# bhansconnect/burn-ppo

Hardware: AMD Instinct MI355X
Metric: env-steps/sec (rollout+GAE+PPO update) at 1/2/4/8 MI355X; steps-to-475-return CartPole (higher is better)
Workload: dtype f32

## Files before the change

### burn-ppo_amd/csrc/bppo_api.hip

```cpp
#include <algorithm>
#include <pthread.h>
#include <chrono>
#include <cmath>
#include <cstdio>
#include <cstdlib>
#include <cstring>
#include <new>
#include <thread>
#include <sys/prctl.h>
#include <x86intrin.h>
#include "bppo_internal.h"
#include "shuffle_host.h"
#include "bppo_wide.h"

using namespace bppo;

namespace bppo {
static double tsc_per_ms() {
    static double v = 0.0;
    if (v == 0.0) {
        const auto t0 = std::chrono::steady_clock::now();
        const uint64_t c0 = __rdtsc();
        std::this_thread::sleep_for(std::chrono::milliseconds(20));
        const uint64_t c1 = __rdtsc();
// ... 210 lines not shown
    }
    c->net = make_layout(*cfg, c->D, c->G, c->A);
    const size_t np = c->net.n_params;
    const size_t TN = (size_t)c->T * c->N;
    c->adam_t.assign(2 * c->net.n_layers, 0);
    TRY(dalloc(c, &c->d_params, np));
    TRY(dalloc(c, &c->d_m1, np));
    TRY(dalloc(c, &c->d_m2, np));
    TRY(dalloc(c, &c->d_grad, np + 64));
    c->slab_rows = 256 * 8;
    c->relu_mfma = cfg->relu ? 1 : 0;
    if (!c->wide) TRY(dalloc(c, &c->d_slab, c->slab_rows * (np + 64)));
    TRY(dalloc(c, &c->d_cp, (size_t)4 * c->N));
    TRY(dalloc(c, &c->d_steps, (size_t)c->N));
    TRY(dalloc(c, &c->d_env_pos, (size_t)c->N));
    TRY(dalloc(c, &c->d_ep_ret, (size_t)c->N * c->P));
    TRY(dalloc(c, &c->d_ep_len, (size_t)c->N));
    if (!c->wide) TRY(dalloc(c, &c->d_obs, TN * c->D));
    TRY(dalloc(c, &c->d_rew, TN));
    TRY(dalloc(c, &c->d_rew_raw, TN));
    TRY(dalloc(c, &c->d_done, TN));
    TRY(dalloc(c, &c->d_val, TN));
    TRY(dalloc(c, &c->d_logp, TN));
    TRY(dalloc(c, &c->d_adv, TN));
    TRY(dalloc(c, &c->d_ret, TN));
    TRY(dalloc(c, &c->d_act, TN));
    if (!c->wide || cfg->normalize_returns) TRY(dalloc(c, &c->d_X, TN));
    if (!c->wide && cfg->hidden_size == 64 && cfg->num_hidden == 2 && cfg->relu)
    {
        TRY(dalloc(c, &c->d_gumbel, TN * 2));
        TRY(dalloc(c, &c->d_rpool, (size_t)RPOOL_K * c->N));
        TRY(dalloc(c, &c->d_rpos, (size_t)RPOOL_K * c->N));
    }
    TRY(dalloc(c, &c->d_on, (size_t)2 * c->D + 1));
    if (!c->wide) TRY(dalloc(c, &c->d_obs_part, (size_t)c->N * 2 * c->D));
    if (!c->wide) {
        TRY(dalloc(c, &c->d_act_in, (size_t)c->N));
        TRY(dalloc(c, &c->d_scr_r, (size_t)c->N));
        TRY(dalloc(c, &c->d_bxc, (size_t)c->N * c->D));
        BPPO_HIP(c, hipMalloc((void **)&c->d_scr_d, (size_t)c->N));
    }
    TRY(dalloc(c, &c->d_rn_returns, (size_t)c->N * c->P));
    TRY(dalloc(c, &c->d_rn_stats, 4));
    TRY(dalloc(c, &c->d_scan_agg, (TN + 4095) / 4096 + 1));
    TRY(dalloc(c, &c->d_last_v, (size_t)c->N));
    c->eps_cap = (int)std::min<size_t>((size_t)c->T * c->N + 4096, (size_t)INT32_MAX / 2);
    TRY(dalloc(c, &c->d_eps, (size_t)c->eps_cap));
    TRY(dalloc(c, &c->d_ep_count, 1));
    TRY(dalloc(c, &c->d_ep_sum, ROLL_HOST_WORDS));
    TRY(dalloc(c, &c->d_err, 1));
    TRY(dalloc(c, &c->d_perm_base, TN));
    c->d_perm = c->d_perm_base;
    TRY(dalloc(c, &c->d_perm_ep, TN * (size_t)cfg->num_epochs));
    TRY(dalloc(c, &c->d_inv_ep, TN * (size_t)cfg->num_epochs));
    TRY(dalloc(c, &c->d_advpart, (size_t)ADV_STREAM_BLOCKS * ADV_STREAM_MAXM * 4));
    BPPO_HIP(c, make_side_stream(dev, &c->fy_stream));
    for (int e = 0; e < cfg->num_epochs && e < SHUF_MAX_EPOCHS; e++)
        BPPO_HIP(c, hipEventCreateWithFlags(&c->fy_ev[e], hipEventDisableTiming));
    TRY(dalloc(c, &c->d_fy, 4 * TN));
    TRY(dalloc(c, &c->d_scan, TN / 8192 + 2));
    BPPO_HIP(c, fy_ranges_init(c->fyr, (uint32_t)TN));
    TRY(dalloc(c, &c->d_red, 4 * 1024 + 64));
    TRY(dalloc(c, &c->d_mb_stats, (size_t)4 * std::max(cfg->num_minibatches, 2)));
    c->d_mb_cur = c->d_mb_stats;
    TRY(dalloc(c, &c->d_rows, (size_t)cfg->num_epochs * cfg->num_minibatches * (WM_COUNT + 4)));
    BPPO_HIP(c, hipHostMalloc((void **)&c->h_rows,
                              sizeof(float) * (size_t)cfg->num_epochs * cfg->num_minibatches * (WM_COUNT + 4),
                              hipHostMallocDefault));
    if (!c->wide && cfg->hidden_size == 64 && cfg->num_hidden == 2 && cfg->relu && c->D == 5)
    {
        BPPO_HIP(c, hipMalloc((void **)&c->d_rowA, sizeof(float4) * 2 * TN));
        BPPO_HIP(c, hipMalloc((void **)&c->d_rowB, sizeof(float2) * TN));
    }
    BPPO_HIP(c, hipHostMalloc((void **)&c->h_red, sizeof(double) * (4 * 1024 + 64 + 2 * ROLL_HOST_WORDS),
                              hipHostMallocDefault));
    BPPO_HIP(c, hipEventCreateWithFlags(&c->ev_upd, hipEventDisableTiming));
    BPPO_HIP(c, hipEventRecord(c->ev_upd, c->stream));
    BPPO_HIP(c, hipEventCreateWithFlags(&c->ev_block, hipEventDisableTiming | hipEventBlockingSync));
    for (int i = 0; i < TM_SLOTS; i++) {
        BPPO_HIP(c, hipEventCreate(&c->ev[i][0]));
        BPPO_HIP(c, hipEventCreate(&c->ev[i][1]));
    }
    for (int i = 0; i < bppo_ctx::MB_EV; i++) {
        BPPO_HIP(c, hipEventCreate(&c->mb_ev[i][0]));
        BPPO_HIP(c, hipEventCreate(&c->mb_ev[i][1]));
    }
    c->rng_key = seed_key(cfg->seed);
    c->rng_pos = 0;
    TRY(c->shuf.init(dev, c->rng_key, cfg->rng_stream, (uint32_t)TN, cfg->num_epochs, TN * (uint64_t)c->A, c->err,
                     cfg->shuffle_windows != 0));
    c->on_mean.assign(c->D, 0.0); c->on_m2.assign(c->D, 0.0); c->on_count = 0;
    c->u_ret = c->d_ret; c->u_val = c->d_val;
    c->shaping_v.assign(1, cfg->reward_shaping_coef); c->shaping_s.assign(1, 0);
    if (cfg->normalize_values) TRY(popart_alloc(c));
    if (c->wide) {
        TRY(wide_init(c));
        TRY(wide_reset(c));
        TRY(wide_pack(c));
    } else {
        TRY(launch_cartpole_reset(c));
    }
    BPPO_HIP(c, sync_stream(c));
    return BPPO_OK;
}

extern "C" bppo_status bppo_create(const bppo_config *cfg, int hip_device, void *hip_stream,
                                   bppo_ctx **out) {
    if (!cfg || !out) return BPPO_ERR_ARG;
    bppo_ctx *c = new bppo_ctx();
    bppo_status s = ctx_init(c, cfg, hip_device, hip_stream);
    *out = c;
    return s;
}

extern "C" void bppo_destroy(bppo_ctx *c) {
    if (!c) return;
    if (c->ev_thread.joinable()) c->ev_thread.join();
    if (c->ev_stream) { (void)hipStreamSynchronize(c->ev_stream); (void)hipStreamDestroy(c->ev_stream); }
    if (c->ev_gae) (void)hipEventDestroy(c->ev_gae);
    if (c->ev_copied) (void)hipEventDestroy(c->ev_copied);
    for (float *h : {c->h_ev_v, c->h_ev_r, c->h_ev_valid}) if (h) (void)hipHostFree(h);
    if (c->fy_stream) (void)hipStreamSynchronize(c->fy_stream);
    c->shuf.shutdown();
    if (c->stream) (void)hipStreamSynchronize(c->stream);
    wide_free(c);
    popart_free(c);
    void *ptrs[] = {c->d_params, c->d_m1, c->d_m2, c->d_grad, c->d_slab, c->d_cp, c->d_steps,
                    c->d_env_pos, c->d_ep_ret, c->d_ep_len, c->d_obs, c->d_rew, c->d_rew_raw,
                    c->d_done, c->d_val, c->d_logp, c->d_adv, c->d_ret, c->d_act, c->d_X, c->d_on,
                    c->d_obs_part, c->d_rn_returns, c->d_rn_stats, c->d_scan_agg, c->d_last_v,
                    c->d_eps, c->d_ep_count, c->d_ep_sum, c->d_err, c->d_perm_base, c->d_perm_ep, c->d_inv_ep, c->d_advpart, c->d_fy, c->d_scan,
                    c->d_red, c->d_mb_stats, c->d_gumbel, c->d_rpool, c->d_rpos, c->d_rows, c->d_rowA, c->d_rowB};
    for (void *p : ptrs) if (p) (void)hipFree(p);
    fy_ranges_free(c->fyr);
    if (c->h_red) (void)hipHostFree(c->h_red);
    if (c->h_rows) (void)hipHostFree(c->h_rows);
    if (c->ev_block) (void)hipEventDestroy(c->ev_block);
    if (c->ev_upd) (void)hipEventDestroy(c->ev_upd);
    for (int i = 0; i < TM_SLOTS; i++) {
        if (c->ev[i][0]) (void)hipEventDestroy(c->ev[i][0]);
        if (c->ev[i][1]) (void)hipEventDestroy(c->ev[i][1]);
    }
    for (auto &pr : c->mb_ev)
        for (hipEvent_t e : pr) if (e) (void)hipEventDestroy(e);
    if (c->fy_stream) { (void)hipStreamSynchronize(c->fy_stream); (void)hipStreamDestroy(c->fy_stream); }
    for (hipEvent_t e : c->fy_ev) if (e) (void)hipEventDestroy(e);
    if (c->own_stream && c->stream) (void)hipStreamDestroy(c->stream);
    delete c;
}

extern "C" size_t bppo_num_params(const bppo_ctx *c) { return c ? c->net.n_params : 0; }

static void drop_prefetch(bppo_ctx *c) {
    if (!c->prefetched) return;
    c->prefetched = false;
    c->collected = 0;
    c->gae_done = 0;
}

extern "C" bppo_status bppo_params_set(bppo_ctx *c, const float *h, size_t n) {
    if (!c || !h || n != c->net.n_params) { if (c) c->err = "params_set: size mismatch"; return BPPO_ERR_ARG; }
    drop_prefetch(c);
    BPPO_HIP(c, hipMemcpyAsync(c->d_params, h, n * 4, hipMemcpyHostToDevice, c->stream));
    if (c->wide) TRY(wide_pack(c));
    BPPO_HIP(c, sync_stream(c));
    return BPPO_OK;
}

extern "C" bppo_status bppo_params_get(bppo_ctx *c, float *h, size_t n) {
    if (!c || !h || n != c->net.n_params) { if (c) c->err = "params_get: size mismatch"; return BPPO_ERR_ARG; }
    BPPO_HIP(c, hipMemcpyAsync(h, c->d_params, n * 4, hipMemcpyDeviceToHost, c->stream));
    BPPO_HIP(c, sync_stream(c));
    return BPPO_OK;
}

extern "C" bppo_status bppo_forward(bppo_ctx *c, const float *obs, const float *priv, int32_t B,
                                    float *logits, float *values) {
    if (!c || !obs || B <= 0) return BPPO_ERR_ARG;
    if (c->wide) return wide_forward_host(c, obs, priv, B, logits, values);
    struct Scratch { float *p[3] = {nullptr, nullptr, nullptr}; ~Scratch() { for (float *q : p) (void)hipFree(q); } } t;
    BPPO_HIP(c, hipMalloc((void **)&t.p[0], sizeof(float) * (size_t)B * c->D));
    BPPO_HIP(c, hipMalloc((void **)&t.p[1], sizeof(float) * (size_t)B * c->A));
    BPPO_HIP(c, hipMalloc((void **)&t.p[2], sizeof(float) * (size_t)B));
    float *d_o = t.p[0], *d_l = t.p[1], *d_v = t.p[2];
    BPPO_HIP(c, hipMemcpyAsync(d_o, obs, sizeof(float) * (size_t)B * c->D, hipMemcpyHostToDevice, c->stream));
    bppo_status s = launch_forward_rows(c, d_o, B, d_l, d_v);
    if (s == BPPO_OK) {
        if (logits) BPPO_HIP(c, hipMemcpyAsync(logits, d_l, sizeof(float) * (size_t)B * c->A, hipMemcpyDeviceToHost, c->stream));
        if (values) BPPO_HIP(c, hipMemcpyAsync(values, d_v, sizeof(float) * (size_t)B, hipMemcpyDeviceToHost, c->stream));
    }
    const bppo_status ss = sync_stream(c) == hipSuccess ? BPPO_OK : BPPO_ERR_HIP;
    return s != BPPO_OK ? s : ss;
}

extern "C" bppo_status bppo_rng_get(bppo_ctx *c, uint64_t *p) {
    if (!c || !p) return BPPO_ERR_ARG;
    *p = c->rng_pos;
    return BPPO_OK;
}
extern "C" bppo_status bppo_rng_set(bppo_ctx *c, uint64_t p) {
    if (!c) return BPPO_ERR_ARG;
    drop_prefetch(c);
    c->shuf_slot = -1;
    c->fy_slot = -1; c->fy_done = 0;
    c->rng_pos = p;
    return BPPO_OK;
}

extern "C" bppo_status bppo_rng_fill_bytes(bppo_ctx *c, uint8_t *dst, size_t n) {
    if (!c || (!dst && n)) return BPPO_ERR_ARG;
    const size_t nw = (n + 3) / 4;
    uint32_t blk[16];
    uint64_t cached = ~0ull;
    for (size_t i = 0; i < nw; i++) {
        const uint64_t pos = c->rng_pos + i;
        if ((pos >> 4) != cached) { chacha12_block(c->rng_key, pos >> 4, c->cfg.rng_stream, blk); cached = pos >> 4; }
        const uint32_t w = blk[pos & 15];
        for (int b = 0; b < 4 && 4 * i + b < n; b++) dst[4 * i + b] = (uint8_t)(w >> (8 * b));
    }
    c->rng_pos += nw;
    c->shuf_slot = -1;
    c->fy_slot = -1; c->fy_done = 0;
    return BPPO_OK;
}

extern "C" bppo_status bppo_rng_from_seed(bppo_ctx *c, const uint8_t *seed) {
    if (!c || !seed) return BPPO_ERR_ARG;
    drop_prefetch(c);
    Key8 k;
    for (int i = 0; i < 8; i++)
        k.k[i] = (uint32_t)seed[4 * i] | ((uint32_t)seed[4 * i + 1] << 8) | ((uint32_t)seed[4 * i + 2] << 16) |
                 ((uint32_t)seed[4 * i + 3] << 24);
    BPPO_HIP(c, sync_stream(c));
    BPPO_HIP(c, hipStreamSynchronize(c->fy_stream));
    c->fy_slot = -1; c->fy_done = 0;
    c->shuf.shutdown();
    c->shuf.~ShuffleEngine();
    new (&c->shuf) ShuffleEngine();
    c->rng_key = k;
    c->rng_pos = 0;
    c->shuf_slot = -1;
    const size_t TN = (size_t)c->T * c->N;
    TRY(c->shuf.init(c->dev, c->rng_key, c->cfg.rng_stream, (uint32_t)TN, c->cfg.num_epochs, TN * (uint64_t)c->A, c->err,
                     c->cfg.shuffle_windows != 0));
    return BPPO_OK;
}

extern "C" bppo_status bppo_rng_key_get(bppo_ctx *c, uint32_t *key) {
    if (!c || !key) return BPPO_ERR_ARG;
    for (int i = 0; i < 8; i++) key[i] = c->rng_key.k[i];
    return BPPO_OK;
}

extern "C" bppo_status bppo_optimizer_get(bppo_ctx *c, float *m1, float *m2, int32_t *steps, size_t n) {
    if (!c || n != c->net.n_params) { if (c) c->err = "optimizer_get: size mismatch"; return BPPO_ERR_ARG; }
    if (m1) BPPO_HIP(c, hipMemcpyAsync(m1, c->d_m1, n * 4, hipMemcpyDeviceToHost, c->stream));
    if (m2) BPPO_HIP(c, hipMemcpyAsync(m2, c->d_m2, n * 4, hipMemcpyDeviceToHost, c->stream));
    BPPO_HIP(c, sync_stream(c));
    if (steps)
        for (int l = 0; l < c->net.n_layers; l++)
            for (int k = 0; k < 2; k++) steps[2 * c->net.rec[l] + k] = c->adam_t[2 * l + k];
    return BPPO_OK;
}

extern "C" bppo_status bppo_optimizer_set(bppo_ctx *c, const float *m1, const float *m2, const int32_t *steps,
                                          size_t n) {
    if (!c || !m1 || !m2 || !steps || n != c->net.n_params) {
        if (c) c->err = "optimizer_set: size mismatch";
        return BPPO_ERR_ARG;
    }
    BPPO_HIP(c, hipMemcpyAsync(c->d_m1, m1, n * 4, hipMemcpyHostToDevice, c->stream));
    BPPO_HIP(c, hipMemcpyAsync(c->d_m2, m2, n * 4, hipMemcpyHostToDevice, c->stream));
    BPPO_HIP(c, sync_stream(c));
    for (int l = 0; l < c->net.n_layers; l++)
        for (int k = 0; k < 2; k++) c->adam_t[2 * l + k] = steps[2 * c->net.rec[l] + k];
    return BPPO_OK;
}

extern "C" size_t bppo_num_param_tensors(const bppo_ctx *c) { return c ? c->adam_t.size() : 0; }

extern "C" bppo_status bppo_vecenv_reset(bppo_ctx *c) {
    if (!c) return BPPO_ERR_ARG;
    drop_prefetch(c);
    TRY(c->wide ? wide_reset(c) : launch_cartpole_reset(c));
    BPPO_HIP(c, sync_stream(c));
    return BPPO_OK;
}

extern "C" bppo_status bppo_vecenv_observe(bppo_ctx *c, float *obs, int32_t *players, uint8_t *masks,
                                           float *priv) {
    (void)priv; (void)masks;
    if (!c) return BPPO_ERR_ARG;
    if (c->wide) return wide_observe_host(c, obs, players, masks, priv);
    if (obs) {
        TRY(launch_cartpole_observe(c, c->d_bxc));
        BPPO_HIP(c, hipMemcpyAsync(obs, c->d_bxc, sizeof(float) * (size_t)c->N * c->D, hipMemcpyDeviceToHost, c->stream));
        BPPO_HIP(c, sync_stream(c));
    }
    if (players) std::fill(players, players + c->N, 0);
    return BPPO_OK;
}

extern "C" bppo_status bppo_vecenv_step(bppo_ctx *c, const int32_t *actions, float *obs, float *rewards,
                                        uint8_t *dones, bppo_episode *eps, int32_t cap, int32_t *n_eps) {
    if (!c || !actions) return BPPO_ERR_ARG;
    const int N = c->N;
    if (c->wide) {
        BPPO_HIP(c, hipMemsetAsync(c->d_ep_count, 0, 4, c->stream));
        int32_t cnt = 0;
        TRY(wide_step_host(c, actions, obs, rewards, dones, &cnt));
        if (n_eps) *n_eps = cnt;
        if (eps && cap > 0 && cnt > 0) {
            std::vector<EpisodeRec> recs(std::min(cnt, c->eps_cap));
            BPPO_HIP(c, hipMemcpy(recs.data(), c->d_eps, sizeof(EpisodeRec) * recs.size(), hipMemcpyDeviceToHost));
            std::sort(recs.begin(), recs.end(), [](const EpisodeRec &a, const EpisodeRec &b) {
                return a.env_index < b.env_index; });
            for (int i = 0; i < (int)recs.size() && i < cap; i++) {
                std::memcpy(eps[i].total_reward, recs[i].total_reward, sizeof(float) * BPPO_MAX_PLAYERS);
                eps[i].length = recs[i].length; eps[i].env_index = recs[i].env_index;
                eps[i].step = recs[i].step; eps[i].pad = 0;
            }
        }
        return BPPO_OK;
    }
    int32_t *d_a = c->d_act_in; float *d_r = c->d_scr_r, *d_o = c->d_bxc; uint8_t *d_d = c->d_scr_d;
    BPPO_HIP(c, hipMemcpyAsync(d_a, actions, sizeof(int32_t) * N, hipMemcpyHostToDevice, c->stream));
    BPPO_HIP(c, hipMemsetAsync(c->d_ep_count, 0, 4, c->stream));
    TRY(launch_cartpole_vecenv_step(c, d_a, d_r, d_d, d_o));
    if (rewards) BPPO_HIP(c, hipMemcpyAsync(rewards, d_r, sizeof(float) * N, hipMemcpyDeviceToHost, c->stream));
    if (dones) BPPO_HIP(c, hipMemcpyAsync(dones, d_d, N, hipMemcpyDeviceToHost, c->stream));
    if (obs) BPPO_HIP(c, hipMemcpyAsync(obs, d_o, sizeof(float) * (size_t)N * c->D, hipMemcpyDeviceToHost, c->stream));
    int32_t cnt = 0;
    BPPO_HIP(c, hipMemcpyAsync(&cnt, c->d_ep_count, 4, hipMemcpyDeviceToHost, c->stream));
    BPPO_HIP(c, sync_stream(c));
    if (n_eps) *n_eps = cnt;
    if (eps && cap > 0 && cnt > 0) {
        std::vector<EpisodeRec> recs(std::min(cnt, c->eps_cap));
        BPPO_HIP(c, hipMemcpy(recs.data(), c->d_eps, sizeof(EpisodeRec) * recs.size(), hipMemcpyDeviceToHost));
        std::sort(recs.begin(), recs.end(), [](const EpisodeRec &a, const EpisodeRec &b) {
            return a.env_index < b.env_index; });
        for (int i = 0; i < (int)recs.size() && i < cap; i++) {
            std::memcpy(eps[i].total_reward, recs[i].total_reward, sizeof(float) * BPPO_MAX_PLAYERS);
            eps[i].length = recs[i].length; eps[i].env_index = recs[i].env_index;
            eps[i].step = recs[i].step; eps[i].pad = 0;
        }
    }
    return BPPO_OK;
}

extern "C" bppo_status bppo_vecenv_set_step(bppo_ctx *c, uint64_t s) {
    if (!c) return BPPO_ERR_ARG;
    c->env_step = s;
    return BPPO_OK;
}

extern "C" bppo_status bppo_set_reward_shaping_schedule(bppo_ctx *c, const double *values, const uint64_t *steps,
                                                        int32_t n) {
    if (!c || n < 0 || (n > 0 && (!values || !steps))) return BPPO_ERR_ARG;
    std::vector<double> v(values, values + n);
    std::vector<uint64_t> s(steps, steps + n);
    if (bppo::schedule_get(v, s, 0) < 0.0) { c->err = "reward_shaping_coef must be >= 0"; return BPPO_ERR_ARG; }
    c->shaping_v = std::move(v); c->shaping_s = std::move(s);
    return BPPO_OK;
}

extern "C" bppo_status bppo_obs_norm_get(bppo_ctx *c, double *mean, double *m2, double *count) {
    if (!c) return BPPO_ERR_ARG;
    std::vector<double> h(2 * c->D + 1);
    BPPO_HIP(c, hipMemcpyAsync(h.data(), c->d_on, sizeof(double) * h.size(), hipMemcpyDeviceToHost, c->stream));
    BPPO_HIP(c, sync_stream(c));
    if (mean) std::memcpy(mean, h.data(), sizeof(double) * c->D);
    if (m2) std::memcpy(m2, h.data() + c->D, sizeof(double) * c->D);
    if (count) *count = h[2 * c->D];
    return BPPO_OK;
}

extern "C" bppo_status bppo_obs_norm_set(bppo_ctx *c, const double *mean, const double *m2, double count) {
    if (!c || !mean || !m2) return BPPO_ERR_ARG;
    drop_prefetch(c);
    std::vector<double> h(2 * c->D + 1);
    std::memcpy(h.data(), mean, sizeof(double) * c->D);
    std::memcpy(h.data() + c->D, m2, sizeof(double) * c->D);
    h[2 * c->D] = count;
    BPPO_HIP(c, hipMemcpyAsync(c->d_on, h.data(), sizeof(double) * h.size(), hipMemcpyHostToDevice, c->stream));
    BPPO_HIP(c, sync_stream(c));
    return BPPO_OK;
}

extern "C" bppo_status bppo_ret_norm_get(bppo_ctx *c, double *mvc, double *returns) {
    if (!c) return BPPO_ERR_ARG;
    if (mvc) BPPO_HIP(c, hipMemcpyAsync(mvc, c->d_rn_stats, sizeof(double) * 3, hipMemcpyDeviceToHost, c->stream));
    if (returns) BPPO_HIP(c, hipMemcpyAsync(returns, c->d_rn_returns, sizeof(double) * (size_t)c->N * c->P, hipMemcpyDeviceToHost, c->stream));
    BPPO_HIP(c, sync_stream(c));
    return BPPO_OK;
}

extern "C" bppo_status bppo_ret_norm_set(bppo_ctx *c, const double *mvc, const double *returns) {
    if (!c) return BPPO_ERR_ARG;
    drop_prefetch(c);
    if (mvc) BPPO_HIP(c, hipMemcpyAsync(c->d_rn_stats, mvc, sizeof(double) * 3, hipMemcpyHostToDevice, c->stream));
    if (returns) BPPO_HIP(c, hipMemcpyAsync(c->d_rn_returns, returns, sizeof(double) * (size_t)c->N * c->P, hipMemcpyHostToDevice, c->stream));
    BPPO_HIP(c, sync_stream(c));
    return BPPO_OK;
}

extern "C" bppo_status bppo_popart_get(bppo_ctx *c, double *st) {
    if (!c || !st) return BPPO_ERR_ARG;
    st[0] = c->pa_mean; st[1] = c->pa_m2; st[2] = c->pa_count; st[3] = c->pa_eps;
    return BPPO_OK;
}

extern "C" bppo_status bppo_popart_set(bppo_ctx *c, const double *st) {
    if (!c || !st) return BPPO_ERR_ARG;
    drop_prefetch(c);
    c->pa_mean = st[0]; c->pa_m2 = st[1]; c->pa_count = st[2]; c->pa_eps = st[3];
    return BPPO_OK;
}

static bppo_status tm_begin(bppo_ctx *c, int slot) {
    BPPO_HIP(c, hipEventRecord(c->ev[slot][0], c->stream));
    return BPPO_OK;
}
static bppo_status tm_end(bppo_ctx *c, int slot) {
    BPPO_HIP(c, hipEventRecord(c->ev[slot][1], c->stream));
    return BPPO_OK;
}
static void tm_read(bppo_ctx *c, int slot) {
    float ms = 0;
    if (event_ms(c->ev[slot][0], c->ev[slot][1], &ms)) c->last_ms[slot] = ms;
}

static bppo_status fy_enqueue_ready(bppo_ctx *c, int slot) {
    const size_t B = (size_t)c->T * c->N;
    if (slot != c->fy_slot) {
        c->fy_slot = slot; c->fy_done = 0;
        BPPO_HIP(c, hipStreamWaitEvent(c->fy_stream, c->ev_upd, 0));
    }
    if (c->shuf.failed(c->err)) return BPPO_ERR_HIP;
    while (c->fy_done < c->cfg.num_epochs && c->shuf.epoch_ready(slot, c->fy_done)) {
        const int e = c->fy_done;
        if (c->shuf.failed(c->err)) return BPPO_ERR_HIP;
        BPPO_HIP(c, hipStreamWaitEvent(c->fy_stream, c->shuf.ev[slot][e], 0));
        if (e > 0) BPPO_HIP(c, hipStreamWaitEvent(c->fy_stream, c->fy_ev[e - 1], 0));
        BPPO_HIP(c, hipEventRecord(c->ev[TM_SHUFFLE][0], c->fy_stream));
        BPPO_HIP(c, fisher_yates_device(c->shuf.d_J[slot] + (size_t)e * B, (uint32_t)B, c->d_fy, c->d_scan,
                                        c->d_perm_ep + (size_t)e * B, c->fy_stream, &c->fyr,
                                        c->d_inv_ep + (size_t)e * B));
        BPPO_HIP(c, hipEventRecord(c->ev[TM_SHUFFLE][1], c->fy_stream));
        BPPO_HIP(c, hipEventRecord(c->fy_ev[e], c->fy_stream));
        c->fy_done++;
    }
    return BPPO_OK;
}

static double *roll_host(bppo_ctx *c, int slot) { return c->h_red + 4 * 1024 + 64 + (size_t)slot * ROLL_HOST_WORDS; }

static bppo_status collect_enqueue(bppo_ctx *c, bool summary) {
    const size_t TN = (size_t)c->T * c->N;
    c->coll_slot ^= 1;
    const int tro = c->coll_slot ? TM_ROLLOUT_B : TM_ROLLOUT, trn = c->coll_slot ? TM_RETNORM_B : TM_RETNORM;
    if (c->wide) {
        BPPO_HIP(c, hipMemsetAsync(c->d_ep_count, 0, 4, c->stream));
        BPPO_HIP(c, hipMemsetAsync(c->d_err, 0, 4, c->stream));
    }
    const uint64_t base = c->rng_pos;
    TRY(tm_begin(c, tro));
    if (c->wide) TRY(wide_collect(c, base));
    else {
        TRY(launch_cartpole_rollout(c, base, nullptr, nullptr, c->cfg.normalize_obs));
        TRY(popart_denorm(c, c->d_val, TN));
    }
    TRY(tm_end(c, tro));
    if (!opp_active(c)) {
        c->shuf_slot = c->shuf.ensure(base + TN * (uint64_t)c->A);
        TRY(fy_enqueue_ready(c, c->shuf_slot));
    }
    if (opp_active(c)) {
        TRY(opp_rollout_end(c));
    } else {
        c->rng_pos = base + TN * (uint64_t)c->A;
        c->shuf_slot = c->shuf.ensure(c->rng_pos);
    }
    if (c->cfg.normalize_obs) TRY(launch_obs_norm_merge(c));
    TRY(tm_begin(c, trn));
    if (c->cfg.normalize_returns) TRY(launch_return_norm(c));
    else if (!c->wide) BPPO_HIP(c, hipMemcpyAsync(c->d_rew, c->d_rew_raw, TN * 4, hipMemcpyDeviceToDevice, c->stream));
    TRY(tm_end(c, trn));
    int32_t *hv = reinterpret_cast<int32_t *>(roll_host(c, c->coll_slot));
    if (summary) {
        TRY(launch_episode_summary(c, c->d_ep_sum));
        BPPO_HIP(c, hipMemcpyAsync(hv, c->d_ep_sum, sizeof(double) * ROLL_HOST_WORDS, hipMemcpyDeviceToHost, c->stream));
    } else {
        BPPO_HIP(c, hipMemcpyAsync(&hv[0], c->d_ep_count, 4, hipMemcpyDeviceToHost, c->stream));
        BPPO_HIP(c, hipMemcpyAsync(&hv[1], c->d_err, 4, hipMemcpyDeviceToHost, c->stream));
    }
    c->collected = 1; c->gae_done = 0;
    c->rollout_rng_pos[c->coll_slot] = c->rng_pos;
    return BPPO_OK;
}

static bppo_status collect_finish(bppo_ctx *c, bppo_rollout_info *info, int slot) {
    float ms = 0;
    const int tro = slot ? TM_ROLLOUT_B : TM_ROLLOUT, trn = slot ? TM_RETNORM_B : TM_RETNORM;
    if (event_ms(c->ev[tro][0], c->ev[tro][1], &ms)) c->last_ms[TM_ROLLOUT] = ms;
    if (event_ms(c->ev[trn][0], c->ev[trn][1], &ms)) c->last_ms[TM_RETNORM] = ms;
    const int32_t *hv = reinterpret_cast<const int32_t *>(roll_host(c, slot));
    const double *part = roll_host(c, slot) + 2;
    if (hv[1] & 2) { c->err = "Empty action mask: an env has no valid action"; return BPPO_ERR_EMPTY_MASK; }
    if (hv[1] & 1) { c->err = "NaN/Inf in log probs — model producing corrupt logits"; return BPPO_ERR_NONFINITE; }
    if (hv[1] & 4) { c->err = "opponent pool: pos_to_opp names a model index outside [0, n_models)"; return BPPO_ERR_ARG; }
    if (hv[1] & 8) { c->err = "Invalid action: outside the env's action mask"; return BPPO_ERR_ARG; }
    if (hv[1]) { c->err = "collect_rollouts: unknown device error flag"; return BPPO_ERR_HIP; }
    if (info) {
        info->episodes = hv[0];
        info->rng_word_pos = c->rollout_rng_pos[slot];
        info->mean_return = 0; info->mean_length = 0;
        const int n = std::min(hv[0], c->eps_cap);
        if (n > 0) {
            double sr = 0, sl = 0;
            for (int b = 0; b < EP_SUMMARY_BLOCKS; b++) { sr += part[2 * b]; sl += part[2 * b + 1]; }
            info->mean_return = (float)(sr / n); info->mean_length = (float)(sl / n);
        }
    }
    return BPPO_OK;
}

extern "C" bppo_status bppo_collect_rollouts(bppo_ctx *c, bppo_rollout_info *info) {
    if (!c) return BPPO_ERR_ARG;
    if (c->prefetched) c->prefetched = false;
    else TRY(collect_enqueue(c, info != nullptr));
    BPPO_HIP(c, sync_stream(c));
    return collect_finish(c, info, c->coll_slot);
}

extern "C" bppo_status bppo_rollout_episodes(bppo_ctx *c, bppo_episode *eps, int32_t cap, int32_t *n) {
    if (!c) return BPPO_ERR_ARG;
    int32_t cnt = 0;
    BPPO_HIP(c, hipMemcpyAsync(&cnt, c->d_ep_count, 4, hipMemcpyDeviceToHost, c->stream));
    BPPO_HIP(c, sync_stream(c));
    int m = std::min(cnt, c->eps_cap);
    std::vector<EpisodeRec> recs(m);
    if (m) {
        BPPO_HIP(c, hipMemcpyAsync(recs.data(), c->d_eps, sizeof(EpisodeRec) * m, hipMemcpyDeviceToHost, c->stream));
        BPPO_HIP(c, sync_stream(c));
    }
    std::sort(recs.begin(), recs.end(), [](const EpisodeRec &a, const EpisodeRec &b) {
        return a.step != b.step ? a.step < b.step : a.env_index < b.env_index; });
    for (int i = 0; i < m && i < cap; i++) {
        std::memcpy(eps[i].total_reward, recs[i].total_reward, sizeof(float) * BPPO_MAX_PLAYERS);
        eps[i].length = recs[i].length; eps[i].env_index = recs[i].env_index;
        eps[i].step = recs[i].step; eps[i].pad = 0;
    }
    if (n) *n = cnt;
    return BPPO_OK;
}

static bppo_status gae_enqueue(bppo_ctx *c) {
    c->prefetched = false;
    if (c->wide) {
        TRY(tm_begin(c, TM_GAE));
        TRY(wide_bootstrap_gae(c));
        TRY(tm_end(c, TM_GAE));
        c->gae_done = 1;
        return BPPO_OK;
    }
    TRY(tm_begin(c, TM_BOOT));
    TRY(launch_bootstrap(c, nullptr, nullptr, c->cfg.normalize_obs));
    TRY(popart_denorm(c, c->d_last_v, (size_t)c->N));
    TRY(tm_end(c, TM_BOOT));
    TRY(tm_begin(c, TM_GAE));
    bool packed = false;
    hipError_t he = hipSuccess;
    bppo_status s = launch_gae_1p(c->d_rew, c->d_done, c->d_val, c->d_last_v, c->T, c->N,
                                  (float)c->cfg.gamma, (float)c->cfg.gae_lambda, c->d_adv, c->d_ret,
                                  c->stream, c->rows_from_rollout ? c->d_rowB : nullptr, &packed, &he);
    c->rows_packed = packed;
    if (s != BPPO_OK) return he != hipSuccess ? hip_fail(c, he, "k_gae_1p launch") : s;
    TRY(tm_end(c, TM_GAE));
    c->gae_done = 1;
    return BPPO_OK;
}

extern "C" bppo_status bppo_compute_gae(bppo_ctx *c) {
    if (!c || !c->collected) { if (c) c->err = "compute_gae before collect_rollouts"; return BPPO_ERR_ARG; }
    TRY(gae_enqueue(c));
    BPPO_HIP(c, sync_stream(c));
    if (!c->wide) tm_read(c, TM_BOOT);
    tm_read(c, TM_GAE);
    return BPPO_OK;
}

static float ev_reference_f32(const float *v, const float *r, const float *valid, size_t n_all) {
#pragma clang fp contract(off)
    size_t n_ = 0;
    float s_r = 0.0f, s_res = 0.0f;
    for (size_t i = 0; i < n_all; i++) {
        if (valid && !(valid[i] > 0.5f)) continue;
        s_r += r[i];
        s_res += r[i] - v[i];
        n_++;
    }
    const float n = (float)n_;
    if (n < 2.0f) return 0.0f;
    const float mr = s_r / n, mres = s_res / n;
    float q_r = 0.0f, q_res = 0.0f;
    for (size_t i = 0; i < n_all; i++) {
        if (valid && !(valid[i] > 0.5f)) continue;
        const float d = r[i] - mr;
        q_r += d * d;
        const float e = (r[i] - v[i]) - mres;
        q_res += e * e;
    }
    const float vr = q_r / n;
    if (vr < 1e-8f) return 0.0f;
    return 1.0f - (q_res / n) / vr;
}

extern "C" bppo_status bppo_set_explained_variance_mode(bppo_ctx *c, int32_t mode) {
    if (!c || mode < 0 || mode > 1) return BPPO_ERR_ARG;
    if (mode == 1 && !c->h_ev_v) {
        const size_t TN = (size_t)c->T * c->N;
        hipStream_t st = nullptr;
        hipEvent_t e_gae = nullptr, e_cp = nullptr;
        float *hv = nullptr, *hr = nullptr, *hm = nullptr;
        hipError_t e = hipStreamCreateWithFlags(&st, hipStreamNonBlocking);
        if (e == hipSuccess) e = hipEventCreateWithFlags(&e_gae, hipEventDisableTiming);
        if (e == hipSuccess) e = hipEventCreateWithFlags(&e_cp, hipEventDisableTiming | hipEventBlockingSync);
        if (e == hipSuccess) e = hipHostMalloc((void **)&hv, TN * 4, hipHostMallocDefault);
        if (e == hipSuccess) e = hipHostMalloc((void **)&hr, TN * 4, hipHostMallocDefault);
        if (e == hipSuccess) e = hipHostMalloc((void **)&hm, TN * 4, hipHostMallocDefault);
        if (e != hipSuccess) {
            for (float *h : {hv, hr, hm}) if (h) (void)hipHostFree(h);
            if (e_cp) (void)hipEventDestroy(e_cp);
            if (e_gae) (void)hipEventDestroy(e_gae);
            if (st) (void)hipStreamDestroy(st);
            return hip_fail(c, e, "explained-variance reference mode: allocation");
        }
        c->ev_stream = st; c->ev_gae = e_gae; c->ev_copied = e_cp;
        c->h_ev_r = hr; c->h_ev_valid = hm;
        c->h_ev_v = hv;
    }
    c->ev_mode = mode;
    return BPPO_OK;
}

extern "C" bppo_status bppo_debug_record_params(bppo_ctx *c, float *host, int32_t max_minibatches) {
    if (!c || max_minibatches < 0) return BPPO_ERR_ARG;
    c->dbg_params = max_minibatches > 0 ? host : nullptr;
    c->dbg_params_max = host ? max_minibatches : 0;
    return BPPO_OK;
}

extern "C" bppo_status bppo_set_minibatch_kernel(bppo_ctx *c, int32_t mode) {
    if (!c || mode < 0 || mode > 2) return BPPO_ERR_ARG;
    c->mb_kernel = mode;
    return BPPO_OK;
}

static bppo_status ev_reference_begin(bppo_ctx *c, const float *d_valid) {
    const size_t TN = (size_t)c->T * c->N;
    if (c->ev_thread.joinable()) c->ev_thread.join();
    BPPO_HIP(c, hipEventRecord(c->ev_gae, c->stream));
    BPPO_HIP(c, hipStreamWaitEvent(c->ev_stream, c->ev_gae, 0));
    BPPO_HIP(c, hipMemcpyAsync(c->h_ev_v, c->d_val, TN * 4, hipMemcpyDeviceToHost, c->ev_stream));
    BPPO_HIP(c, hipMemcpyAsync(c->h_ev_r, c->d_ret, TN * 4, hipMemcpyDeviceToHost, c->ev_stream));
    if (d_valid) BPPO_HIP(c, hipMemcpyAsync(c->h_ev_valid, d_valid, TN * 4, hipMemcpyDeviceToHost, c->ev_stream));
    BPPO_HIP(c, hipEventRecord(c->ev_copied, c->ev_stream));
    const bool vf = d_valid != nullptr;
    c->ev_thread = std::thread([c, TN, vf]() {
        (void)pthread_setname_np(pthread_self(), "bppo-ev");
        (void)hipEventSynchronize(c->ev_copied);
        c->ev_ref = ev_reference_f32(c->h_ev_v, c->h_ev_r, vf ? c->h_ev_valid : nullptr, TN);
    });
    return BPPO_OK;
}

extern "C" bppo_status bppo_ppo_update(bppo_ctx *c, double lr, double ent_coef, bppo_update_metrics *m) {
    if (!c || !c->gae_done) { if (c) c->err = "ppo_update before compute_gae"; return BPPO_ERR_ARG; }
    const bool opp = opp_active(c);
    if (opp) {
        if (c->fy_done > 0) BPPO_HIP(c, hipStreamWaitEvent(c->stream, c->fy_ev[c->fy_done - 1], 0));
        c->fy_slot = -1; c->fy_done = 0;
        c->d_perm = c->d_perm_base;
        TRY(opp_compact_valid(c));
    }
    if (!opp && c->shuf_slot < 0) c->shuf_slot = c->shuf.ensure(c->rng_pos);
    const int slot = c->shuf_slot;
    const size_t B = opp ? (size_t)c->n_valid : (size_t)c->T * c->N;
    std::vector<uint32_t> Jh(opp ? std::max<size_t>(B, 1) * c->cfg.num_epochs : 0);
    uint64_t opp_pos = c->rng_pos;
    const int M = c->cfg.num_minibatches;
    const size_t base_mb = B / M, rem = B % M;
    const int np = (int)c->net.n_params;
    const int NM = WM_COUNT;
    std::vector<float> rows;
    int epochs_run = 0;
    bool stop = false;
    double wait_ms = 0.0;
    TRY(tm_begin(c, TM_UPDATE));
    struct EvCopyGuard {
        bppo_ctx *c; bool armed = false;
        ~EvCopyGuard() { if (armed) (void)hipStreamWaitEvent(c->stream, c->ev_copied, 0); }
    } ev_guard{c};
    if (c->ev_mode == 1) { TRY(ev_reference_begin(c, opp ? c->d_valid : nullptr)); ev_guard.armed = true; }
    TRY(popart_update_begin(c, opp ? c->d_valid : nullptr));
    if (c->d_rowA && !c->rows_packed) TRY(launch_pack_rows(c));
    c->rows_packed = false;
    float fw_ms = 0, sh_ms = 0;
    const bool deferred = c->cfg.target_kl < 0 && !(c->allreduce && c->world > 1 && !c->allreduce_async);
    int nrow = 0;
    const int last_run_mb = (base_mb > 0 || (c->allreduce && c->world > 1)) ? M - 1 : (int)rem - 1;
    bool fw_recorded = false;
    bool first_mb = true;
    size_t rows_done = 0;
    for (int ep = 0; ep < c->cfg.num_epochs && !stop; ep++) {
        epochs_run++;
        hipEvent_t s0 = c->ev[TM_SHUFFLE][0], s1 = c->ev[TM_SHUFFLE][1];
        if (opp) {
            uint32_t *J = Jh.data() + (size_t)ep * B;
            auto w0 = std::chrono::steady_clock::now();
            opp_pos = shuffle_walk_host(c->rng_key, c->cfg.rng_stream, opp_pos, (uint32_t)B, J);
            wait_ms += std::chrono::duration<double, std::milli>(std::chrono::steady_clock::now() - w0).count();
            BPPO_HIP(c, hipMemcpyAsync(c->d_Jopp, J, sizeof(uint32_t) * B, hipMemcpyHostToDevice, c->stream));
            BPPO_HIP(c, hipEventRecord(s0, c->stream));
            if (B) TRY(launch_fisher_yates(c, c->d_Jopp, (uint32_t)B));
            if (B) TRY(opp_map_perm(c, (uint32_t)B));
            BPPO_HIP(c, hipEventRecord(s1, c->stream));
        } else {
            if (slot != c->fy_slot || ep >= c->fy_done) {
                auto w0 = std::chrono::steady_clock::now();
                c->shuf.wait_epoch(slot, ep);
                wait_ms += std::chrono::duration<double, std::milli>(std::chrono::steady_clock::now() - w0).count();
            }
            TRY(fy_enqueue_ready(c, slot));
            BPPO_HIP(c, hipStreamWaitEvent(c->stream, c->fy_ev[ep], 0));
            c->d_perm = c->d_perm_ep + (size_t)ep * B;
        }
        const bool lockstep = c->allreduce && c->world > 1;
        if (B == 0 && !lockstep) continue;
        if (B) TRY(launch_epoch_adv_stats(c, (uint32_t)B, M, opp ? nullptr : c->d_inv_ep + (size_t)ep * B));
        size_t start = 0;
        for (int mb = 0; mb < M; mb++) {
            const size_t sz = base_mb + ((size_t)mb < rem ? 1 : 0);
            if (sz == 0 && !lockstep) continue;
            const bool fw_timed = !deferred || (ep == c->cfg.num_epochs - 1 && mb == last_run_mb);
            if (fw_timed) BPPO_HIP(c, hipEventRecord(c->ev[TM_FWDBWD][0], c->stream));
            c->d_mb_cur = c->d_mb_stats + 4 * mb;
            float c1[64], c2[64];
            for (int t = 0; t < 2 * c->net.n_layers; t++) {
                int ti = ++c->adam_t[t];
                c1[t] = 1.0f - powi_f32(0.9f, ti);
                c2[t] = 1.0f - powi_f32(0.999f, ti);
            }
            float *metric_dst = c->d_rows + (size_t)nrow * (NM + 4);
            const bool multi = c->allreduce && c->world > 1;
            if (sz == 0) {
                BPPO_HIP(c, hipMemsetAsync(c->d_grad, 0, sizeof(float) * ((size_t)np + 64), c->stream));
                BPPO_HIP(c, hipMemsetAsync(c->d_mb_cur, 0, sizeof(float) * 4, c->stream));
                static const float ninf = -INFINITY;
                BPPO_HIP(c, hipMemcpyAsync(c->d_grad + np + GRAD_VEMAX_LOCAL, &ninf, sizeof(float),
                                           hipMemcpyHostToDevice, c->stream));
            } else if (c->wide) {
                if (c->dbg_params && nrow < c->dbg_params_max)
                    BPPO_HIP(c, hipMemcpyAsync(c->dbg_params + (size_t)nrow * np, c->d_params, sizeof(float) * np,
                                               hipMemcpyDeviceToHost, c->stream));
                TRY(wide_minibatch(c, (uint32_t)start, (uint32_t)sz, ent_coef, first_mb));
            } else {
                if (c->dbg_params && nrow < c->dbg_params_max)
                    BPPO_HIP(c, hipMemcpyAsync(c->dbg_params + (size_t)nrow * np, c->d_params, sizeof(float) * np,
                                               hipMemcpyDeviceToHost, c->stream));
                TRY(launch_minibatch(c, (uint32_t)start, (uint32_t)sz, (float)ent_coef, first_mb));
            }
            if (fw_timed) { BPPO_HIP(c, hipEventRecord(c->ev[TM_FWDBWD][1], c->stream)); fw_recorded = true; }
            first_mb = false;
            if (multi) {
                if (!c->allreduce_async) BPPO_HIP(c, sync_stream(c));
                if (c->allreduce(c->d_grad, (size_t)np + NM, c->allreduce_user) != 0) {
                    c->err = "all-reduce callback failed";
                    return BPPO_ERR_COMM;
                }
            }
            TRY(launch_adam(c, (float)lr, c1, c2, metric_dst, NM));
            if (c->wide) TRY(wide_pack(c));
            nrow++;
            if (!deferred) {
                std::vector<float> row(NM + 4);
                BPPO_HIP(c, hipMemcpyAsync(row.data(), c->d_rows + (size_t)(nrow - 1) * (NM + 4), sizeof(float) * (NM + 4),
                                           hipMemcpyDeviceToHost, c->stream));
                BPPO_HIP(c, sync_stream(c));
                float ms = 0;
                if (event_ms(c->ev[TM_FWDBWD][0], c->ev[TM_FWDBWD][1], &ms)) fw_ms = ms;
                if (mb == 0 && event_ms(s0, s1, &ms)) sh_ms = ms;
                rows.insert(rows.end(), row.begin(), row.end());
            }
            if (!deferred && c->cfg.target_kl >= 0) {
                const float *row = &rows[rows.size() - (NM + 4)];
                const float n = row[10] > 0 ? row[10] : 1.0f;
                if (row[3] / n > (float)c->cfg.target_kl) { stop = true; rows_done = start + sz; break; }
            }
            start += sz;
        }
    }
    if (deferred && nrow > 0) {
        rows.resize((size_t)nrow * (NM + 4));
        BPPO_HIP(c, hipMemcpyAsync(c->h_rows, c->d_rows, sizeof(float) * rows.size(), hipMemcpyDeviceToHost, c->stream));
    }
    TRY(tm_end(c, TM_UPDATE));
    c->last_wait_ms = wait_ms;
    c->last_walk_ms = 0.0;
    c->last_met = 0;
    if (opp) {
        c->rng_pos = opp_pos;
        c->last_walk_ms = wait_ms;
        BPPO_HIP(c, hipStreamSynchronize(c->stream));
    } else {
        c->rng_pos = c->shuf.win ? c->shuf.job_end(slot) : c->shuf.end_pos[slot][epochs_run - 1];
        for (int e = 0; e < epochs_run; e++) {
            c->last_walk_ms += c->shuf.walk_ms[slot][e];
            c->last_met += c->shuf.coalesced[slot][e] >= 0 && e > 0;
        }
        c->last_spec_mwords = (double)c->shuf.spec_words.exchange(0) * 1e-6;
        c->last_true_mwords = (double)c->shuf.true_words.exchange(0) * 1e-6;
        c->last_walk_cpu_ms = (double)c->shuf.tsc_walk.exchange(0) / tsc_per_ms();
        c->last_words_cpu_ms = (double)c->shuf.tsc_words.exchange(0) / tsc_per_ms();
        c->shuf_slot = -1;
        if (c->fy_slot == slot && c->fy_done > 0)
            BPPO_HIP(c, hipStreamWaitEvent(c->stream, c->fy_ev[c->fy_done - 1], 0));
        c->fy_slot = -1;
        c->fy_done = 0;
        BPPO_HIP(c, c->shuf.release(slot, c->stream));
        c->shuf.ensure(c->rng_pos + (uint64_t)c->T * c->N * (uint64_t)c->A);
    }
    TRY(popart_target_stats(c, stop ? epochs_run - 1 : epochs_run, rows_done, opp ? c->d_valid : nullptr));
    TRY(launch_explained_variance(c, opp ? c->d_valid : nullptr));
    if (ev_guard.armed) { ev_guard.armed = false; BPPO_HIP(c, hipStreamWaitEvent(c->stream, c->ev_copied, 0)); }
    BPPO_HIP(c, hipEventRecord(c->ev_upd, c->stream));
    if (c->prefetch_next) {
        c->prefetch_next = false;
        c->env_step = c->prefetch_env_step;
        TRY(collect_enqueue(c, true));
        c->prefetched = true;
        BPPO_HIP(c, wait_event(c, c->ev_upd));
    } else {
        BPPO_HIP(c, sync_stream(c));
    }
    if (deferred && nrow > 0) {
        std::memcpy(rows.data(), c->h_rows, sizeof(float) * rows.size());
        float ms = 0;
        if (fw_recorded && event_ms(c->ev[TM_FWDBWD][0], c->ev[TM_FWDBWD][1], &ms)) fw_ms = ms;
        if (event_ms(c->ev[TM_SHUFFLE][0], c->ev[TM_SHUFFLE][1], &ms)) sh_ms = ms;
    }
    double ev4[4];
    explained_variance_sums(c, ev4);
    if (c->ev_thread.joinable()) c->ev_thread.join();
    tm_read(c, TM_UPDATE);
    if (c->mb_ev_n > 0) {
        double sum = 0.0, ks[2] = {0.0, 0.0};
        float lo = INFINITY, hi = 0.0f;
        int n = 0, kn[2] = {0, 0};
        for (int i = 0; i < c->mb_ev_n; i++) {
            float ms = 0.0f;
            if (!event_ms(c->mb_ev[i][0], c->mb_ev[i][1], &ms)) continue;
            sum += ms; lo = std::min(lo, ms); hi = std::max(hi, ms); n++;
            ks[c->mb_ev_split[i]] += ms; kn[c->mb_ev_split[i]]++;
        }
        if (n) { c->mb_k_mean = (float)(sum / n); c->mb_k_min = lo; c->mb_k_max = hi; }
        c->mb_k_exact = kn[0] ? (float)(ks[0] / kn[0]) : 0.0f;
        c->mb_k_split = kn[1] ? (float)(ks[1] / kn[1]) : 0.0f;
        c->mb_ev_n = 0;
    }
    c->mb_launch = 0;
    c->last_ms[TM_FWDBWD] = fw_ms;
    c->last_ms[TM_SHUFFLE] = sh_ms;
    c->last_rows = rows;
    if (m) {
        std::memset(m, 0, sizeof *m);
        const int nup = (int)(rows.size() / (NM + 4));
        float tp = 0, tv = 0, th = 0, tk = 0, tc = 0, tl = 0, tvm = 0, trm = 0, tam = 0, tas = 0;
        float tamin = INFINITY, tamax = -INFINITY, tvem = 0, tves = 0, tvemax = -INFINITY;
        float tav = 0, tevp = 0;
        for (int u = 0; u < nup; u++) {
            const float *r = &rows[(size_t)u * (NM + 4)];
            const float n = r[10] > 0 ? r[10] : 1.0f;
            const float pl = r[0] / n, vl = 0.5f * (r[1] / n), h = r[2] / n;
            tp += pl; tv += vl; th += h; tk += r[3] / n; tc += r[4] / n;
            tl += pl + vl * (float)c->cfg.value_coef + (-h) * (float)ent_coef;
            tvm += r[5] / n; trm += r[6] / n;
            const float vem = r[7] / n;
            tvem += vem;
            const double var = n > 1 ? ((double)r[8] - (double)n * vem * vem) / (double)(n - 1) : 0.0;
            tves += sqrtf((float)std::max(var, 0.0));
            tvemax = std::max(tvemax, r[9]);
            tav += r[WM_VALID] / n;
            tevp += r[WM_NCHOICE] > 0 ? r[WM_HV] / r[WM_NCHOICE] : 0.0f;
            tam += r[NM]; tas += r[NM + 1];
            tamin = std::min(tamin, r[NM + 2]); tamax = std::max(tamax, r[NM + 3]);
        }
        const float n = (float)nup;
        m->policy_loss = tp / n; m->value_loss = tv / n; m->entropy = th / n;
        m->entropy_scaled = m->entropy / logf((float)c->A);
        m->approx_kl = tk / n; m->clip_fraction = tc / n; m->total_loss = tl / n;
        m->value_mean = tvm / n; m->returns_mean = trm / n;
        m->adv_mean_raw = tam / n; m->adv_std_raw = tas / n; m->adv_min_raw = tamin; m->adv_max_raw = tamax;
        m->value_error_mean = tvem / n; m->value_error_std = tves / n; m->value_error_max = tvemax;
        const double Bn = (double)B;
        const double mr = ev4[0] / Bn, vr = ev4[1] / Bn - mr * mr;
        const double mres = ev4[2] / Bn, vres = ev4[3] / Bn - mres * mres;
        m->explained_variance = (B < 2 || vr < 1e-8) ? 0.0f : (float)(1.0 - vres / vr);
        if (c->ev_mode == 1) m->explained_variance = c->ev_ref;
        if (c->cfg.env_kind != BPPO_ENV_CARTPOLE) { m->avg_valid_actions = tav / n; m->entropy_valid_pct = tevp / n; }
        m->num_updates = nup; m->epochs_run = epochs_run;
        m->value_norm_target_mean = m->value_norm_target_std = NAN;
        m->value_norm_rescale_mag = c->pa_rescale_mag;
        if (c->cfg.normalize_values && c->pa_tcount > 0) {
            const double mean = c->pa_tsum / c->pa_tcount, var = c->pa_tsq / c->pa_tcount - mean * mean;
            m->value_norm_target_mean = (float)mean;
            m->value_norm_target_std = (float)std::sqrt(std::max(var, 0.0));
        }
    }
    c->collected = 0; c->gae_done = 0;
    return BPPO_OK;
}

extern "C" bppo_status bppo_train_step(bppo_ctx *c, double lr, double ent_coef, bppo_rollout_info *info,
                                       bppo_update_metrics *m) {
    if (!c) return BPPO_ERR_ARG;
    const auto t0 = std::chrono::steady_clock::now();
    c->sync_wait_ms = 0.0;
    if (c->prefetched) c->prefetched = false;
    else TRY(collect_enqueue(c, info != nullptr));
    TRY(gae_enqueue(c));
    const bppo_status us = bppo_ppo_update(c, lr, ent_coef, m);
    if (us == BPPO_OK) { if (!c->wide) tm_read(c, TM_BOOT); tm_read(c, TM_GAE); }
    const bppo_status cs = collect_finish(c, info, c->coll_slot);
    c->last_host_ms = std::chrono::duration<double, std::milli>(std::chrono::steady_clock::now() - t0).count() -
                      c->sync_wait_ms;
    c->last_sync_ms = c->sync_wait_ms;
    return cs != BPPO_OK ? cs : us;
}

extern "C" bppo_status bppo_train_steps(bppo_ctx *c, int32_t n, const double *lr, const double *ent_coef,
                                        uint64_t global_step0, bppo_rollout_info *infos, bppo_update_metrics *ms,
                                        const char *const *phase_keys, int32_t nkeys, float *phase_sums) {
    if (!c || n < 0 || !lr || !ent_coef || (nkeys > 0 && (!phase_keys || !phase_sums))) return BPPO_ERR_ARG;
    for (int k = 0; k < nkeys; k++) phase_sums[k] = 0.0f;
    const uint64_t TN = (uint64_t)c->T * c->N * (uint64_t)c->world;
    for (int32_t k = 0; k < n; k++) {
        const auto t0 = std::chrono::steady_clock::now();
        c->sync_wait_ms = 0.0;
        if (!c->prefetched) { c->env_step = global_step0 + (uint64_t)k * TN; TRY(collect_enqueue(c, true)); }
        c->prefetched = false;
        const int slot = c->coll_slot;
        TRY(gae_enqueue(c));
        c->prefetch_next = k + 1 < n;
        c->prefetch_env_step = global_step0 + (uint64_t)(k + 1) * TN;
        const bppo_status us = bppo_ppo_update(c, lr[k], ent_coef[k], ms ? &ms[k] : nullptr);
        c->prefetch_next = false;
        if (us != BPPO_OK) { (void)sync_stream(c); c->collected = c->prefetched ? 1 : 0; return us; }
        if (!c->wide) tm_read(c, TM_BOOT);
        tm_read(c, TM_GAE);
        const bppo_status cs = collect_finish(c, infos ? &infos[k] : nullptr, slot);
        if (cs != BPPO_OK) { (void)sync_stream(c); c->collected = c->prefetched ? 1 : 0; return cs; }
        c->last_host_ms = std::chrono::duration<double, std::milli>(std::chrono::steady_clock::now() - t0).count() -
                          c->sync_wait_ms;
        c->last_sync_ms = c->sync_wait_ms;
        for (int q = 0; q < nkeys; q++) {
            float v = 0.0f;
            if (bppo_last_kernel_ms(c, phase_keys[q], &v) == BPPO_OK) phase_sums[q] += v;
        }
    }
    return BPPO_OK;
}

static bppo_status check_world(bppo_ctx *c, int32_t world) {
    if (world > 1 && c->cfg.normalize_values) {
        if (c->d_pa_gather) { BPPO_HIP(c, hipFree(c->d_pa_gather)); c->d_pa_gather = nullptr; }
        BPPO_HIP(c, hipMalloc((void **)&c->d_pa_gather, sizeof(float) * 9 * (size_t)world));
    }
    return BPPO_OK;
}

extern "C" bppo_status bppo_set_rank(bppo_ctx *c, int32_t rank) {
    if (!c || rank < 0) return BPPO_ERR_ARG;
    c->rank = rank;
    return BPPO_OK;
}

extern "C" bppo_status bppo_set_allreduce(bppo_ctx *c, bppo_allreduce_fn fn, void *user, int32_t world) {
    if (!c || world < 1) return BPPO_ERR_ARG;
    TRY(check_world(c, world));
    c->allreduce = fn; c->allreduce_user = user; c->world = world; c->allreduce_async = 0;
    return BPPO_OK;
}

extern "C" bppo_status bppo_set_allreduce_async(bppo_ctx *c, bppo_allreduce_fn fn, void *user, int32_t world) {
    if (!c || world < 1) return BPPO_ERR_ARG;
    TRY(check_world(c, world));
    c->allreduce = fn; c->allreduce_user = user; c->world = world; c->allreduce_async = 1;
    return BPPO_OK;
}

extern "C" bppo_status bppo_get_stream(bppo_ctx *c, void **stream) {
    if (!c || !stream) return BPPO_ERR_ARG;
    *stream = (void *)c->stream;
    return BPPO_OK;
}

struct BufDesc { void *ptr; size_t bytes; };
static BufDesc find_buf(bppo_ctx *c, const char *name) {
    const size_t TN = (size_t)c->T * c->N;
    if (!strcmp(name, "obs")) return {c->d_obs, TN * c->D * 4};
    if (!strcmp(name, "actions")) return {c->d_act, TN * 4};
    if (!strcmp(name, "rewards")) return {c->d_rew, TN * 4};
    if (!strcmp(name, "raw_rewards")) return {c->d_rew_raw, TN * 4};
    if (!strcmp(name, "valid")) return {c->d_valid, c->d_valid ? TN * 4 : 0};
    if (!strcmp(name, "dones")) return {c->d_done, TN * 4};
    if (!strcmp(name, "values")) return {c->d_val, TN * 4};
    if (!strcmp(name, "log_probs")) return {c->d_logp, TN * 4};
    if (!strcmp(name, "advantages")) return {c->d_adv, TN * 4};
    if (!strcmp(name, "returns")) return {c->d_ret, TN * 4};
    if (!strcmp(name, "all_rewards")) return {c->d_rew, TN * 4};
    if (!strcmp(name, "perm")) return {c->d_perm, TN * 4};
    if (!strncmp(name, "perm_ep:", 8)) {
        const int e = atoi(name + 8);
        if (e < 0 || e >= c->cfg.num_epochs || !c->d_perm_ep) return {nullptr, 0};
        return {c->d_perm_ep + (size_t)e * TN, TN * 4};
    }
    if (!strcmp(name, "last_values")) return {c->d_last_v, (size_t)c->N * 4};
    if (!strcmp(name, "grad")) return {c->d_grad, c->net.n_params * 4};
    return {nullptr, 0};
}

extern "C" bppo_status bppo_buffer_get(bppo_ctx *c, const char *name, void *host, size_t bytes) {
    if (!c || !name || !host) return BPPO_ERR_ARG;
    if (c->wide) {
        bool handled = false;
        bppo_status s = wide_buffer_get(c, name, host, bytes, &handled);
        if (handled) return s;
    }
    BufDesc b = find_buf(c, name);
    if (!b.ptr || bytes < b.bytes) { c->err = std::string("buffer_get: unknown buffer or too small: ") + name; return BPPO_ERR_ARG; }
    BPPO_HIP(c, hipMemcpyAsync(host, b.ptr, b.bytes, hipMemcpyDeviceToHost, c->stream));
    BPPO_HIP(c, sync_stream(c));
    return BPPO_OK;
}

extern "C" int32_t bppo_minibatch_rows(bppo_ctx *c, float *out, int32_t max_rows, int32_t *row_width) {
    if (!c) return -1;
    const int32_t w = WM_COUNT + 4;
    const int32_t n = (int32_t)(c->last_rows.size() / (size_t)w);
    if (row_width) *row_width = w;
    if (out && max_rows > 0)
        std::memcpy(out, c->last_rows.data(), sizeof(float) * (size_t)std::min(n, max_rows) * (size_t)w);
    return n;
}

extern "C" bppo_status bppo_buffer_set(bppo_ctx *c, const char *name, const void *host, size_t bytes) {
    if (!c || !name || !host) return BPPO_ERR_ARG;
    BufDesc b = find_buf(c, name);
    if (!b.ptr || bytes != b.bytes) { c->err = std::string("buffer_set: unknown buffer or size mismatch: ") + name; return BPPO_ERR_ARG; }
    BPPO_HIP(c, hipMemcpyAsync(b.ptr, host, b.bytes, hipMemcpyHostToDevice, c->stream));
    BPPO_HIP(c, sync_stream(c));
    if (!strcmp(name, "advantages") || !strcmp(name, "returns")) c->gae_done = c->collected = 1;
    c->rows_packed = c->rows_from_rollout = false;
    return BPPO_OK;
}

extern "C" bppo_status bppo_gae_device(const float *r, const float *d, const float *v, const float *lv,
                                       int32_t T, int32_t N, float gamma, float lambda, float *adv,
                                       float *ret, void *stream) {
    if (!r || !d || !v || !lv || !adv || !ret || T < 0 || N < 0) return BPPO_ERR_ARG;
    return launch_gae_1p(r, d, v, lv, T, N, gamma, lambda, adv, ret, (hipStream_t)stream);
}

extern "C" bppo_status bppo_gae_rows_device(const float *r, const float *d, const float *v, const float *lv,
                                            int32_t T, int32_t N, float gamma, float lambda, float *adv,
                                            float *ret, float *rows, void *stream) {
    if (!r || !d || !v || !lv || !adv || !ret || !rows || T < 0 || N < 0) return BPPO_ERR_ARG;
    if (N % 4 != 0 || T > 128 ||
        ((uintptr_t)r | (uintptr_t)d | (uintptr_t)v | (uintptr_t)lv | (uintptr_t)adv | (uintptr_t)ret | (uintptr_t)rows) % 16)
        return BPPO_ERR_UNSUPPORTED;
    bool packed = false;
    const bppo_status s = launch_gae_1p(r, d, v, lv, T, N, gamma, lambda, adv, ret, (hipStream_t)stream,
                                        reinterpret_cast<float2 *>(rows), &packed);
    return s != BPPO_OK ? s : packed ? BPPO_OK : BPPO_ERR_UNSUPPORTED;
}

extern "C" bppo_status bppo_gae_mp_device(const float *ar, const int32_t *pl, const float *d,
                                          const float *v, const float *lvpp, int32_t T, int32_t N,
                                          int32_t P, float gamma, float lambda, float *adv, float *ret,
                                          void *stream) {
    if (!ar || !pl || !d || !v || !lvpp || !adv || !ret || T < 0 || N < 0 || P < 1 || P > BPPO_MAX_PLAYERS)
        return BPPO_ERR_ARG;
    return launch_gae_mp(ar, pl, d, v, lvpp, T, N, P, gamma, lambda, adv, ret, (hipStream_t)stream);
}

extern "C" bppo_status bppo_last_kernel_ms(bppo_ctx *c, const char *k, float *ms) {
    if (!c || !k || !ms) return BPPO_ERR_ARG;
    static const char *names[8] = {"rollout", "gae", "update", "minibatch", "return_norm", "shuffle",
                                   "adam", "bootstrap"};
    for (int i = 0; i < 8; i++)
        if (!strcmp(k, names[i])) { *ms = c->last_ms[i]; return BPPO_OK; }
    if (!strcmp(k, "shuffle_walk")) { *ms = (float)c->last_walk_ms; return BPPO_OK; }
    if (!strcmp(k, "minibatch_kernel")) { *ms = c->mb_k_mean; return BPPO_OK; }
    if (!strcmp(k, "minibatch_kernel_min")) { *ms = c->mb_k_min; return BPPO_OK; }
    if (!strcmp(k, "minibatch_kernel_max")) { *ms = c->mb_k_max; return BPPO_OK; }
    if (!strcmp(k, "minibatch_kernel_split")) { *ms = c->mb_k_split; return BPPO_OK; }
    if (!strcmp(k, "minibatch_kernel_exact")) { *ms = c->mb_k_exact; return BPPO_OK; }
    if (!strcmp(k, "shuffle_wait")) { *ms = (float)c->last_wait_ms; return BPPO_OK; }
    if (!strcmp(k, "host_enqueue")) { *ms = (float)c->last_host_ms; return BPPO_OK; }
    if (!strcmp(k, "host_sync_wait")) { *ms = (float)c->last_sync_ms; return BPPO_OK; }
    if (!strcmp(k, "shuffle_walk_tsc_ms")) { *ms = (float)c->last_walk_cpu_ms; return BPPO_OK; }
    if (!strcmp(k, "shuffle_words_tsc_ms")) { *ms = (float)c->last_words_cpu_ms; return BPPO_OK; }
    if (!strcmp(k, "shuffle_spec_mwords")) { *ms = (float)c->last_spec_mwords; return BPPO_OK; }
    if (!strcmp(k, "shuffle_true_mwords")) { *ms = (float)c->last_true_mwords; return BPPO_OK; }
    if (!strcmp(k, "shuffle_met")) { *ms = (float)c->last_met; return BPPO_OK; }
    return BPPO_ERR_ARG;
}

extern "C" bppo_status bppo_debug_libm(int32_t which, int32_t device, const float *x, float *y, size_t n) {
    if (!x || !y) return BPPO_ERR_ARG;
    if (!device) {
        for (size_t i = 0; i < n; i++) {
            float v = x[i];
            switch (which) {
            case 0: y[i] = bppo_math::logf_glibc(v); break;
            case 1: y[i] = bppo_math::sinf_glibc(v); break;
            case 2: y[i] = bppo_math::cosf_glibc(v); break;
            case 3: y[i] = -bppo_math::logf_glibc(-bppo_math::logf_glibc(v)); break;
            case 5: y[i] = bppo_math::tanhf_glibc(v); break;
            default: y[i] = bppo_math::expf_glibc(v); break;
            }
        }
        return BPPO_OK;
    }
    float *dx = nullptr, *dy = nullptr;
    if (hipMalloc((void **)&dx, n * 4) != hipSuccess || hipMalloc((void **)&dy, n * 4) != hipSuccess) return BPPO_ERR_HIP;
    bppo_status s = BPPO_ERR_HIP;
    if (hipMemcpy(dx, x, n * 4, hipMemcpyHostToDevice) == hipSuccess &&
        launch_libm(which, dx, dy, n) == BPPO_OK && hipDeviceSynchronize() == hipSuccess &&
        hipMemcpy(y, dy, n * 4, hipMemcpyDeviceToHost) == hipSuccess)
        s = BPPO_OK;
    (void)hipFree(dx); (void)hipFree(dy);
    return s;
}

extern "C" bppo_status bppo_debug_shuffle_chain(uint64_t seed, uint64_t stream, uint64_t word_pos, uint32_t n,
                                                uint32_t *J, uint64_t *end_pos) {
    if (!J && n) return BPPO_ERR_ARG;
    const Key8 key = seed_key(seed);
    const uint64_t e = shuffle_walk_host(key, stream, word_pos, n, J);
    if (end_pos) *end_pos = e;
    return BPPO_OK;
}

extern "C" bppo_status bppo_debug_chain_walk2(uint64_t seed, uint64_t stream, uint64_t pos_a, uint64_t pos_b,
                                              uint32_t n, uint32_t piece, uint64_t *end_a, uint64_t *end_b) {
    if (!end_a || !end_b || piece < 1) return BPPO_ERR_ARG;
    const Key8 key = seed_key(seed);
    struct Ch { uint64_t pos; uint32_t r; std::vector<uint32_t> w; size_t off, left; } ch[2];
    ch[0].pos = pos_a; ch[1].pos = pos_b;
    auto refill = [&](Ch &c) {
        const uint64_t q = (c.pos / piece + 1) * piece;
        c.w.resize(q - c.pos);
        bppo_host::chacha12_words(key.k, stream, c.pos, c.w.data(), c.w.size());
        c.off = 0;
        c.left = c.w.size();
    };
    for (Ch &c : ch) { c.r = n; refill(c); }
    auto live = [](const Ch &c) { return c.r >= 2; };
    auto advance = [&](Ch &c, size_t u) {
        c.off += u; c.left -= u; c.pos += u;
        if (live(c) && c.left == 0) refill(c);
    };
    while (live(ch[0]) && live(ch[1])) {
        size_t u0 = 0, u1 = 0;
        bppo_host::chain_walk2_nj(ch[0].w.data() + ch[0].off, ch[0].left, &ch[0].r, &u0,
                                  ch[1].w.data() + ch[1].off, ch[1].left, &ch[1].r, &u1);
        advance(ch[0], u0);
        advance(ch[1], u1);
    }
    for (Ch &c : ch)
        while (live(c)) advance(c, bppo_host::chain_walk_nj(c.w.data() + c.off, c.left, &c.r));
    *end_a = ch[0].pos;
    *end_b = ch[1].pos;
    return BPPO_OK;
}

extern "C" bppo_status bppo_debug_shuffle_engine(uint64_t seed, uint64_t stream, uint64_t start, uint32_t n,
                                                 int32_t epochs, uint64_t gap, int32_t jobs, int32_t windows,
                                                 uint32_t *J, uint64_t *ends, int32_t *met) {
    if (!J || !ends || n < 2 || epochs < 1 || epochs > SHUF_MAX_EPOCHS || jobs < 1) return BPPO_ERR_ARG;
    ShuffleEngine *e = new ShuffleEngine();
    std::string err;
    bppo_status s = e->init(0, seed_key(seed), stream, n, epochs, gap, err, windows != 0);
    uint64_t pos = start;
    for (int j = 0; j < jobs && s == BPPO_OK; j++) {
        const int slot = e->ensure(pos);
        for (int k = 0; k < epochs; k++) e->wait_epoch(slot, k);
        const size_t o = (size_t)j * epochs;
        if (hipStreamSynchronize(e->copy) != hipSuccess ||
            hipMemcpy(J + o * n, e->d_J[slot], sizeof(uint32_t) * (size_t)n * epochs, hipMemcpyDeviceToHost) != hipSuccess)
            s = BPPO_ERR_HIP;
        for (int k = 0; k < epochs; k++) {
            ends[o + k] = e->end_pos[slot][k];
            if (met) met[o + k] = e->coalesced[slot][k];
        }
        pos = e->job_end(slot) + gap;
    }
    e->shutdown();
    delete e;
    return s;
}

extern "C" bppo_status bppo_debug_fisher_yates(int32_t device, const uint32_t *J, uint32_t n, uint32_t *perm) {
    if (!J || !perm) return BPPO_ERR_ARG;
// ... 51 lines not shown
```

### burn-ppo_amd/csrc/bppo_internal.h

```cpp
#pragma once
#include <hip/hip_runtime.h>
#include <stdint.h>
#include <stddef.h>
#include <stdlib.h>
#include <string>
#include <vector>
#include <thread>
#include <mutex>
#include <condition_variable>
#include <atomic>
#include <memory>
#include "../../include/bppo.h"
#include "bppo_device.h"

namespace bppo {

struct NetLayout {
    static constexpr int MAX_LAYERS = 16;
    int n_layers = 0;
    int in[MAX_LAYERS], out[MAX_LAYERS];
    size_t w[MAX_LAYERS], b[MAX_LAYERS];
    int n_actor_hidden = 0;
    int policy = 0, value = 0;
    int critic_first = -1;
// ... 173 lines not shown

struct bppo_ctx {
    bppo_config cfg;
    int dev = 0;
    hipStream_t stream = nullptr;
    bool own_stream = false;
    std::string err;
    int N = 0, T = 0, D = 0, A = 0, P = 1, G = 0;
    int Pa = 1;
    bppo::NetLayout net;
    float *d_params = nullptr, *d_m1 = nullptr, *d_m2 = nullptr;
    std::vector<int32_t> adam_t;
    float *d_grad = nullptr;
    double *d_grad64 = nullptr;
    float *d_slab = nullptr;
    size_t slab_rows = 0;
    int slab_used = 0;
    int relu_mfma = 1;
    int mb_kernel = 0;
    float *dbg_params = nullptr;
    int dbg_params_max = 0;
    float *d_cp = nullptr;
    int32_t *d_steps = nullptr;
    uint64_t *d_env_pos = nullptr;
    float *d_ep_ret = nullptr;
    int32_t *d_ep_len = nullptr;
    uint64_t env_step = 0;
    std::vector<double> shaping_v;
    std::vector<uint64_t> shaping_s;
    float *d_obs = nullptr, *d_rew = nullptr, *d_rew_raw = nullptr, *d_done = nullptr;
    float *d_val = nullptr, *d_logp = nullptr, *d_adv = nullptr, *d_ret = nullptr;
    int32_t *d_act = nullptr;
    double *d_X = nullptr;
    float *d_gumbel = nullptr;
    float4 *d_rpool = nullptr;
    uint64_t *d_rpos = nullptr;
    double *d_on = nullptr;
    std::vector<double> on_mean, on_m2;
    double on_count = 0;
    double *d_obs_part = nullptr;
    double *d_rn_returns = nullptr;
    double *d_rn_stats = nullptr;
    bppo::Welford *d_scan_agg = nullptr;
    float *d_last_v = nullptr;
    bppo::EpisodeRec *d_eps = nullptr;
    int32_t *d_ep_count = nullptr;
    int32_t eps_cap = 0;
    double *d_ep_sum = nullptr;
    int32_t *d_err = nullptr;
    bppo::Key8 rng_key{};
    uint64_t rng_pos = 0;
    bppo::ShuffleEngine shuf;
    uint32_t *d_perm = nullptr;
    uint32_t *d_perm_base = nullptr;
    uint32_t *d_perm_ep = nullptr;
    uint32_t *d_inv_ep = nullptr;
    double *d_advpart = nullptr;
    hipStream_t fy_stream = nullptr;
    hipEvent_t fy_ev[bppo::SHUF_MAX_EPOCHS] = {};
    int fy_slot = -1, fy_done = 0;
    uint32_t *d_fy = nullptr;
    uint32_t *d_scan = nullptr;
    bppo::FyRanges fyr;
    int shuf_slot = -1;
    double *d_red = nullptr;
    double *h_red = nullptr;
    float *h_rows = nullptr;
    float *d_mb_stats = nullptr;
    float *d_mb_cur = nullptr;
    float *d_rows = nullptr;
    std::vector<float> last_rows;
    float4 *d_rowA = nullptr;
    float2 *d_rowB = nullptr;
    bppo_allreduce_fn allreduce = nullptr;
    void *allreduce_user = nullptr;
    int world = 1;
    int rank = -1;
    float *d_pa_gather = nullptr;
    int allreduce_async = 0;
    int wide = 0;
    int L = 0;
    int rows_max = 0;
    void *d_wstate = nullptr;
    float *d_xc = nullptr;
    float *d_obs_raw = nullptr;
    int opp_K = 0, n_opp = 0;
    float *d_opp_params = nullptr;
    double *d_opp_on = nullptr;
    std::vector<int> opp_has_norm;
    int32_t *d_lpos = nullptr, *d_p2o = nullptr, *d_curopp = nullptr;
    int32_t *d_group = nullptr, *d_gpos = nullptr;
    float *d_valid = nullptr;
    uint64_t *d_rngpos = nullptr;
    float *d_oraw = nullptr, *d_oxc = nullptr, *d_ologits = nullptr;
    uint32_t *d_vidx = nullptr, *d_Jopp = nullptr;
    uint32_t *d_nvalid = nullptr;
    uint32_t n_valid = 0;
    int32_t *d_gbase = nullptr, *h_gbase = nullptr;
    double *d_obsw_part = nullptr;
    size_t obsw_part_n = 0;
    uint8_t *d_mask = nullptr;
    int32_t *d_players = nullptr;
    float *d_allr = nullptr;
    float *d_lvpp = nullptr;
    float *d_hbuf = nullptr;
    size_t hoff[16] = {};
    float *d_logits = nullptr, *d_values = nullptr;
    float *d_xcg = nullptr;
    float *d_dout = nullptr;
    float *d_dz[2] = {nullptr, nullptr};
    float *d_heads = nullptr, *d_heads_b = nullptr;
    float *d_part = nullptr, *d_colsum = nullptr;
    double *d_mpart = nullptr;
    float *d_cnn_y[2][4] = {};
    float *d_cnn_f[2] = {nullptr, nullptr};
    float *d_cnn_dy[2] = {nullptr, nullptr};
    float *d_cnn_wt = nullptr, *d_cnn_wd = nullptr, *d_cnn_owt = nullptr, *d_cnn_dwt = nullptr;
    size_t cnn_wt_off[2][4] = {};
    size_t cnn_wd_off[2][4] = {};
    int cnn_stacks = 1;
    double pa_mean = 0.0, pa_m2 = 0.0, pa_count = 0.0, pa_eps = 1e-4;
    float pa_rescale_mag = 0.0f;
    double pa_tsum = 0.0, pa_tsq = 0.0, pa_tcount = 0.0;
    float *d_ret_n = nullptr, *d_val_n = nullptr;
    double *d_pa_part = nullptr;
    const float *u_ret = nullptr, *u_val = nullptr;
    float *d_bxc = nullptr;
    uint8_t *d_bmask = nullptr;
    int32_t *d_bplayers = nullptr;
    int32_t *d_act_in = nullptr;
    float *d_scr_r = nullptr;
    uint8_t *d_scr_d = nullptr;
    hipEvent_t ev[bppo::TM_SLOTS][2] = {};
    hipEvent_t ev_block = nullptr;
    float last_ms[8] = {0};
    double last_walk_ms = 0.0, last_wait_ms = 0.0;
    double sync_wait_ms = 0.0, last_host_ms = 0.0, last_sync_ms = 0.0;
    double wait_est_us = 0.0;
    static constexpr int MB_EV = 64;
    hipEvent_t mb_ev[MB_EV][2] = {};
    int mb_ev_n = 0;
    int mb_launch = 0;
    float mb_k_mean = 0.0f, mb_k_min = 0.0f, mb_k_max = 0.0f;
    bool mb_ev_split[MB_EV] = {};
    float mb_k_split = 0.0f, mb_k_exact = 0.0f;
    double last_spec_mwords = 0.0, last_true_mwords = 0.0;
    double last_walk_cpu_ms = 0.0, last_words_cpu_ms = 0.0;
    int last_met = 0;
    int collected = 0, gae_done = 0;
    hipEvent_t ev_upd = nullptr;
    int coll_slot = 1;
    uint64_t rollout_rng_pos[2] = {0, 0};
    bool prefetch_next = false, prefetched = false;
    bool rows_from_rollout = false, rows_packed = false;
    uint64_t prefetch_env_step = 0;
    int ev_mode = 0;
    hipStream_t ev_stream = nullptr;
    hipEvent_t ev_gae = nullptr, ev_copied = nullptr;
    float *h_ev_v = nullptr, *h_ev_r = nullptr, *h_ev_valid = nullptr;
    std::thread ev_thread;
    float ev_ref = 0.0f;
};

namespace bppo {
inline bool env_set(const char *name) { return getenv(name) != nullptr; }
inline int env_int(const char *name, int dflt) {
    const char *v = getenv(name);
    return v ? atoi(v) : dflt;
}
enum { TM_ROLLOUT = 0, TM_GAE = 1, TM_UPDATE = 2, TM_FWDBWD = 3, TM_RETNORM = 4, TM_SHUFFLE = 5,
       TM_ADAM = 6, TM_BOOT = 7 };
enum { TM_ROLLOUT_B = 8, TM_RETNORM_B = 9 };

bppo_status launch_cartpole_reset(bppo_ctx *c);
bppo_status launch_cartpole_rollout(bppo_ctx *c, uint64_t base_pos, const double *mean,
                                    const double *sd, int norm_on);
bppo_status launch_cartpole_vecenv_step(bppo_ctx *c, const int32_t *d_actions, float *d_rew,
                                        uint8_t *d_done, float *d_obs_out);
bppo_status launch_cartpole_observe(bppo_ctx *c, float *d_obs_out);
bppo_status launch_obs_norm_merge(bppo_ctx *c);
bppo_status launch_episode_summary(bppo_ctx *c, double *host_slot);
bppo_status launch_obs_norm_rows(bppo_ctx *c, int rows, float *x, int ld, float *raw);
bppo_status launch_obs_norm_rows_on(bppo_ctx *c, int rows, float *x, int ld, float *raw, const double *on);
bppo_status launch_bootstrap(bppo_ctx *c, const double *mean, const double *sd, int norm_on);
bppo_status launch_forward_rows(bppo_ctx *c, const float *d_obs, int B, float *d_logits,
                                float *d_values);
bppo_status launch_gae_1p(const float *r, const float *d, const float *v, const float *lv, int T,
                          int N, float gamma, float lambda, float *adv, float *ret, hipStream_t s,
                          float2 *pairs = nullptr, bool *pairs_done = nullptr, hipError_t *herr = nullptr);
bppo_status launch_gae_mp(const float *ar, const int32_t *pl, const float *d, const float *v,
                          const float *lvpp, int T, int N, int P, float gamma, float lambda,
                          float *adv, float *ret, hipStream_t s, hipError_t *herr = nullptr);
bppo_status launch_return_norm(bppo_ctx *c);
bppo_status launch_fisher_yates(bppo_ctx *c, const uint32_t *d_J, uint32_t n);
hipError_t fisher_yates_device(const uint32_t *d_J, uint32_t n, uint32_t *scratch, uint32_t *scan, uint32_t *perm,
                               hipStream_t st, const FyRanges *rg, uint32_t *inv = nullptr);
hipError_t fy_ranges_init(FyRanges &r, uint32_t n);
void fy_ranges_free(FyRanges &r);
bppo_status launch_epoch_adv_stats(bppo_ctx *c, uint32_t B, int M, const uint32_t *inv = nullptr);
bppo_status launch_minibatch(bppo_ctx *c, uint32_t start, uint32_t n, float ent_coef, bool exact);
bppo_status launch_adam(bppo_ctx *c, float lr, const float *c1, const float *c2, float *metric_dst = nullptr,
                        int nm = 0);
bppo_status launch_metric_row(bppo_ctx *c, float *dst, int nm);
bppo_status launch_pack_rows(bppo_ctx *c);
bppo_status launch_explained_variance(bppo_ctx *c, const float *valid);
void explained_variance_sums(bppo_ctx *c, double *out4);
bppo_status wide_init(bppo_ctx *c);
void wide_free(bppo_ctx *c);
bppo_status wide_reset(bppo_ctx *c);
bppo_status wide_pack(bppo_ctx *c);
bppo_status wide_forward(bppo_ctx *c, int rows, const float *xc, int ldxc, float *logits, float *values,
                         int split = 0);
bppo_status wide_forward_actor(bppo_ctx *c, int rows, const float *xc, int ldxc, const float *params, float *logits);
bppo_status cnn_alloc(bppo_ctx *c);
void cnn_free(bppo_ctx *c);
bppo_status cnn_pack(bppo_ctx *c, const float *params, float *wt, float *wd);
bppo_status cnn_features(bppo_ctx *c, int s, int rows, const float *x, int ldx, const float *params, const float *wt);
bppo_status cnn_backward(bppo_ctx *c, int s, int rows, const float *x, int ldx, float *dF, float *grad, int exact);
inline int wide_exact_grad(const bppo_ctx *c) {
    if (c->mb_kernel == 1) return 2;
    return c->mb_kernel == 0 ? 1 : 0;
}
bool opp_active(const bppo_ctx *c);
bppo_status opp_alloc(bppo_ctx *c);
void opp_free(bppo_ctx *c);
bppo_status opp_rollout_begin(bppo_ctx *c, uint64_t base);
bppo_status opp_step_group(bppo_ctx *c, int t);
bppo_status opp_step_forwards(bppo_ctx *c);
bppo_status opp_step_seats(bppo_ctx *c, int t);
bppo_status opp_rollout_end(bppo_ctx *c);
bppo_status opp_compact_valid(bppo_ctx *c);
bppo_status opp_map_perm(bppo_ctx *c, uint32_t n);
bppo_status wide_collect(bppo_ctx *c, uint64_t base);
bppo_status wide_bootstrap_gae(bppo_ctx *c);
bppo_status wide_minibatch(bppo_ctx *c, uint32_t start, uint32_t n, double ent_coef, bool first);
bppo_status wide_observe_host(bppo_ctx *c, float *obs, int32_t *players, uint8_t *masks, float *priv);
bppo_status wide_step_host(bppo_ctx *c, const int32_t *actions, float *obs, float *rewards, uint8_t *dones,
                           int32_t *n_eps);
bppo_status wide_forward_host(bppo_ctx *c, const float *obs, const float *priv, int B, float *logits,
                              float *values);
bppo_status wide_buffer_get(bppo_ctx *c, const char *name, void *host, size_t bytes, bool *handled);
double popart_std(const bppo_ctx *c);

inline double schedule_get(const std::vector<double> &v, const std::vector<uint64_t> &s, uint64_t step) {
    const size_t n = v.size();
    if (n == 0) return 0.0;
    if (n == 1 || step <= s[0]) return v[0];
    for (size_t i = 0; i + 1 < n; i++)
        if (step >= s[i] && step < s[i + 1]) {
            const double t = (double)(step - s[i]) / (double)(s[i + 1] - s[i]);
            return v[i] + (v[i + 1] - v[i]) * t;
        }
    return v[n - 1];
}
inline float shaping_coef(const bppo_ctx *c) { return (float)schedule_get(c->shaping_v, c->shaping_s, c->env_step); }
bppo_status popart_alloc(bppo_ctx *c);
void popart_free(bppo_ctx *c);
bppo_status popart_denorm(bppo_ctx *c, float *v, size_t n);
bppo_status popart_update_begin(bppo_ctx *c, const float *valid);
bppo_status popart_target_stats(bppo_ctx *c, int full_epochs, size_t rows_done, const float *valid);
bppo_status launch_libm(int which, const float *d_x, float *d_y, size_t n);

inline bppo_status hip_fail(bppo_ctx *c, hipError_t e, const char *what) {
    if (c) c->err = std::string(what) + ": " + hipGetErrorString(e);
    return BPPO_ERR_HIP;
}
inline bppo_status launch_check(bppo_ctx *c, const char *kernel) {
    const hipError_t e = hipGetLastError();
    return e == hipSuccess ? BPPO_OK : hip_fail(c, e, kernel);
}
inline hipError_t event_query(hipEvent_t ev) {
    const hipError_t e = hipEventQuery(ev);
    if (e != hipSuccess) (void)hipGetLastError();
    return e;
}
inline bool event_ms(hipEvent_t a, hipEvent_t b, float *ms) {
    const hipError_t e = hipEventElapsedTime(ms, a, b);
    if (e != hipSuccess) (void)hipGetLastError();
    return e == hipSuccess;
}
}

#define TRY(x)                                 \
    do {                                       \
        bppo_status _s = (x);                  \
        if (_s != BPPO_OK) return _s;          \
    } while (0)

#define BPPO_HIP(c, expr)                                                   \
    do {                                                                    \
        hipError_t _e = (expr);                                             \
        if (_e != hipSuccess) return bppo::hip_fail((c), _e, #expr);        \
    } while (0)
```

### burn-ppo_amd/csrc/k_gae.hip

```cpp
#include "bppo_internal.h"
#include <algorithm>

namespace bppo {

constexpr int GAE_UNROLL = 8;

__global__ void __launch_bounds__(256) k_gae_1p(const float *__restrict__ r,
                                                const float *__restrict__ d,
                                                const float *__restrict__ v,
                                                const float *__restrict__ lv, int T, int N,
                                                float gamma, float lambda, float *__restrict__ adv,
                                                float *__restrict__ ret) {
    const int e = blockIdx.x * blockDim.x + threadIdx.x;
    if (e >= N) return;
    const float gl = gamma * lambda;
    float last = 0.0f;
    float nv = lv[e];
    int t = T - 1;
    for (; t >= GAE_UNROLL - 1; t -= GAE_UNROLL) {
        float rr[GAE_UNROLL], dd[GAE_UNROLL], vv[GAE_UNROLL];
#pragma unroll
        for (int u = 0; u < GAE_UNROLL; u++) {
            const size_t i = (size_t)(t - u) * N + e;
            rr[u] = r[i]; dd[u] = d[i]; vv[u] = v[i];
        }
#pragma unroll
        for (int u = 0; u < GAE_UNROLL; u++) {
            const size_t i = (size_t)(t - u) * N + e;
            const float om = 1.0f - dd[u];
            const float delta = __fsub_rn(__builtin_fmaf(gamma * nv, om, rr[u]), vv[u]);
            last = __builtin_fmaf(gl * om, last, delta);
            adv[i] = last;
            ret[i] = __fadd_rn(last, vv[u]);
            nv = vv[u];
        }
    }
    for (; t >= 0; t--) {
        const size_t i = (size_t)t * N + e;
        const float vv = v[i], om = 1.0f - d[i];
        const float delta = __fsub_rn(__builtin_fmaf(gamma * nv, om, r[i]), vv);
        last = __builtin_fmaf(gl * om, last, delta);
        adv[i] = last;
        ret[i] = __fadd_rn(last, vv);
        nv = vv;
    }
}

constexpr int GSEG_WAVES = 16, GSEG_L = 8;
__global__ void __launch_bounds__(GSEG_WAVES * 64) k_gae_1p_seg(const float4 *__restrict__ r,
                                                                 const float4 *__restrict__ d,
                                                                 const float4 *__restrict__ v,
                                                                 const float4 *__restrict__ lv, int T, int N4,
                                                                 int L, float gamma, float lambda,
                                                                 float4 *__restrict__ adv, float4 *__restrict__ ret,
                                                                 float2 *__restrict__ pairs) {
    __shared__ float4 carry[GSEG_WAVES][64];
    const int lane = threadIdx.x & 63, w = threadIdx.x >> 6;
    const int g = blockIdx.x * 64 + lane;
    const bool ok = g < N4;
    const int t0 = w * L, n = max(0, min(T, t0 + L) - t0);
    const float gl = gamma * lambda;
    float4 x0[GSEG_L], x1[GSEG_L], vv[GSEG_L], vnext = make_float4(0.f, 0.f, 0.f, 0.f);
    if (ok) {
#pragma unroll
        for (int u = 0; u < GSEG_L; u++)
            if (u < n) {
                const size_t i = (size_t)(t0 + u) * N4 + g;
                x0[u] = r[i]; x1[u] = d[i]; vv[u] = v[i];
            }
        if (n > 0) vnext = t0 + n < T ? v[(size_t)(t0 + n) * N4 + g] : lv[g];
    }
#pragma unroll
    for (int u = 0; u < GSEG_L; u++) {
        if (u >= n) continue;
        const float4 nv = u + 1 < n ? vv[u + 1 < GSEG_L ? u + 1 : u] : vnext;
        float4 &a = x0[u], &b = x1[u];
        const float4 vu = vv[u];
        float om;
        om = 1.0f - b.x; a.x = __fsub_rn(__builtin_fmaf(gamma * nv.x, om, a.x), vu.x); b.x = gl * om;
        om = 1.0f - b.y; a.y = __fsub_rn(__builtin_fmaf(gamma * nv.y, om, a.y), vu.y); b.y = gl * om;
        om = 1.0f - b.z; a.z = __fsub_rn(__builtin_fmaf(gamma * nv.z, om, a.z), vu.z); b.z = gl * om;
        om = 1.0f - b.w; a.w = __fsub_rn(__builtin_fmaf(gamma * nv.w, om, a.w), vu.w); b.w = gl * om;
    }
    for (int k = GSEG_WAVES - 1; k >= 0; k--) {
        if (w == k) {
            float4 A = k == GSEG_WAVES - 1 ? make_float4(0.f, 0.f, 0.f, 0.f) : carry[k + 1][lane];
#pragma unroll
            for (int u = GSEG_L - 1; u >= 0; u--) {
                if (u >= n) continue;
                A.x = __builtin_fmaf(x1[u].x, A.x, x0[u].x);
                A.y = __builtin_fmaf(x1[u].y, A.y, x0[u].y);
                A.z = __builtin_fmaf(x1[u].z, A.z, x0[u].z);
                A.w = __builtin_fmaf(x1[u].w, A.w, x0[u].w);
                x0[u] = A;
            }
            carry[k][lane] = A;
        }
        __syncthreads();
    }
    if (!ok) return;
#pragma unroll
    for (int u = 0; u < GSEG_L; u++) {
        if (u >= n) continue;
        const size_t i = (size_t)(t0 + u) * N4 + g;
        const float4 A = x0[u], vu = vv[u];
        adv[i] = A;
        const float4 R = make_float4(__fadd_rn(A.x, vu.x), __fadd_rn(A.y, vu.y), __fadd_rn(A.z, vu.z), __fadd_rn(A.w, vu.w));
        ret[i] = R;
        if (pairs) {
            float4 *o = reinterpret_cast<float4 *>(pairs + 4 * i);
            o[0] = make_float4(A.x, R.x, A.y, R.y);
            o[1] = make_float4(A.z, R.z, A.w, R.w);
        }
    }
}

template <int P>
__global__ void __launch_bounds__(256) k_gae_mp(const float *__restrict__ ar,
                                                const int32_t *__restrict__ pl,
                                                const float *__restrict__ d,
                                                const float *__restrict__ v,
                                                const float *__restrict__ lvpp, int T, int N,
                                                float gamma, float lambda, float *__restrict__ adv,
                                                float *__restrict__ ret) {
    const int e = blockIdx.x * blockDim.x + threadIdx.x;
    if (e >= N) return;
    const float gl = gamma * lambda;
    float carry[P], gc[P], nv[P];
#pragma unroll
    for (int p = 0; p < P; p++) { carry[p] = 0.0f; gc[p] = 0.0f; nv[p] = lvpp[(size_t)e * P + p]; }
    for (int t = T - 1; t >= 0; t--) {
        const size_t i = (size_t)t * N + e;
        const int a = pl[i];
        const float dn = d[i], vv = v[i];
        float rw[P];
#pragma unroll
        for (int p = 0; p < P; p++) rw[p] = ar[i * P + p];
        if (dn > 0.5f) {
#pragma unroll
            for (int p = 0; p < P; p++) carry[p] = 0.0f;
        }
        float ca = 0.0f, ra = 0.0f;
#pragma unroll
        for (int p = 0; p < P; p++) if (p == a) { ca = carry[p]; ra = rw[p]; }
        const float attributed = __fadd_rn(ra, ca);
#pragma unroll
        for (int p = 0; p < P; p++) carry[p] = p == a ? 0.0f : __fadd_rn(carry[p], rw[p]);
        if (dn > 0.5f) {
#pragma unroll
            for (int p = 0; p < P; p++) { gc[p] = 0.0f; if (p != a) nv[p] = 0.0f; }
        }
        float nva = 0.0f, gca = 0.0f;
#pragma unroll
        for (int p = 0; p < P; p++) if (p == a) { nva = nv[p]; gca = gc[p]; }
        const float om = 1.0f - dn;
        const float delta = __fsub_rn(__builtin_fmaf(gamma * nva, om, attributed), vv);
        const float A = __builtin_fmaf(gl * om, gca, delta);
        adv[i] = A;
        ret[i] = __fadd_rn(A, vv);
#pragma unroll
        for (int p = 0; p < P; p++) if (p == a) { gc[p] = A; nv[p] = vv; }
    }
}

template <int P>
__global__ void __launch_bounds__(GSEG_WAVES * 64) k_gae_mp_seg(const float *__restrict__ ar,
                                                               const int32_t *__restrict__ pl,
                                                               const float *__restrict__ d,
                                                               const float *__restrict__ v,
                                                               const float *__restrict__ lvpp, int T, int N, int L,
                                                               float gamma, float lambda, float *__restrict__ adv,
                                                               float *__restrict__ ret) {
    __shared__ float st[3 * P][64];
    const int lane = threadIdx.x & 63, w = threadIdx.x >> 6;
    const int e = blockIdx.x * 64 + lane;
    const bool ok = e < N;
    const int t0 = w * L, n = max(0, min(T, t0 + L) - t0);
    const float gl = gamma * lambda;
    int a_[GSEG_L];
    float dn_[GSEG_L], v_[GSEG_L], rw_[GSEG_L][P];
    if (ok) {
#pragma unroll
        for (int u = 0; u < GSEG_L; u++)
            if (u < n) {
                const size_t i = (size_t)(t0 + u) * N + e;
                a_[u] = pl[i]; dn_[u] = d[i]; v_[u] = v[i];
#pragma unroll
                for (int p = 0; p < P; p++) rw_[u][p] = ar[i * P + p];
            }
    }
    float out_a[GSEG_L];
    for (int k = GSEG_WAVES - 1; k >= 0; k--) {
        if (w == k && ok) {
            float carry[P], gc[P], nv[P];
#pragma unroll
            for (int p = 0; p < P; p++) {
                if (k == GSEG_WAVES - 1) { carry[p] = 0.0f; gc[p] = 0.0f; nv[p] = lvpp[(size_t)e * P + p]; }
                else { carry[p] = st[p][lane]; gc[p] = st[P + p][lane]; nv[p] = st[2 * P + p][lane]; }
            }
#pragma unroll
            for (int u = GSEG_L - 1; u >= 0; u--) {
                if (u >= n) continue;
                const int a = a_[u];
                const float dn = dn_[u], vv = v_[u];
                if (dn > 0.5f) {
#pragma unroll
                    for (int p = 0; p < P; p++) carry[p] = 0.0f;
                }
                float ca = 0.0f, ra = 0.0f;
#pragma unroll
                for (int p = 0; p < P; p++) if (p == a) { ca = carry[p]; ra = rw_[u][p]; }
                const float attributed = __fadd_rn(ra, ca);
#pragma unroll
                for (int p = 0; p < P; p++) carry[p] = p == a ? 0.0f : __fadd_rn(carry[p], rw_[u][p]);
                if (dn > 0.5f) {
#pragma unroll
                    for (int p = 0; p < P; p++) { gc[p] = 0.0f; if (p != a) nv[p] = 0.0f; }
                }
                float nva = 0.0f, gca = 0.0f;
#pragma unroll
                for (int p = 0; p < P; p++) if (p == a) { nva = nv[p]; gca = gc[p]; }
                const float om = 1.0f - dn;
                const float delta = __fsub_rn(__builtin_fmaf(gamma * nva, om, attributed), vv);
                const float A = __builtin_fmaf(gl * om, gca, delta);
                out_a[u] = A;
#pragma unroll
                for (int p = 0; p < P; p++) if (p == a) { gc[p] = A; nv[p] = vv; }
            }
#pragma unroll
            for (int p = 0; p < P; p++) { st[p][lane] = carry[p]; st[P + p][lane] = gc[p]; st[2 * P + p][lane] = nv[p]; }
        }
        __syncthreads();
    }
    if (!ok) return;
#pragma unroll
    for (int u = 0; u < GSEG_L; u++) {
        if (u >= n) continue;
        const size_t i = (size_t)(t0 + u) * N + e;
        adv[i] = out_a[u];
        ret[i] = __fadd_rn(out_a[u], v_[u]);
    }
}

bppo_status launch_gae_1p(const float *r, const float *d, const float *v, const float *lv, int T,
                          int N, float gamma, float lambda, float *adv, float *ret, hipStream_t s,
                          float2 *pairs, bool *pairs_done, hipError_t *herr) {
    if (pairs_done) *pairs_done = false;
    if (T <= 0 || N <= 0) return BPPO_OK;
    const bool al = ((uintptr_t)r | (uintptr_t)d | (uintptr_t)v | (uintptr_t)lv | (uintptr_t)adv | (uintptr_t)ret |
                     (uintptr_t)pairs) % 16 == 0;
    if (N % 4 == 0 && T <= GSEG_WAVES * GSEG_L && al) {
        const int N4 = N / 4, L = (T + GSEG_WAVES - 1) / GSEG_WAVES;
        hipLaunchKernelGGL(k_gae_1p_seg, dim3((N4 + 63) / 64), dim3(GSEG_WAVES * 64), 0, s, (const float4 *)r,
                           (const float4 *)d, (const float4 *)v, (const float4 *)lv, T, N4, L, gamma, lambda,
                           (float4 *)adv, (float4 *)ret, pairs);
        if (pairs_done) *pairs_done = pairs != nullptr;
    } else {
        hipLaunchKernelGGL(k_gae_1p, dim3((N + 255) / 256), dim3(256), 0, s, r, d, v, lv, T, N, gamma,
                           lambda, adv, ret);
    }
    const hipError_t e = hipGetLastError();
    if (herr) *herr = e;
    return e == hipSuccess ? BPPO_OK : BPPO_ERR_HIP;
}

bppo_status launch_gae_mp(const float *ar, const int32_t *pl, const float *d, const float *v,
                          const float *lvpp, int T, int N, int P, float gamma, float lambda,
                          float *adv, float *ret, hipStream_t s, hipError_t *herr) {
    if (T <= 0 || N <= 0) return BPPO_OK;
    if (T <= GSEG_WAVES * GSEG_L && P >= 1 && P <= 6) {
        const int L = (T + GSEG_WAVES - 1) / GSEG_WAVES;
        const dim3 gs((N + 63) / 64), bs(GSEG_WAVES * 64);
#define MPSEG(P_) hipLaunchKernelGGL(k_gae_mp_seg<P_>, gs, bs, 0, s, ar, pl, d, v, lvpp, T, N, L, gamma, lambda, adv, ret)
        switch (P) {
        case 1: MPSEG(1); break;
        case 2: MPSEG(2); break;
        case 3: MPSEG(3); break;
        case 4: MPSEG(4); break;
        case 5: MPSEG(5); break;
        default: MPSEG(6); break;
        }
#undef MPSEG
        const hipError_t e = hipGetLastError();
        if (herr) *herr = e;
        return e == hipSuccess ? BPPO_OK : BPPO_ERR_HIP;
    }
    dim3 g((N + 255) / 256), b(256);
    switch (P) {
    case 1: hipLaunchKernelGGL(k_gae_mp<1>, g, b, 0, s, ar, pl, d, v, lvpp, T, N, gamma, lambda, adv, ret); break;
    case 2: hipLaunchKernelGGL(k_gae_mp<2>, g, b, 0, s, ar, pl, d, v, lvpp, T, N, gamma, lambda, adv, ret); break;
    case 3: hipLaunchKernelGGL(k_gae_mp<3>, g, b, 0, s, ar, pl, d, v, lvpp, T, N, gamma, lambda, adv, ret); break;
    case 4: hipLaunchKernelGGL(k_gae_mp<4>, g, b, 0, s, ar, pl, d, v, lvpp, T, N, gamma, lambda, adv, ret); break;
    case 5: hipLaunchKernelGGL(k_gae_mp<5>, g, b, 0, s, ar, pl, d, v, lvpp, T, N, gamma, lambda, adv, ret); break;
    case 6: hipLaunchKernelGGL(k_gae_mp<6>, g, b, 0, s, ar, pl, d, v, lvpp, T, N, gamma, lambda, adv, ret); break;
    default: return BPPO_ERR_ARG;
    }
    const hipError_t e = hipGetLastError();
    if (herr) *herr = e;
    return e == hipSuccess ? BPPO_OK : BPPO_ERR_HIP;
}

__device__ __forceinline__ Welford wmerge(Welford a, Welford b) {
    if (b.n == 0.0) return a;
    if (a.n == 0.0) return b;
    const double n = a.n + b.n, dl = b.mean - a.mean;
    Welford r;
    r.n = n;
    r.mean = a.mean + dl * (b.n / n);
    r.m2 = a.m2 + b.m2 + dl * dl * (a.n * b.n / n);
    return r;
}
__device__ __forceinline__ void wpush(Welford &s, double x) {
    s.n += 1.0;
    const double delta = x - s.mean;
    s.mean += delta / s.n;
    s.m2 += delta * (x - s.mean);
}

constexpr int RN_IPT = 16, RN_BLOCK = 256, RN_SEG = RN_IPT * RN_BLOCK;

constexpr int RN_TU = 16;
__global__ void k_rn_returns(int T, int N, double gamma, const float *__restrict__ rew_raw,
                             const float *__restrict__ done, double *__restrict__ returns_state,
                             double *__restrict__ X) {
    const int e = blockIdx.x * blockDim.x + threadIdx.x;
    if (e >= N) return;
    double x = returns_state[e];
    int t0 = 0;
    for (; t0 + RN_TU <= T; t0 += RN_TU) {
        float r[RN_TU], d[RN_TU];
#pragma unroll
        for (int k = 0; k < RN_TU; k++) {
            const size_t i = (size_t)(t0 + k) * N + e;
            r[k] = rew_raw[i];
            d[k] = done[i];
        }
#pragma unroll
        for (int k = 0; k < RN_TU; k++) {
            x = x * gamma + (double)r[k];
            X[(size_t)(t0 + k) * N + e] = x;
            if (d[k] != 0.0f) x = 0.0;
        }
    }
    for (; t0 < T; t0++) {
        const size_t i = (size_t)t0 * N + e;
        x = x * gamma + (double)rew_raw[i];
        X[i] = x;
        if (done[i] != 0.0f) x = 0.0;
    }
    returns_state[e] = x;
}

__global__ void k_rn_returns_mp(int T, int N, int P, double gamma, const float *rew_raw, const float *done,
                                const int32_t *players, const float *valid, double *returns_state, double *X) {
    const int e = blockIdx.x * blockDim.x + threadIdx.x;
    if (e >= N) return;
    double R0 = returns_state[(size_t)e * P], R1 = P > 1 ? returns_state[(size_t)e * P + 1] : 0.0;
    double R2 = P > 2 ? returns_state[(size_t)e * P + 2] : 0.0, R3 = P > 3 ? returns_state[(size_t)e * P + 3] : 0.0;
    auto step = [&](size_t i, int p, float r, float d, bool ok) {
        double x = p == 0 ? R0 : p == 1 ? R1 : p == 2 ? R2 : R3;
        x = x * gamma + (double)r;
        X[i] = ok ? x : __longlong_as_double(0x7ff8000000000000ll);
        if (d != 0.0f) x = 0.0;
        R0 = p == 0 ? x : R0; R1 = p == 1 ? x : R1; R2 = p == 2 ? x : R2; R3 = p == 3 ? x : R3;
    };
    const bool has_valid = valid != nullptr;
    const float *vsrc = has_valid ? valid : done;
    int t0 = 0;
    for (; t0 + RN_TU <= T; t0 += RN_TU) {
        int pl[RN_TU];
        float r[RN_TU], d[RN_TU], vv[RN_TU];
#pragma unroll
        for (int k = 0; k < RN_TU; k++) {
            const size_t i = (size_t)(t0 + k) * N + e;
            pl[k] = players[i]; r[k] = rew_raw[i]; d[k] = done[i]; vv[k] = vsrc[i];
        }
        bool ok[RN_TU];
#pragma unroll
        for (int k = 0; k < RN_TU; k++) ok[k] = !has_valid || vv[k] > 0.5f;
#pragma unroll
        for (int k = 0; k < RN_TU; k++) step((size_t)(t0 + k) * N + e, pl[k], r[k], d[k], ok[k]);
    }
    for (; t0 < T; t0++) {
        const size_t i = (size_t)t0 * N + e;
        step(i, players[i], rew_raw[i], done[i], !valid || valid[i] > 0.5f);
    }
    returns_state[(size_t)e * P] = R0;
    if (P > 1) returns_state[(size_t)e * P + 1] = R1;
    if (P > 2) returns_state[(size_t)e * P + 2] = R2;
    if (P > 3) returns_state[(size_t)e * P + 3] = R3;
}

__global__ void k_rn_scatter_acting(size_t n, int P, const int32_t *players, const float *rew, float *all_r) {
    for (size_t i = blockIdx.x * (size_t)blockDim.x + threadIdx.x; i < n; i += (size_t)gridDim.x * blockDim.x)
        all_r[i * P + players[i]] = rew[i];
}

__device__ Welford block_exclusive_scan(Welford mine, Welford *sh) {
    sh[threadIdx.x] = mine;
    __syncthreads();
    for (int off = 1; off < (int)blockDim.x; off <<= 1) {
        Welford v = sh[threadIdx.x];
        Welford u = threadIdx.x >= (unsigned)off ? sh[threadIdx.x - off] : Welford{0, 0, 0};
        __syncthreads();
        sh[threadIdx.x] = threadIdx.x >= (unsigned)off ? wmerge(u, v) : v;
        __syncthreads();
    }
    Welford incl = sh[threadIdx.x];
    Welford excl = threadIdx.x > 0 ? sh[threadIdx.x - 1] : Welford{0, 0, 0};
    (void)incl;
    __syncthreads();
    return excl;
}

constexpr int RN_PAD = RN_IPT + 1;
template <typename V>
__device__ __forceinline__ void rn_stage(size_t n, const V *X, V *xs) {
    const size_t base = (size_t)blockIdx.x * RN_SEG;
    V v[RN_IPT];
#pragma unroll
    for (int j = 0; j < RN_IPT; j++) {
        const size_t i = base + threadIdx.x + (size_t)j * RN_BLOCK;
        v[j] = i < n ? X[i] : (V)0;
    }
#pragma unroll
    for (int j = 0; j < RN_IPT; j++) {
        const int k = threadIdx.x + j * RN_BLOCK;
        xs[(k / RN_IPT) * RN_PAD + (k % RN_IPT)] = v[j];
    }
    __syncthreads();
}

__global__ void __launch_bounds__(RN_BLOCK) k_rn_block_agg(size_t n, const double *X, Welford *agg) {
    __shared__ Welford sh[RN_BLOCK];
    __shared__ double xs[RN_BLOCK * RN_PAD];
    rn_stage(n, X, xs);
    const size_t base = (size_t)blockIdx.x * RN_SEG + (size_t)threadIdx.x * RN_IPT;
    Welford s{0, 0, 0};
    for (int k = 0; k < RN_IPT; k++)
        if (base + k < n && !isnan(xs[threadIdx.x * RN_PAD + k])) wpush(s, xs[threadIdx.x * RN_PAD + k]);
    Welford ex = block_exclusive_scan(s, sh);
    if (threadIdx.x == blockDim.x - 1) agg[blockIdx.x] = wmerge(ex, s);
}

__global__ void __launch_bounds__(1024) k_rn_agg_scan(int nb, Welford *agg, double *stats) {
    __shared__ Welford sh[1024];
    const int per = (nb + 1023) / 1024;
    const int lo = threadIdx.x * per;
    Welford s{0, 0, 0};
    for (int k = 0; k < per; k++)
        if (lo + k < nb) s = wmerge(s, agg[lo + k]);
    Welford ex = block_exclusive_scan(s, sh);
    Welford run = wmerge(Welford{stats[2], stats[0], stats[1]}, ex);
    for (int k = 0; k < per; k++)
        if (lo + k < nb) {
            Welford a = agg[lo + k];
            agg[lo + k] = run;
            run = wmerge(run, a);
        }
    if (threadIdx.x == blockDim.x - 1 || (lo < nb && lo + per >= nb)) {
        if (lo < nb && lo + per >= nb) { stats[0] = run.mean; stats[1] = run.m2; stats[2] = run.n; }
    }
}

__global__ void __launch_bounds__(RN_BLOCK) k_rn_apply(size_t n, const double *X,
                                                       const float *rew_raw, const Welford *agg,
                                                       float clip, float *rew) {
    __shared__ Welford sh[RN_BLOCK];
    __shared__ double xs[RN_BLOCK * RN_PAD];
    __shared__ float rs[RN_BLOCK * RN_PAD];
    rn_stage(n, rew_raw, rs);
    rn_stage(n, X, xs);
    const size_t base = (size_t)blockIdx.x * RN_SEG + (size_t)threadIdx.x * RN_IPT;
    Welford s{0, 0, 0};
    for (int k = 0; k < RN_IPT; k++)
        if (base + k < n && !isnan(xs[threadIdx.x * RN_PAD + k])) wpush(s, xs[threadIdx.x * RN_PAD + k]);
    Welford ex = block_exclusive_scan(s, sh);
    Welford run = wmerge(agg[blockIdx.x], ex);
    for (int k = 0; k < RN_IPT; k++) {
        const size_t i = base + k;
        if (i >= n) break;
        if (!isnan(xs[threadIdx.x * RN_PAD + k])) wpush(run, xs[threadIdx.x * RN_PAD + k]);
        float r = rs[threadIdx.x * RN_PAD + k];
        if (run.n >= 2.0) {
            const double sd = sqrt(run.m2 / run.n + 1e-8);
            float z = (float)((double)r / sd);
            z = z < -clip ? -clip : z;
            z = z > clip ? clip : z;
            r = z;
        }
        rs[threadIdx.x * RN_PAD + k] = r;
    }
    __syncthreads();
    const size_t b0 = (size_t)blockIdx.x * RN_SEG;
    for (int k = threadIdx.x; k < RN_SEG; k += RN_BLOCK)
        if (b0 + k < n) rew[b0 + k] = rs[(k / RN_IPT) * RN_PAD + (k % RN_IPT)];
}

bppo_status launch_return_norm(bppo_ctx *c) {
    const size_t n = (size_t)c->T * c->N;
    const int nb = (int)((n + RN_SEG - 1) / RN_SEG);
    if (c->wide)
        hipLaunchKernelGGL(k_rn_returns_mp, dim3((c->N + 255) / 256), dim3(256), 0, c->stream, c->T, c->N, c->P,
                           c->cfg.gamma, c->d_rew_raw, c->d_done, c->d_players, c->n_opp ? c->d_valid : nullptr,
                           c->d_rn_returns, c->d_X);
    else
        hipLaunchKernelGGL(k_rn_returns, dim3((c->N + 255) / 256), dim3(256), 0, c->stream, c->T, c->N,
                           c->cfg.gamma, c->d_rew_raw, c->d_done, c->d_rn_returns, c->d_X);
    hipLaunchKernelGGL(k_rn_block_agg, dim3(nb), dim3(RN_BLOCK), 0, c->stream, n, c->d_X,
                       c->d_scan_agg);
    hipLaunchKernelGGL(k_rn_agg_scan, dim3(1), dim3(1024), 0, c->stream, nb, c->d_scan_agg,
                       c->d_rn_stats);
    hipLaunchKernelGGL(k_rn_apply, dim3(nb), dim3(RN_BLOCK), 0, c->stream, n, c->d_X, c->d_rew_raw,
                       c->d_scan_agg, (float)c->cfg.return_clip, c->d_rew);
    if (c->wide)
        hipLaunchKernelGGL(k_rn_scatter_acting, dim3((unsigned)std::min<size_t>((n + 255) / 256, 4096)), dim3(256), 0,
                           c->stream, n, c->P, c->d_players, c->d_rew, c->d_allr);
    TRY(launch_check(c, __func__));
    return BPPO_OK;
}

}
```

### burn-ppo_amd/csrc/k_rollout.hip

```cpp
#include "bppo_internal.h"
#include "bppo_mlp64.h"

namespace bppo {

struct ObsNorm5 {
    double mean[5], sd[5];
    bool on;
    __device__ __forceinline__ void load(const double *__restrict__ st, int norm_on) {
        const double cnt = st[10];
        on = norm_on && cnt >= 2.0;
#pragma unroll
        for (int d = 0; d < 5; d++) {
            const double var = st[5 + d] / cnt;
            double s = sqrt(var);
            sd[d] = s < 1e-8 ? 1e-8 : s;
            mean[d] = st[d];
        }
    }
    __device__ __forceinline__ void apply(const float (&raw)[5], float (&out)[5]) const {
#pragma unroll
        for (int d = 0; d < 5; d++) {
            if (!on) { out[d] = raw[d]; continue; }
            float z = (float)(((double)raw[d] - mean[d]) / sd[d]);
            z = z < -10.0f ? -10.0f : z;
            z = z > 10.0f ? 10.0f : z;
            out[d] = z;
        }
    }
};

struct ObsAcc5 {
    double x0[5], s1[5], s2[5];
    __device__ __forceinline__ void init(const float (&raw)[5]) {
#pragma unroll
        for (int d = 0; d < 5; d++) { x0[d] = (double)raw[d]; s1[d] = s2[d] = 0.0; }
    }
    __device__ __forceinline__ void push(const float (&raw)[5]) {
#pragma unroll
        for (int d = 0; d < 5; d++) {
            const double dd = (double)raw[d] - x0[d];
            s1[d] += dd;
            s2[d] += dd * dd;
        }
    }
    __device__ __forceinline__ void store(double T, double *part) const {
#pragma unroll
        for (int d = 0; d < 5; d++) {
            part[d] = x0[d] + s1[d] / T;
            const double m2 = s2[d] - s1[d] * s1[d] / T;
            part[5 + d] = m2 > 0.0 ? m2 : 0.0;
        }
    }
};

__device__ __forceinline__ void load_state(const float *cp, const int32_t *steps, int N, int e,
                                           CartPoleState &s) {
    s.x = cp[e]; s.x_dot = cp[N + e]; s.theta = cp[2 * N + e]; s.theta_dot = cp[3 * N + e];
    s.steps = steps[e];
}
__device__ __forceinline__ void store_state(float *cp, int32_t *steps, int N, int e,
                                            const CartPoleState &s) {
    cp[e] = s.x; cp[N + e] = s.x_dot; cp[2 * N + e] = s.theta; cp[3 * N + e] = s.theta_dot;
    steps[e] = s.steps;
}

__global__ void k_cartpole_reset(int N, uint64_t seed_base, float *cp, int32_t *steps,
                                 uint64_t *env_pos, float *ep_ret, int32_t *ep_len, float *obs) {
    int e = blockIdx.x * blockDim.x + threadIdx.x;
    if (e >= N) return;
    WordCursor c;
    c.init(seed_key(seed_base + (uint64_t)e), 0, 0);
    CartPoleState s;
    cartpole_reset(s, c);
    cartpole_reset(s, c);
    store_state(cp, steps, N, e, s);
    env_pos[e] = c.pos;
    ep_ret[e] = 0.0f;
    ep_len[e] = 0;
    if (obs) {
        float o[5];
        cartpole_obs(s, o);
        for (int d = 0; d < 5; d++) obs[e * 5 + d] = o[d];
    }
}

struct RolloutArgs {
    int N, T;
    uint64_t seed_base;
    float *cp; int32_t *steps; uint64_t *env_pos; float *ep_ret; int32_t *ep_len;
    Key8 key; uint64_t stream; uint64_t base_pos;
    const float *params; int n_params;
    const double *on; int norm_on;
    float *obs, *rew_raw, *done, *val, *logp; int32_t *act;
    double *obs_part;
    EpisodeRec *eps; int32_t *ep_count; int eps_cap;
    int32_t *err;
    float4 *rows;
    unsigned long long *stamps;
    const float4 *rpool; const uint64_t *rpos; int rpool_k;
};

#ifdef BPPO_RO_STAMPS
constexpr int RO_NSEG = 8;
#define RO_STAMP(k)                                                                              \
    do {                                                                                         \
        __builtin_amdgcn_sched_barrier(0);                                                       \
        unsigned long long t_;                                                                   \
        asm volatile("s_memtime %0\n\ts_waitcnt lgkmcnt(0)" : "=s"(t_)::"memory");               \
        __builtin_amdgcn_sched_barrier(0);                                                       \
        ro_acc[k] += t_ - ro_prev;                                                               \
        ro_prev = t_;                                                                            \
    } while (0)
#else
#define RO_STAMP(k) \
    do {            \
    } while (0)
#endif

template <int H, int NL, int ACT>
__global__ void __launch_bounds__(256) k_cartpole_rollout(RolloutArgs a) {
    extern __shared__ __attribute__((aligned(16))) float sP[];
    constexpr CpOffsets O = cp_offsets<H, NL>();
    for (int i = threadIdx.x; i < O.n; i += blockDim.x) sP[i] = a.params[i];
    __syncthreads();
    const int e = blockIdx.x * blockDim.x + threadIdx.x;
    if (e >= a.N) return;
    const int N = a.N;
    CartPoleState s;
    load_state(a.cp, a.steps, N, e, s);
    WordCursor ec;
    ec.init(seed_key(a.seed_base + (uint64_t)e), 0, a.env_pos[e]);
    float ep_ret = a.ep_ret[e];
    int32_t ep_len = a.ep_len[e];
    ObsNorm5 nz;
    nz.load(a.on, a.norm_on);
    ObsAcc5 oa;
    {
        float raw0[5];
        cartpole_obs(s, raw0);
        oa.init(raw0);
    }
    int32_t bad = 0;
#pragma unroll 1
    for (int t = 0; t < a.T; t++) {
        float raw[5], x[5];
        cartpole_obs(s, raw);
        oa.push(raw);
        nz.apply(raw, x);
        const size_t row = (size_t)t * N + e;
#pragma unroll
        for (int d = 0; d < 5; d++) a.obs[row * 5 + d] = x[d];
        float lg[2], v;
        int zero = 0;
        asm volatile("" : "+v"(zero));
        cp_forward<H, NL, ACT>(sP + zero, x, lg, v, sP + cp_stage_ofs<H, NL>() + threadIdx.x, blockDim.x);
        const uint64_t p0 = a.base_pos + row * 2;
        uint32_t blk[16];
        chacha12_block(a.key, p0 >> 4, a.stream, blk);
        const uint32_t l0 = (uint32_t)(p0 & 15);
        uint32_t w0 = blk[0], w1 = blk[1];
#pragma unroll
        for (int i = 1; i < 16; i++) w0 = l0 == (uint32_t)i ? blk[i] : w0;
#pragma unroll
        for (int i = 0; i < 15; i++) w1 = l0 == (uint32_t)i ? blk[i + 1] : w1;
        if (l0 == 15) {
            uint32_t b2[16];
            chacha12_block(a.key, (p0 >> 4) + 1, a.stream, b2);
            w1 = b2[0];
        }
        const float n0 = __fadd_rn(lg[0], gumbel_from_word(w0));
        const float n1 = __fadd_rn(lg[1], gumbel_from_word(w1));
        const int act = n1 > n0 ? 1 : 0;
        const float lp = log_prob_row<2>(lg, act);
        bad |= !isfinite(lp);
        float r;
        const bool done = cartpole_step(s, act, r);
        ep_ret = __fadd_rn(ep_ret, r);
        ep_len += 1;
        const int32_t k = wave_episode_slot(done, a.ep_count);
        if (done) {
            if (k < a.eps_cap) {
                EpisodeRec rec;
                rec.total_reward[0] = ep_ret;
                for (int p = 1; p < BPPO_MAX_PLAYERS; p++) rec.total_reward[p] = 0.0f;
                rec.length = ep_len; rec.env_index = e; rec.step = t; rec.pad = 0;
                a.eps[k] = rec;
            }
            cartpole_reset(s, ec);
            ep_ret = 0.0f;
            ep_len = 0;
        }
        a.act[row] = act;
        a.rew_raw[row] = r;
        a.done[row] = done ? 1.0f : 0.0f;
        a.val[row] = v;
        a.logp[row] = lp;
    }
    store_state(a.cp, a.steps, N, e, s);
    a.env_pos[e] = ec.pos;
    a.ep_ret[e] = ep_ret;
    a.ep_len[e] = ep_len;
    oa.store((double)a.T, a.obs_part + (size_t)e * 10);
    if (bad) atomicOr(a.err, 1);
}

constexpr int GUM_THREADS = 256;
__global__ void __launch_bounds__(GUM_THREADS) k_gumbel_words(Key8 key, uint64_t stream, uint64_t base,
                                                              uint64_t count, float *__restrict__ g,
                                                              int32_t *zero0, int32_t *zero1) {
    __shared__ float tile[16 * GUM_THREADS + GUM_THREADS / 2];
    if (blockIdx.x == 0 && threadIdx.x == 0) { *zero0 = 0; *zero1 = 0; }
    const uint64_t blk0 = (base >> 4) + blockIdx.x * (uint64_t)GUM_THREADS;
    const uint64_t b = blk0 + threadIdx.x, wb = blk0 * 16;
    if (b * 16 < base + count) {
        uint32_t blk[16];
        chacha12_block(key, b, stream, blk);
#pragma unroll
        for (int j = 0; j < 16; j++) {
            const int k = threadIdx.x * 16 + j;
            tile[k + (k >> 5)] = gumbel_from_word(blk[j]);
        }
    }
    __syncthreads();
#pragma unroll
    for (int j = 0; j < 16; j++) {
        const int k = j * GUM_THREADS + threadIdx.x;
        const uint64_t w = wb + k;
        if (w >= base && w < base + count) g[w - base] = tile[k + (k >> 5)];
    }
}

__global__ void __launch_bounds__(256) k_reset_pool(int N, int K, uint64_t seed_base, const uint64_t *__restrict__ env_pos,
                                                    float4 *__restrict__ pool, uint64_t *__restrict__ ppos) {
    const int e = blockIdx.x * blockDim.x + threadIdx.x;
    if (e >= N) return;
    WordCursor c;
    c.init(seed_key(seed_base + (uint64_t)e), 0, env_pos[e]);
    for (int j = 0; j < K; j++) {
        CartPoleState s;
        cartpole_reset(s, c);
        pool[(size_t)j * N + e] = make_float4(s.x, s.x_dot, s.theta, s.theta_dot);
        ppos[(size_t)j * N + e] = c.pos;
    }
}

__global__ void __launch_bounds__(512, 2) k_cartpole_rollout_mfma(RolloutArgs a, const float *__restrict__ gum) {
    using namespace mmb;
    extern __shared__ __attribute__((aligned(16))) float smem[];
    Params &S = *reinterpret_cast<Params *>(smem);
    const int tid = threadIdx.x, lane = tid & 63, wv = tid >> 6;
    Wave &B = reinterpret_cast<Wave *>(smem + sizeof(Params) / 4)[wv];
    load_params(S, a.params);
    __syncthreads();
    const int c = lane & 31, h = lane >> 5;
    const int N = a.N;
    const int e = (blockIdx.x * WAVES + wv) * TR + c;
    const bool mine = h == 0 && e < N;
    float b0k[2], b1k[2];
#pragma unroll
    for (int ct = 0; ct < 2; ct++) { b0k[ct] = S.b0[c + 32 * ct]; b1k[ct] = S.b1[c + 32 * ct]; }
    CartPoleState s{};
    WordCursor ec;
    float ep_ret = 0.0f;
    int32_t ep_len = 0;
    if (mine) {
        load_state(a.cp, a.steps, N, e, s);
        ec.init(seed_key(a.seed_base + (uint64_t)e), 0, a.env_pos[e]);
        ep_ret = a.ep_ret[e];
        ep_len = a.ep_len[e];
    }
    ObsNorm5 nz;
    nz.load(a.on, a.norm_on);
    ObsAcc5 oa;
    if (mine) {
        float raw0[5];
        cartpole_obs(s, raw0);
        oa.init(raw0);
    }
    int32_t bad = 0;
#pragma unroll 1
    for (int t = 0; t < a.T; t++) {
        const size_t row = (size_t)t * N + e;
        const float2 gz = mine ? *reinterpret_cast<const float2 *>(gum + row * 2) : make_float2(0.0f, 0.0f);
        float4 xa = make_float4(0.f, 0.f, 0.f, 0.f);
        float x4 = 0.0f;
        if (h == 0) {
            float x[5] = {0, 0, 0, 0, 0};
            if (mine) {
                float raw[5];
                cartpole_obs(s, raw);
                oa.push(raw);
                nz.apply(raw, x);
#pragma unroll
                for (int d = 0; d < 5; d++) a.obs[row * 5 + d] = x[d];
                xa = make_float4(x[0], x[1], x[2], x[3]);
                x4 = x[4];
            }
#pragma unroll
            for (int d = 0; d < 5; d++) B.X[c * 9 + d] = x[d];
            B.X[c * 9 + 5] = 0.0f;
        }
        wave_sync();
        f32x16_t h1[2];
#pragma unroll
        for (int ct = 0; ct < 2; ct++)
#pragma unroll
            for (int q = 0; q < 16; q++) h1[ct][q] = 0.0f;
#pragma unroll
        for (int st = 0; st < 3; st++) {
            const float av = B.X[c * 9 + 2 * st + h];
#pragma unroll
            for (int ct = 0; ct < 2; ct++)
                h1[ct] = __builtin_amdgcn_mfma_f32_32x32x2f32(av, S.W0[(2 * st + h) * H + c + 32 * ct], h1[ct], 0, 0, 0);
        }
#pragma unroll
        for (int ct = 0; ct < 2; ct++)
#pragma unroll
            for (int q = 0; q < 16; q++) {
                const float v = __fadd_rn(h1[ct][q], b0k[ct]);
                B.T[cd_row(q, h) * RS + c + 32 * ct] = v > 0.0f ? v : 0.0f;
            }
        wave_sync();
        f32x16_t h2[2];
#pragma unroll
        for (int ct = 0; ct < 2; ct++)
#pragma unroll
            for (int q = 0; q < 16; q++) h2[ct][q] = 0.0f;
#pragma unroll 8
        for (int st = 0; st < 32; st++) {
            const float av = B.T[c * RS + 2 * st + h];
            h2[0] = __builtin_amdgcn_mfma_f32_32x32x2f32(av, S.W1[(2 * st + h) * RS + c], h2[0], 0, 0, 0);
            h2[1] = __builtin_amdgcn_mfma_f32_32x32x2f32(av, S.W1[(2 * st + h) * RS + c + 32], h2[1], 0, 0, 0);
        }
        wave_sync();
#pragma unroll
        for (int ct = 0; ct < 2; ct++)
#pragma unroll
            for (int q = 0; q < 16; q++) {
                const float v = __fadd_rn(h2[ct][q], b1k[ct]);
                B.T[cd_row(q, h) * RS + c + 32 * ct] = v > 0.0f ? v : 0.0f;
            }
        wave_sync();
        float lh = 0.0f, vv = 0.0f;
        if (e < N) {
            const float *hr = B.T + c * RS;
            const float2 *pv = S.PV[h];
#pragma unroll 16
            for (int k = 0; k < H; k++) {
                const float hk = hr[k];
                const float2 w = pv[k];
                lh = __builtin_fmaf(hk, w.x, lh);
                vv = __builtin_fmaf(hk, w.y, vv);
            }
        }
        const float lx = __shfl_xor(lh, 32, 64);
        if (mine) {
            const float l0 = lh, l1 = lx;
            float lg[2];
            lg[0] = __fadd_rn(l0, S.bp[0]);
            lg[1] = __fadd_rn(l1, S.bp[1]);
            const float v = __fadd_rn(vv, S.bv[0]);
            const float n0 = __fadd_rn(lg[0], gz.x);
            const float n1 = __fadd_rn(lg[1], gz.y);
            const int act = n1 > n0 ? 1 : 0;
            const float lp = log_prob_row<2>(lg, act);
            bad |= !isfinite(lp);
            float r;
            const bool done = cartpole_step(s, act, r);
            ep_ret = __fadd_rn(ep_ret, r);
            ep_len += 1;
            const int32_t k = wave_episode_slot(done, a.ep_count);
            if (done) {
                if (k < a.eps_cap) {
                    EpisodeRec rec;
                    rec.total_reward[0] = ep_ret;
                    for (int p = 1; p < BPPO_MAX_PLAYERS; p++) rec.total_reward[p] = 0.0f;
                    rec.length = ep_len; rec.env_index = e; rec.step = t; rec.pad = 0;
                    a.eps[k] = rec;
                }
                cartpole_reset(s, ec);
                ep_ret = 0.0f;
                ep_len = 0;
            }
            a.act[row] = act;
            a.rew_raw[row] = r;
            a.done[row] = done ? 1.0f : 0.0f;
            a.val[row] = v;
            a.logp[row] = lp;
            if (a.rows) { a.rows[row * 2] = xa; a.rows[row * 2 + 1] = make_float4(x4, __int_as_float(act), lp, v); }
        }
        wave_sync();
    }
    if (mine) {
        store_state(a.cp, a.steps, N, e, s);
        a.env_pos[e] = ec.pos;
        a.ep_ret[e] = ep_ret;
// ... 180 lines not shown
                h2[tl][0] = __builtin_amdgcn_mfma_f32_32x32x2f32(w.x, h1[tl][st >> 4][st & 15], h2[tl][0], 0, 0, 0);
                h2[tl][1] = __builtin_amdgcn_mfma_f32_32x32x2f32(w.y, h1[tl][st >> 4][st & 15], h2[tl][1], 0, 0, 0);
            }
        }
        RO_STAMP(2);
#pragma unroll
        for (int tl = 0; tl < 2; tl++)
#pragma unroll
            for (int m = 0; m < 32; m++) Tw[(32 * tl + c) * 65 + 32 * h + m] = h2[tl][m >> 4][m & 15];
        wave_sync();
        RO_STAMP(3);
        int zero = 0;
        asm volatile("" : "+v"(zero));
        const float4 *hw = S.hw + zero;
        const float *hrow = Tw + lane * 65 + zero;
        float l0 = 0.0f, l1 = 0.0f, vv = 0.0f;
#pragma unroll 1
        for (int k0 = 0; k0 < H; k0 += 8) {
            float4 w[8];
            float hz[8];
#pragma unroll
            for (int j = 0; j < 8; j++) { w[j] = hw[k0 + j]; hz[j] = hrow[k0 + j]; }
#pragma unroll
            for (int j = 0; j < 8; j++) {
                float z = __fadd_rn(hz[j], w[j].w);
                z = z > 0.0f ? z : 0.0f;
                l0 = __builtin_fmaf(z, w[j].x, l0);
                l1 = __builtin_fmaf(z, w[j].y, l1);
                vv = __builtin_fmaf(z, w[j].z, vv);
            }
        }
        float lg[2];
        lg[0] = __fadd_rn(l0, S.bp[0]);
        lg[1] = __fadd_rn(l1, S.bp[1]);
        const float v = __fadd_rn(vv, S.bv[0]);
        const float n0 = __fadd_rn(lg[0], gz.x);
        const float n1 = __fadd_rn(lg[1], gz.y);
        const int act = n1 > n0 ? 1 : 0;
        RO_STAMP(4);
        const float lp = log_prob2(S, lg, act);
        bool done = false;
        float r = 0.0f;
        RO_STAMP(5);
        if (mine) {
            bad |= !isfinite(lp);
            done = cartpole_step(s, act, r);
            ep_ret = __fadd_rn(ep_ret, r);
            ep_len += 1;
        }
        flush_eps(t - 1);
        const uint64_t m = (uint64_t)__ballot(done ? 1 : 0);
        if (m) {
            const int leader = __ffsll((unsigned long long)m) - 1;
            if (lane == leader) pbase = atomicAdd(a.ep_count, (int32_t)__popcll(m));
        }
        pm = m;
        if (done) {
            pret = ep_ret;
            plen = ep_len;
            if (rj < a.rpool_k) {
                s.x = rnx.x; s.x_dot = rnx.y; s.theta = rnx.z; s.theta_dot = rnx.w; s.steps = 0;
                env_pos = rnpos;
                rj++;
            } else {
                WordCursor ec;
                ec.init(seed_key(a.seed_base + (uint64_t)e), 0, env_pos);
                cartpole_reset(s, ec);
                env_pos = ec.pos;
            }
            ep_ret = 0.0f;
            ep_len = 0;
        }
        RO_STAMP(6);
        if (mine) {
#pragma unroll
            for (int d = 0; d < 5; d++) a.obs[row * 5 + d] = x[d];
            a.act[row] = act;
            a.rew_raw[row] = r;
            a.done[row] = done ? 1.0f : 0.0f;
            a.val[row] = v;
            a.logp[row] = lp;
            if (a.rows) {
                a.rows[row * 2] = make_float4(x[0], x[1], x[2], x[3]);
                a.rows[row * 2 + 1] = make_float4(x[4], __int_as_float(act), lp, v);
            }
        }
        wave_sync();
        RO_STAMP(7);
    }
    flush_eps(a.T - 1);
#ifdef BPPO_RO_STAMPS
    if (lane == 0 && a.stamps)
        for (int k = 0; k < RO_NSEG; k++) a.stamps[(size_t)(e >> 6) * RO_NSEG + k] = ro_acc[k];
#endif
    if (mine) {
        store_state(a.cp, a.steps, N, e, s);
        a.env_pos[e] = env_pos;
        a.ep_ret[e] = ep_ret;
        a.ep_len[e] = ep_len;
        oa.store((double)a.T, a.obs_part + (size_t)e * 10);
        if (bad) atomicOr(a.err, 1);
    }
}

__global__ void k_cartpole_step(int N, uint64_t seed_base, float *cp, int32_t *steps,
                                uint64_t *env_pos, float *ep_ret, int32_t *ep_len,
                                const int32_t *actions, float *rew, uint8_t *dn, float *obs,
                                EpisodeRec *eps, int32_t *ep_count, int cap) {
    int e = blockIdx.x * blockDim.x + threadIdx.x;
    if (e >= N) return;
    CartPoleState s;
    load_state(cp, steps, N, e, s);
    float r;
    bool done = cartpole_step(s, actions[e], r);
    float er = __fadd_rn(ep_ret[e], r);
    int32_t el = ep_len[e] + 1;
    const int32_t k = wave_episode_slot(done, ep_count);
    if (done) {
        if (k < cap) {
            EpisodeRec rec;
            rec.total_reward[0] = er;
            for (int p = 1; p < BPPO_MAX_PLAYERS; p++) rec.total_reward[p] = 0.0f;
            rec.length = el; rec.env_index = e; rec.step = 0; rec.pad = 0;
            eps[k] = rec;
        }
        WordCursor c;
        c.init(seed_key(seed_base + (uint64_t)e), 0, env_pos[e]);
        cartpole_reset(s, c);
        env_pos[e] = c.pos;
        er = 0.0f; el = 0;
    }
    store_state(cp, steps, N, e, s);
    ep_ret[e] = er; ep_len[e] = el;
    rew[e] = r;
    dn[e] = done ? 1 : 0;
    if (obs) {
        float o[5];
        cartpole_obs(s, o);
        for (int d = 0; d < 5; d++) obs[e * 5 + d] = o[d];
    }
}

__global__ void k_cartpole_observe(int N, const float *cp, const int32_t *steps, float *obs) {
    int e = blockIdx.x * blockDim.x + threadIdx.x;
    if (e >= N) return;
    CartPoleState s;
    load_state(cp, steps, N, e, s);
    float o[5];
    cartpole_obs(s, o);
    for (int d = 0; d < 5; d++) obs[e * 5 + d] = o[d];
}

template <int H, int NL, int ACT>
__global__ void __launch_bounds__(256) k_cartpole_bootstrap(int N, const float *cp,
                                                            const int32_t *steps,
                                                            const float *params, const double *on,
                                                            int norm_on, float *last_v) {
    extern __shared__ __attribute__((aligned(16))) float sP[];
    constexpr CpOffsets O = cp_offsets<H, NL>();
    for (int i = threadIdx.x; i < O.n; i += blockDim.x) sP[i] = params[i];
    __syncthreads();
    int e = blockIdx.x * blockDim.x + threadIdx.x;
    if (e >= N) return;
    CartPoleState s;
    load_state(cp, steps, N, e, s);
    float raw[5], x[5], lg[2], v;
    cartpole_obs(s, raw);
    ObsNorm5 nz;
    nz.load(on, norm_on);
    nz.apply(raw, x);
    cp_forward<H, NL, ACT>(sP, x, lg, v, sP + cp_stage_ofs<H, NL>() + threadIdx.x, blockDim.x);
    last_v[e] = v;
}

template <int H, int NL, int ACT>
__global__ void __launch_bounds__(256) k_cartpole_forward_rows(int B, const float *obs,
                                                               const float *params, float *logits,
                                                               float *values) {
    extern __shared__ __attribute__((aligned(16))) float sP[];
    constexpr CpOffsets O = cp_offsets<H, NL>();
    for (int i = threadIdx.x; i < O.n; i += blockDim.x) sP[i] = params[i];
    __syncthreads();
    int r = blockIdx.x * blockDim.x + threadIdx.x;
    if (r >= B) return;
    float x[5], lg[2], v;
    for (int d = 0; d < 5; d++) x[d] = obs[(size_t)r * 5 + d];
    cp_forward<H, NL, ACT>(sP, x, lg, v, sP + cp_stage_ofs<H, NL>() + threadIdx.x, blockDim.x);
    logits[(size_t)r * 2] = lg[0];
    logits[(size_t)r * 2 + 1] = lg[1];
    values[r] = v;
}

constexpr int OBS_PART_BLOCKS = 64, OBS_MAX_D = 8;
__global__ void __launch_bounds__(256) k_obs_norm_part(int N, int D, double T, const double *part, double *bp) {
    __shared__ double sn[256], sm[256][OBS_MAX_D], sq[256][OBS_MAX_D];
    const int per = (N + gridDim.x - 1) / gridDim.x;
    const int e0 = blockIdx.x * per, e1 = min(N, e0 + per);
    double n = 0.0, mean[OBS_MAX_D], m2[OBS_MAX_D];
    for (int d = 0; d < OBS_MAX_D; d++) mean[d] = m2[d] = 0.0;
    for (int e = e0 + threadIdx.x; e < e1; e += blockDim.x) {
        const double *pe = part + (size_t)e * 2 * D;
        const double nn = n + T, f = T / nn, g = n * T / nn;
        for (int d = 0; d < D; d++) {
            const double delta = pe[d] - mean[d];
            mean[d] += delta * f;
            m2[d] += pe[D + d] + delta * delta * g;
        }
        n = nn;
    }
    sn[threadIdx.x] = n;
    for (int d = 0; d < D; d++) { sm[threadIdx.x][d] = mean[d]; sq[threadIdx.x][d] = m2[d]; }
    __syncthreads();
    for (int st = blockDim.x / 2; st > 0; st >>= 1) {
        if (threadIdx.x < st) {
            const double na = sn[threadIdx.x], nb = sn[threadIdx.x + st], nn = na + nb;
            if (nb > 0) {
                const double f = na > 0 ? nb / nn : 1.0, g = na * nb / nn;
                for (int d = 0; d < D; d++) {
                    const double delta = sm[threadIdx.x + st][d] - sm[threadIdx.x][d];
                    sm[threadIdx.x][d] += delta * f;
                    sq[threadIdx.x][d] += sq[threadIdx.x + st][d] + delta * delta * g;
                }
                sn[threadIdx.x] = nn;
            }
        }
        __syncthreads();
    }
    if (threadIdx.x < D) {
        double *o = bp + ((size_t)blockIdx.x * OBS_MAX_D + threadIdx.x) * 3;
        o[0] = sn[0]; o[1] = sm[0][threadIdx.x]; o[2] = sq[0][threadIdx.x];
    }
}
__global__ void k_obs_norm_final(int D, int nblk, const double *bp, double *on) {
    const int d = threadIdx.x;
    if (d >= D) return;
    double n = 0.0, mean = 0.0, m2 = 0.0;
    constexpr int U = 16;
    for (int b0 = 0; b0 < nblk; b0 += U) {
        double pn[U], pm[U], p2[U];
#pragma unroll
        for (int k = 0; k < U; k++) {
            const double *o = bp + ((size_t)min(b0 + k, nblk - 1) * OBS_MAX_D + d) * 3;
            pn[k] = o[0]; pm[k] = o[1]; p2[k] = o[2];
        }
#pragma unroll
        for (int k = 0; k < U; k++) {
            if (b0 + k >= nblk) break;
            const double nb = pn[k];
            if (nb <= 0) continue;
            const double nn = n + nb, delta = pm[k] - mean;
            mean = n > 0 ? mean + delta * (nb / nn) : pm[k];
            m2 += p2[k] + (n > 0 ? delta * delta * (n * nb / nn) : 0.0);
            n = nn;
        }
    }
    const double na = on[2 * D], nn = na + n, delta = mean - on[d];
    const double ma = on[d];
    on[d] = na > 0 ? ma + delta * (n / nn) : mean;
    on[D + d] = on[D + d] + m2 + (na > 0 ? delta * delta * (na * n / nn) : 0.0);
    __syncthreads();
    if (d == 0) on[2 * D] = nn;
}

#define CP_DISPATCH(H_, NL_, CALL)                                                 \
    if (h == H_ && nl == NL_) {                                                    \
        if (c->cfg.relu) CALL(H_, NL_, ACT_RELU); else CALL(H_, NL_, ACT_TANH);   \
        return launch_check(c, __func__);                                          \
    }

static bool cp_supported(int h, int nl) {
    return (h == 16 || h == 32 || h == 64) && (nl == 1 || nl == 2);
}

bppo_status launch_cartpole_reset(bppo_ctx *c) {
    int N = c->N;
    hipLaunchKernelGGL(k_cartpole_reset, dim3((N + 255) / 256), dim3(256), 0, c->stream, N,
                       c->cfg.env_seed_base, c->d_cp, c->d_steps, c->d_env_pos, c->d_ep_ret,
                       c->d_ep_len, nullptr);
    TRY(launch_check(c, __func__));
    return BPPO_OK;
}

bppo_status launch_cartpole_rollout(bppo_ctx *c, uint64_t base_pos, const double *, const double *,
                                    int norm_on) {
    const int h = c->cfg.hidden_size, nl = c->cfg.num_hidden;
    const bool lanes64 = env_int("BPPO_ROLLOUT_LANES64", 1) != 0;
    const bool gum_path = h == 64 && nl == 2 && c->cfg.relu && c->d_gumbel;
    if (!gum_path) {
        BPPO_HIP(c, hipMemsetAsync(c->d_ep_count, 0, 4, c->stream));
        BPPO_HIP(c, hipMemsetAsync(c->d_err, 0, 4, c->stream));
    }
    if (!cp_supported(h, nl)) {
        c->err = "CartPole rollout kernel supports MLPs with hidden in {16,32,64} x {1,2} layers";
        return BPPO_ERR_UNSUPPORTED;
    }
    RolloutArgs a;
    a.N = c->N; a.T = c->T; a.seed_base = c->cfg.env_seed_base;
    a.cp = c->d_cp; a.steps = c->d_steps; a.env_pos = c->d_env_pos; a.ep_ret = c->d_ep_ret;
    a.ep_len = c->d_ep_len; a.key = c->rng_key; a.stream = c->cfg.rng_stream; a.base_pos = base_pos;
    a.params = c->d_params; a.n_params = (int)c->net.n_params; a.on = c->d_on; a.norm_on = norm_on;
    a.obs = c->d_obs; a.rew_raw = c->d_rew_raw; a.done = c->d_done; a.val = c->d_val;
    a.logp = c->d_logp; a.act = c->d_act; a.obs_part = c->d_obs_part; a.eps = c->d_eps;
    a.ep_count = c->d_ep_count; a.eps_cap = c->eps_cap; a.err = c->d_err;
    a.rows = nullptr;
    a.stamps = nullptr;
    a.rpool = nullptr; a.rpos = nullptr; a.rpool_k = 0;
    c->rows_from_rollout = false;
    if (gum_path) {
        if (c->d_rowA && !c->cfg.normalize_values && !env_set("BPPO_NO_FUSED_PACK")) {
            a.rows = c->d_rowA;
            c->rows_from_rollout = true;
        }
        const uint64_t count = (uint64_t)c->T * c->N * 2;
        const uint64_t blocks = ((base_pos + count + 15) >> 4) - (base_pos >> 4);
        hipLaunchKernelGGL(k_gumbel_words, dim3((unsigned)((blocks + 255) / 256)), dim3(256), 0, c->stream,
                           c->rng_key, (uint64_t)c->cfg.rng_stream, base_pos, count, c->d_gumbel, c->d_ep_count,
                           (int32_t *)c->d_err);
        TRY(launch_check(c, "k_gumbel_words"));
        if (!lanes64) {
            const int waves = (c->N + mmb::TR - 1) / mmb::TR;
            hipLaunchKernelGGL(k_cartpole_rollout_mfma, dim3((waves + mmb::WAVES - 1) / mmb::WAVES), dim3(64 * mmb::WAVES),
                               mmb::LDS, c->stream, a, (const float *)c->d_gumbel);
        } else {
            const int waves = (c->N + 63) / 64;
            const int pk = std::max(0, std::min(RPOOL_K, env_int("BPPO_RESET_POOL_K", RPOOL_K)));
            if (c->d_rpool && pk > 0) {
                hipLaunchKernelGGL(k_reset_pool, dim3((c->N + 255) / 256), dim3(256), 0, c->stream, c->N, pk,
                                   c->cfg.env_seed_base, (const uint64_t *)c->d_env_pos, c->d_rpool, c->d_rpos);
                TRY(launch_check(c, "k_reset_pool"));
                a.rpool = c->d_rpool; a.rpos = c->d_rpos; a.rpool_k = pk;
            }
#ifdef BPPO_RO_STAMPS
            static unsigned long long *d_st = nullptr;
            if (!d_st) BPPO_HIP(c, hipMalloc((void **)&d_st, sizeof(unsigned long long) * (size_t)waves * RO_NSEG));
            a.stamps = d_st;
#endif
            hipLaunchKernelGGL(k_cartpole_rollout_mfma64, dim3((waves + mmr::WAVES - 1) / mmr::WAVES),
                               dim3(64 * mmr::WAVES), 0, c->stream, a, (const float *)c->d_gumbel);
#ifdef BPPO_RO_STAMPS
            {
                static double acc_s[RO_NSEG] = {};
                static int nl = 0;
                std::vector<unsigned long long> hs((size_t)waves * RO_NSEG);
                BPPO_HIP(c, hipMemcpyAsync(hs.data(), d_st, hs.size() * 8, hipMemcpyDeviceToHost, c->stream));
                BPPO_HIP(c, hipStreamSynchronize(c->stream));
                for (int w = 0; w < waves; w++)
                    for (int k = 0; k < RO_NSEG; k++) acc_s[k] += (double)hs[(size_t)w * RO_NSEG + k] / waves;
                if (++nl % 4 == 0) {
                    double tot = 0;
                    for (int k = 0; k < RO_NSEG; k++) tot += acc_s[k];
                    fprintf(stderr, "[rostamp] launches=%d cycles/wave/step=%.0f shares:", nl, tot / nl / c->T);
                    for (int k = 0; k < RO_NSEG; k++) fprintf(stderr, " s%d=%.3f", k, acc_s[k] / tot);
                    fprintf(stderr, "\n");
                }
            }
#endif
        }
        TRY(launch_check(c, __func__));
        return BPPO_OK;
    }
    dim3 grid((c->N + 255) / 256), blk(256);
#define L(H_, NL_, A_) hipLaunchKernelGGL((k_cartpole_rollout<H_, NL_, A_>), grid, blk, (cp_lds<H_, NL_>(A_, 256)), c->stream, a)
    CP_DISPATCH(16, 1, L) CP_DISPATCH(16, 2, L) CP_DISPATCH(32, 1, L) CP_DISPATCH(32, 2, L)
    CP_DISPATCH(64, 1, L) CP_DISPATCH(64, 2, L)
#undef L
    return BPPO_ERR_UNSUPPORTED;
}

bppo_status launch_bootstrap(bppo_ctx *c, const double *, const double *, int norm_on) {
    const int h = c->cfg.hidden_size, nl = c->cfg.num_hidden;
    dim3 grid((c->N + 255) / 256), blk(256);
#define L(H_, NL_, A_)                                                                          \
    hipLaunchKernelGGL((k_cartpole_bootstrap<H_, NL_, A_>), grid, blk, (cp_lds<H_, NL_>(A_, 256)), c->stream, c->N, c->d_cp, \
                       c->d_steps, c->d_params, c->d_on, norm_on, c->d_last_v)
    CP_DISPATCH(16, 1, L) CP_DISPATCH(16, 2, L) CP_DISPATCH(32, 1, L) CP_DISPATCH(32, 2, L)
    CP_DISPATCH(64, 1, L) CP_DISPATCH(64, 2, L)
#undef L
    return BPPO_ERR_UNSUPPORTED;
}

bppo_status launch_forward_rows(bppo_ctx *c, const float *d_obs, int B, float *d_logits,
                                float *d_values) {
    const int h = c->cfg.hidden_size, nl = c->cfg.num_hidden;
    dim3 grid((B + 255) / 256), blk(256);
#define L(H_, NL_, A_)                                                                            \
    hipLaunchKernelGGL((k_cartpole_forward_rows<H_, NL_, A_>), grid, blk, (cp_lds<H_, NL_>(A_, 256)), c->stream, B, d_obs, \
                       c->d_params, d_logits, d_values)
    CP_DISPATCH(16, 1, L) CP_DISPATCH(16, 2, L) CP_DISPATCH(32, 1, L) CP_DISPATCH(32, 2, L)
    CP_DISPATCH(64, 1, L) CP_DISPATCH(64, 2, L)
#undef L
    return BPPO_ERR_UNSUPPORTED;
}

bppo_status launch_cartpole_vecenv_step(bppo_ctx *c, const int32_t *d_actions, float *d_rew,
                                        uint8_t *d_done, float *d_obs_out) {
    int N = c->N;
    hipLaunchKernelGGL(k_cartpole_step, dim3((N + 255) / 256), dim3(256), 0, c->stream, N,
                       c->cfg.env_seed_base, c->d_cp, c->d_steps, c->d_env_pos, c->d_ep_ret,
                       c->d_ep_len, d_actions, d_rew, d_done, d_obs_out, c->d_eps, c->d_ep_count,
                       c->eps_cap);
    TRY(launch_check(c, __func__));
    return BPPO_OK;
}

bppo_status launch_cartpole_observe(bppo_ctx *c, float *d_obs_out) {
    int N = c->N;
    hipLaunchKernelGGL(k_cartpole_observe, dim3((N + 255) / 256), dim3(256), 0, c->stream, N,
                       c->d_cp, c->d_steps, d_obs_out);
    TRY(launch_check(c, __func__));
    return BPPO_OK;
}

__global__ void __launch_bounds__(256) k_obs_norm_rows(int rows, int D, int ld, float *x, float *raw,
                                                       const double *on, float clip) {
    const double cnt = on[2 * D];
    const size_t n = (size_t)rows * D;
    for (size_t i = blockIdx.x * (size_t)blockDim.x + threadIdx.x; i < n; i += (size_t)gridDim.x * blockDim.x) {
        const size_t r = i / D;
        const int d = (int)(i - r * D);
        float *p = x + r * ld + d;
        const float v = *p;
        if (raw) raw[i] = v;
        if (cnt >= 2.0) {
            double sd = sqrt(on[D + d] / cnt);
            sd = sd < 1e-8 ? 1e-8 : sd;
            float z = (float)(((double)v - on[d]) / sd);
            z = z < -clip ? -clip : z;
            z = z > clip ? clip : z;
            *p = z;
        }
    }
}
bppo_status launch_obs_norm_rows(bppo_ctx *c, int rows, float *x, int ld, float *raw) {
    return launch_obs_norm_rows_on(c, rows, x, ld, raw, c->d_on);
}
bppo_status launch_obs_norm_rows_on(bppo_ctx *c, int rows, float *x, int ld, float *raw, const double *on) {
    const size_t n = (size_t)rows * c->D;
    hipLaunchKernelGGL(k_obs_norm_rows, dim3((unsigned)std::min<size_t>((n + 255) / 256, 8192)), dim3(256), 0,
                       c->stream, rows, c->D, ld, x, raw, on, 10.0f);
    TRY(launch_check(c, __func__));
    return BPPO_OK;
}

constexpr int OBSW_CHUNKS = 256;
__global__ void __launch_bounds__(256) k_obsw_part(size_t rows, int D, const float *raw, double *part) {
    const int d = blockIdx.x * blockDim.x + threadIdx.x;
    if (d >= D) return;
    const size_t per = (rows + gridDim.y - 1) / gridDim.y;
    const size_t r0 = blockIdx.y * per, r1 = r0 + per < rows ? r0 + per : rows;
    double n = 0.0, s1 = 0.0, s2 = 0.0, k = 0.0;
    if (r0 < r1) k = raw[r0 * D + d];
    for (size_t r = r0; r < r1; r++) {
        const double y = (double)raw[r * D + d] - k;
        s1 += y;
        s2 += y * y;
        n += 1.0;
    }
    double *o = part + ((size_t)blockIdx.y * D + d) * 3;
    o[0] = n;
    o[1] = n > 0 ? k + s1 / n : 0.0;
    o[2] = n > 0 ? s2 - s1 * (s1 / n) : 0.0;
}
__global__ void k_obsw_final(int D, int nchunk, const double *part, double *on) {
    const int d = blockIdx.x * blockDim.x + threadIdx.x;
    if (d >= D) return;
    double n = 0.0, mean = 0.0, m2 = 0.0;
    for (int b = 0; b < nchunk; b++) {
        const double *o = part + ((size_t)b * D + d) * 3;
        const double nb = o[0];
        if (nb <= 0) continue;
        const double nn = n + nb, delta = o[1] - mean;
        mean = n > 0 ? mean + delta * (nb / nn) : o[1];
        m2 += o[2] + (n > 0 ? delta * delta * (n * nb / nn) : 0.0);
        n = nn;
    }
    const double na = on[2 * D], nn = na + n, delta = mean - on[d];
    const double ma = on[d];
    on[d] = na > 0 ? ma + delta * (n / nn) : mean;
    on[D + d] = on[D + d] + m2 + (na > 0 ? delta * delta * (na * n / nn) : 0.0);
}
__global__ void k_obsw_count(int D, double add, double *on) { on[2 * D] += add; }

bppo_status launch_obs_norm_merge(bppo_ctx *c) {
    if (c->wide) {
        const size_t rows = (size_t)c->T * c->N;
        if ((size_t)OBSW_CHUNKS * c->D * 3 > c->obsw_part_n) { c->err = "obs normalizer scratch too small"; return BPPO_ERR_ARG; }
        hipLaunchKernelGGL(k_obsw_part, dim3((c->D + 255) / 256, OBSW_CHUNKS), dim3(256), 0, c->stream, rows, c->D,
                           c->d_obs_raw, c->d_obsw_part);
        hipLaunchKernelGGL(k_obsw_final, dim3((c->D + 255) / 256), dim3(256), 0, c->stream, c->D, OBSW_CHUNKS,
                           c->d_obsw_part, c->d_on);
        hipLaunchKernelGGL(k_obsw_count, dim3(1), dim3(1), 0, c->stream, c->D, (double)rows, c->d_on);
        TRY(launch_check(c, __func__));
        return BPPO_OK;
    }
    if (c->D > OBS_MAX_D) { c->err = "observation normalizer: obs dim > 8"; return BPPO_ERR_UNSUPPORTED; }
    const int nblk = std::min(OBS_PART_BLOCKS, std::max(1, (c->N + 255) / 256));
    hipLaunchKernelGGL(k_obs_norm_part, dim3(nblk), dim3(256), 0, c->stream, c->N, c->D, (double)c->T,
                       c->d_obs_part, c->d_red);
    hipLaunchKernelGGL(k_obs_norm_final, dim3(1), dim3(64), 0, c->stream, c->D, nblk, c->d_red, c->d_on);
    TRY(launch_check(c, __func__));
    return BPPO_OK;
}

__global__ void __launch_bounds__(256) k_ep_summary(const EpisodeRec *eps, const int32_t *count, const int32_t *err,
                                                    int cap, double *host_slot) {
    const int cnt = *count;
    const int n = min(cnt, cap);
    double *part = host_slot + 2;
    if (blockIdx.x == 0 && threadIdx.x == 0) {
        int32_t *hv = reinterpret_cast<int32_t *>(host_slot);
        hv[0] = cnt;
        hv[1] = *err;
    }
    double sr = 0.0, sl = 0.0;
    for (int i = blockIdx.x * blockDim.x + threadIdx.x; i < n; i += gridDim.x * blockDim.x) {
        sr += (double)eps[i].total_reward[0];
        sl += (double)eps[i].length;
    }
    __shared__ double sh[2][4];
    for (int o = 32; o > 0; o >>= 1) { sr += __shfl_down(sr, o, 64); sl += __shfl_down(sl, o, 64); }
    const int w = threadIdx.x >> 6;
    if ((threadIdx.x & 63) == 0) { sh[0][w] = sr; sh[1][w] = sl; }
    __syncthreads();
    if (threadIdx.x == 0) {
        part[2 * blockIdx.x] = sh[0][0] + sh[0][1] + sh[0][2] + sh[0][3];
        part[2 * blockIdx.x + 1] = sh[1][0] + sh[1][1] + sh[1][2] + sh[1][3];
    }
}

bppo_status launch_episode_summary(bppo_ctx *c, double *host_slot) {
    hipLaunchKernelGGL(k_ep_summary, dim3(EP_SUMMARY_BLOCKS), dim3(256), 0, c->stream, c->d_eps, c->d_ep_count,
                       (const int32_t *)c->d_err, c->eps_cap, host_slot);
    TRY(launch_check(c, __func__));
    return BPPO_OK;
}

}
```

Measured before the change: 776.2 million.

## Fuse post-rollout normalizer, summary and bootstrap kernels into role-dispatched launches

Combines the post-rollout stages for the cartpole path into three role-dispatched kernels. The head kernel runs the return recurrence, observation-normalizer partials and episode summary. The mid kernel runs the block aggregation and the obs-normalizer final step. The tail kernel runs return-norm apply together with the value bootstrap. Fusing the bootstrap into the rollout tail lets GAE skip its separate bootstrap launch when boot_done is set. The aim is to cut the number of small kernel launches and serialization points per iteration, at the cost of extra state tracking (boot_done invalidation) and shared-memory sizing taken as the max of the roles.

```diff
diff --git a/burn-ppo_amd/csrc/bppo_api.hip b/burn-ppo_amd/csrc/bppo_api.hip
--- a/burn-ppo_amd/csrc/bppo_api.hip
+++ b/burn-ppo_amd/csrc/bppo_api.hip
@@ -386,6 +386,7 @@
 extern "C" size_t bppo_num_params(const bppo_ctx *c) { return c ? c->net.n_params : 0; }
 
 static void drop_prefetch(bppo_ctx *c) {
+    c->boot_done = false;
     if (!c->prefetched) return;
     c->prefetched = false;
     c->collected = 0;
@@ -538,6 +539,7 @@
 extern "C" bppo_status bppo_vecenv_step(bppo_ctx *c, const int32_t *actions, float *obs, float *rewards,
                                         uint8_t *dones, bppo_episode *eps, int32_t cap, int32_t *n_eps) {
     if (!c || !actions) return BPPO_ERR_ARG;
+    c->boot_done = false;
     const int N = c->N;
     if (c->wide) {
         BPPO_HIP(c, hipMemsetAsync(c->d_ep_count, 0, 4, c->stream));
@@ -689,7 +691,7 @@
 
 static double *roll_host(bppo_ctx *c, int slot) { return c->h_red + 4 * 1024 + 64 + (size_t)slot * ROLL_HOST_WORDS; }
 
-static bppo_status collect_enqueue(bppo_ctx *c, bool summary) {
+static bppo_status collect_enqueue(bppo_ctx *c, bool summary, bool boot) {
     const size_t TN = (size_t)c->T * c->N;
     c->coll_slot ^= 1;
     const int tro = c->coll_slot ? TM_ROLLOUT_B : TM_ROLLOUT, trn = c->coll_slot ? TM_RETNORM_B : TM_RETNORM;
@@ -715,14 +717,22 @@
         c->rng_pos = base + TN * (uint64_t)c->A;
         c->shuf_slot = c->shuf.ensure(c->rng_pos);
     }
-    if (c->cfg.normalize_obs) TRY(launch_obs_norm_merge(c));
-    TRY(tm_begin(c, trn));
-    if (c->cfg.normalize_returns) TRY(launch_return_norm(c));
-    else if (!c->wide) BPPO_HIP(c, hipMemcpyAsync(c->d_rew, c->d_rew_raw, TN * 4, hipMemcpyDeviceToDevice, c->stream));
-    TRY(tm_end(c, trn));
+    if (c->wide) {
+        if (c->cfg.normalize_obs) TRY(launch_obs_norm_merge(c));
+        TRY(tm_begin(c, trn));
+        if (c->cfg.normalize_returns) TRY(launch_return_norm(c));
+        TRY(tm_end(c, trn));
+        if (summary) TRY(launch_episode_summary(c, c->d_ep_sum));
+    } else {
+        TRY(tm_begin(c, trn));
+        TRY(launch_post_rollout(c, summary ? c->d_ep_sum : nullptr, boot));
+        if (!c->cfg.normalize_returns)
+            BPPO_HIP(c, hipMemcpyAsync(c->d_rew, c->d_rew_raw, TN * 4, hipMemcpyDeviceToDevice, c->stream));
+        TRY(tm_end(c, trn));
+    }
+    c->boot_done = boot && !c->wide;
     int32_t *hv = reinterpret_cast<int32_t *>(roll_host(c, c->coll_slot));
     if (summary) {
-        TRY(launch_episode_summary(c, c->d_ep_sum));
         BPPO_HIP(c, hipMemcpyAsync(hv, c->d_ep_sum, sizeof(double) * ROLL_HOST_WORDS, hipMemcpyDeviceToHost, c->stream));
     } else {
         BPPO_HIP(c, hipMemcpyAsync(&hv[0], c->d_ep_count, 4, hipMemcpyDeviceToHost, c->stream));
@@ -762,7 +772,7 @@
 extern "C" bppo_status bppo_collect_rollouts(bppo_ctx *c, bppo_rollout_info *info) {
     if (!c) return BPPO_ERR_ARG;
     if (c->prefetched) c->prefetched = false;
-    else TRY(collect_enqueue(c, info != nullptr));
+    else TRY(collect_enqueue(c, info != nullptr, false));
     BPPO_HIP(c, sync_stream(c));
     return collect_finish(c, info, c->coll_slot);
 }
@@ -799,7 +809,8 @@
         return BPPO_OK;
     }
     TRY(tm_begin(c, TM_BOOT));
-    TRY(launch_bootstrap(c, nullptr, nullptr, c->cfg.normalize_obs));
+    if (!c->boot_done) TRY(launch_bootstrap(c));
+    c->boot_done = false;
     TRY(popart_denorm(c, c->d_last_v, (size_t)c->N));
     TRY(tm_end(c, TM_BOOT));
     TRY(tm_begin(c, TM_GAE));
@@ -1072,7 +1083,7 @@
     if (c->prefetch_next) {
         c->prefetch_next = false;
         c->env_step = c->prefetch_env_step;
-        TRY(collect_enqueue(c, true));
+        TRY(collect_enqueue(c, true, true));
         c->prefetched = true;
         BPPO_HIP(c, wait_event(c, c->ev_upd));
     } else {
@@ -1162,7 +1173,7 @@
     const auto t0 = std::chrono::steady_clock::now();
     c->sync_wait_ms = 0.0;
     if (c->prefetched) c->prefetched = false;
-    else TRY(collect_enqueue(c, info != nullptr));
+    else TRY(collect_enqueue(c, info != nullptr, true));
     TRY(gae_enqueue(c));
     const bppo_status us = bppo_ppo_update(c, lr, ent_coef, m);
     if (us == BPPO_OK) { if (!c->wide) tm_read(c, TM_BOOT); tm_read(c, TM_GAE); }
@@ -1182,7 +1193,7 @@
     for (int32_t k = 0; k < n; k++) {
         const auto t0 = std::chrono::steady_clock::now();
         c->sync_wait_ms = 0.0;
-        if (!c->prefetched) { c->env_step = global_step0 + (uint64_t)k * TN; TRY(collect_enqueue(c, true)); }
+        if (!c->prefetched) { c->env_step = global_step0 + (uint64_t)k * TN; TRY(collect_enqueue(c, true, true)); }
         c->prefetched = false;
         const int slot = c->coll_slot;
         TRY(gae_enqueue(c));
@@ -1296,6 +1307,7 @@
     BPPO_HIP(c, hipMemcpyAsync(b.ptr, host, b.bytes, hipMemcpyHostToDevice, c->stream));
     BPPO_HIP(c, sync_stream(c));
     if (!strcmp(name, "advantages") || !strcmp(name, "returns")) c->gae_done = c->collected = 1;
+    c->boot_done = false;
     c->rows_packed = c->rows_from_rollout = false;
     return BPPO_OK;
 }
diff --git a/burn-ppo_amd/csrc/bppo_internal.h b/burn-ppo_amd/csrc/bppo_internal.h
--- a/burn-ppo_amd/csrc/bppo_internal.h
+++ b/burn-ppo_amd/csrc/bppo_internal.h
@@ -349,6 +349,7 @@
     int coll_slot = 1;
     uint64_t rollout_rng_pos[2] = {0, 0};
     bool prefetch_next = false, prefetched = false;
+    bool boot_done = false;
     bool rows_from_rollout = false, rows_packed = false;
     uint64_t prefetch_env_step = 0;
     int ev_mode = 0;
@@ -377,9 +378,10 @@
 bppo_status launch_cartpole_observe(bppo_ctx *c, float *d_obs_out);
 bppo_status launch_obs_norm_merge(bppo_ctx *c);
 bppo_status launch_episode_summary(bppo_ctx *c, double *host_slot);
+bppo_status launch_post_rollout(bppo_ctx *c, double *host_slot, bool boot);
 bppo_status launch_obs_norm_rows(bppo_ctx *c, int rows, float *x, int ld, float *raw);
 bppo_status launch_obs_norm_rows_on(bppo_ctx *c, int rows, float *x, int ld, float *raw, const double *on);
-bppo_status launch_bootstrap(bppo_ctx *c, const double *mean, const double *sd, int norm_on);
+bppo_status launch_bootstrap(bppo_ctx *c);
 bppo_status launch_forward_rows(bppo_ctx *c, const float *d_obs, int B, float *d_logits,
                                 float *d_values);
 bppo_status launch_gae_1p(const float *r, const float *d, const float *v, const float *lv, int T,
@@ -389,6 +391,7 @@
                           const float *lvpp, int T, int N, int P, float gamma, float lambda,
                           float *adv, float *ret, hipStream_t s, hipError_t *herr = nullptr);
 bppo_status launch_return_norm(bppo_ctx *c);
+void launch_rn_agg_scan(bppo_ctx *c, int nb);
 bppo_status launch_fisher_yates(bppo_ctx *c, const uint32_t *d_J, uint32_t n);
 hipError_t fisher_yates_device(const uint32_t *d_J, uint32_t n, uint32_t *scratch, uint32_t *scan, uint32_t *perm,
                                hipStream_t st, const FyRanges *rg, uint32_t *inv = nullptr);
diff --git a/burn-ppo_amd/csrc/bppo_retnorm.h b/burn-ppo_amd/csrc/bppo_retnorm.h
--- /dev/null
+++ b/burn-ppo_amd/csrc/bppo_retnorm.h
@@ -0,0 +1,141 @@
+#pragma once
+#include "bppo_internal.h"
+
+namespace bppo {
+
+__device__ __forceinline__ Welford wmerge(Welford a, Welford b) {
+    if (b.n == 0.0) return a;
+    if (a.n == 0.0) return b;
+    const double n = a.n + b.n, dl = b.mean - a.mean;
+    Welford r;
+    r.n = n;
+    r.mean = a.mean + dl * (b.n / n);
+    r.m2 = a.m2 + b.m2 + dl * dl * (a.n * b.n / n);
+    return r;
+}
+__device__ __forceinline__ void wpush(Welford &s, double x) {
+    s.n += 1.0;
+    const double delta = x - s.mean;
+    s.mean += delta / s.n;
+    s.m2 += delta * (x - s.mean);
+}
+
+constexpr int RN_IPT = 16, RN_BLOCK = 256, RN_SEG = RN_IPT * RN_BLOCK;
+
+constexpr int RN_TU = 16;
+__device__ __forceinline__ void rn_returns_role(int bid, int T, int N, double gamma,
+                                                const float *__restrict__ rew_raw,
+                                                const float *__restrict__ done,
+                                                double *__restrict__ returns_state, double *__restrict__ X) {
+    const int e = bid * blockDim.x + threadIdx.x;
+    if (e >= N) return;
+    double x = returns_state[e];
+    int t0 = 0;
+    for (; t0 + RN_TU <= T; t0 += RN_TU) {
+        float r[RN_TU], d[RN_TU];
+#pragma unroll
+        for (int k = 0; k < RN_TU; k++) {
+            const size_t i = (size_t)(t0 + k) * N + e;
+            r[k] = rew_raw[i];
+            d[k] = done[i];
+        }
+#pragma unroll
+        for (int k = 0; k < RN_TU; k++) {
+            x = x * gamma + (double)r[k];
+            X[(size_t)(t0 + k) * N + e] = x;
+            if (d[k] != 0.0f) x = 0.0;
+        }
+    }
+    for (; t0 < T; t0++) {
+        const size_t i = (size_t)t0 * N + e;
+        x = x * gamma + (double)rew_raw[i];
+        X[i] = x;
+        if (done[i] != 0.0f) x = 0.0;
+    }
+    returns_state[e] = x;
+}
+
+__device__ __forceinline__ Welford block_exclusive_scan(Welford mine, Welford *sh) {
+    sh[threadIdx.x] = mine;
+    __syncthreads();
+    for (int off = 1; off < (int)blockDim.x; off <<= 1) {
+        Welford v = sh[threadIdx.x];
+        Welford u = threadIdx.x >= (unsigned)off ? sh[threadIdx.x - off] : Welford{0, 0, 0};
+        __syncthreads();
+        sh[threadIdx.x] = threadIdx.x >= (unsigned)off ? wmerge(u, v) : v;
+        __syncthreads();
+    }
+    Welford excl = threadIdx.x > 0 ? sh[threadIdx.x - 1] : Welford{0, 0, 0};
+    __syncthreads();
+    return excl;
+}
+
+constexpr int RN_PAD = RN_IPT + 1;
+template <typename V>
+__device__ __forceinline__ void rn_stage(int bid, size_t n, const V *X, V *xs) {
+    const size_t base = (size_t)bid * RN_SEG;
+    V v[RN_IPT];
+#pragma unroll
+    for (int j = 0; j < RN_IPT; j++) {
+        const size_t i = base + threadIdx.x + (size_t)j * RN_BLOCK;
+        v[j] = i < n ? X[i] : (V)0;
+    }
+#pragma unroll
+    for (int j = 0; j < RN_IPT; j++) {
+        const int k = threadIdx.x + j * RN_BLOCK;
+        xs[(k / RN_IPT) * RN_PAD + (k % RN_IPT)] = v[j];
+    }
+    __syncthreads();
+}
+
+struct RnAggLds {
+    Welford sh[RN_BLOCK];
+    double xs[RN_BLOCK * RN_PAD];
+};
+struct RnApplyLds {
+    Welford sh[RN_BLOCK];
+    double xs[RN_BLOCK * RN_PAD];
+    float rs[RN_BLOCK * RN_PAD];
+};
+
+__device__ __forceinline__ void rn_block_agg_role(int bid, size_t n, const double *X, Welford *agg, RnAggLds &l) {
+    rn_stage(bid, n, X, l.xs);
+    const size_t base = (size_t)bid * RN_SEG + (size_t)threadIdx.x * RN_IPT;
+    Welford s{0, 0, 0};
+    for (int k = 0; k < RN_IPT; k++)
+        if (base + k < n && !isnan(l.xs[threadIdx.x * RN_PAD + k])) wpush(s, l.xs[threadIdx.x * RN_PAD + k]);
+    Welford ex = block_exclusive_scan(s, l.sh);
+    if (threadIdx.x == blockDim.x - 1) agg[bid] = wmerge(ex, s);
+}
+
+__device__ __forceinline__ void rn_apply_role(int bid, size_t n, const double *X, const float *rew_raw,
+                                              const Welford *agg, float clip, float *rew, RnApplyLds &l) {
+    rn_stage(bid, n, rew_raw, l.rs);
+    rn_stage(bid, n, X, l.xs);
+    const size_t base = (size_t)bid * RN_SEG + (size_t)threadIdx.x * RN_IPT;
+    Welford s{0, 0, 0};
+    for (int k = 0; k < RN_IPT; k++)
+        if (base + k < n && !isnan(l.xs[threadIdx.x * RN_PAD + k])) wpush(s, l.xs[threadIdx.x * RN_PAD + k]);
+    Welford ex = block_exclusive_scan(s, l.sh);
+    Welford run = wmerge(agg[bid], ex);
+    for (int k = 0; k < RN_IPT; k++) {
+        const size_t i = base + k;
+        if (i >= n) break;
+        if (!isnan(l.xs[threadIdx.x * RN_PAD + k])) wpush(run, l.xs[threadIdx.x * RN_PAD + k]);
+        float r = l.rs[threadIdx.x * RN_PAD + k];
+        if (run.n >= 2.0) {
+            const double sd = sqrt(run.m2 / run.n + 1e-8);
+            float z = (float)((double)r / sd);
+            z = z < -clip ? -clip : z;
+            z = z > clip ? clip : z;
+            r = z;
+        }
+        l.rs[threadIdx.x * RN_PAD + k] = r;
+    }
+    __syncthreads();
+    const size_t b0 = (size_t)bid * RN_SEG;
+    for (int k = threadIdx.x; k < RN_SEG; k += RN_BLOCK)
+        if (b0 + k < n) rew[b0 + k] = l.rs[(k / RN_IPT) * RN_PAD + (k % RN_IPT)];
+}
+
+}
diff --git a/burn-ppo_amd/csrc/k_gae.hip b/burn-ppo_amd/csrc/k_gae.hip
--- a/burn-ppo_amd/csrc/k_gae.hip
+++ b/burn-ppo_amd/csrc/k_gae.hip
@@ -1,4 +1,5 @@
 #include "bppo_internal.h"
+#include "bppo_retnorm.h"
 #include <algorithm>
 
 namespace bppo {
@@ -300,56 +301,6 @@
     return e == hipSuccess ? BPPO_OK : BPPO_ERR_HIP;
 }
 
-__device__ __forceinline__ Welford wmerge(Welford a, Welford b) {
-    if (b.n == 0.0) return a;
-    if (a.n == 0.0) return b;
-    const double n = a.n + b.n, dl = b.mean - a.mean;
-    Welford r;
-    r.n = n;
-    r.mean = a.mean + dl * (b.n / n);
-    r.m2 = a.m2 + b.m2 + dl * dl * (a.n * b.n / n);
-    return r;
-}
-__device__ __forceinline__ void wpush(Welford &s, double x) {
-    s.n += 1.0;
-    const double delta = x - s.mean;
-    s.mean += delta / s.n;
-    s.m2 += delta * (x - s.mean);
-}
-
-constexpr int RN_IPT = 16, RN_BLOCK = 256, RN_SEG = RN_IPT * RN_BLOCK;
-
-constexpr int RN_TU = 16;
-__global__ void k_rn_returns(int T, int N, double gamma, const float *__restrict__ rew_raw,
-                             const float *__restrict__ done, double *__restrict__ returns_state,
-                             double *__restrict__ X) {
-    const int e = blockIdx.x * blockDim.x + threadIdx.x;
-    if (e >= N) return;
-    double x = returns_state[e];
-    int t0 = 0;
-    for (; t0 + RN_TU <= T; t0 += RN_TU) {
-        float r[RN_TU], d[RN_TU];
-#pragma unroll
-        for (int k = 0; k < RN_TU; k++) {
-            const size_t i = (size_t)(t0 + k) * N + e;
-            r[k] = rew_raw[i];
-            d[k] = done[i];
-        }
-#pragma unroll
-        for (int k = 0; k < RN_TU; k++) {
-            x = x * gamma + (double)r[k];
-            X[(size_t)(t0 + k) * N + e] = x;
-            if (d[k] != 0.0f) x = 0.0;
-        }
-    }
-    for (; t0 < T; t0++) {
-        const size_t i = (size_t)t0 * N + e;
-        x = x * gamma + (double)rew_raw[i];
-        X[i] = x;
-        if (done[i] != 0.0f) x = 0.0;
-    }
-    returns_state[e] = x;
-}
 
 __global__ void k_rn_returns_mp(int T, int N, int P, double gamma, const float *rew_raw, const float *done,
                                 const int32_t *players, const float *valid, double *returns_state, double *X) {
@@ -396,51 +347,9 @@
         all_r[i * P + players[i]] = rew[i];
 }
 
-__device__ Welford block_exclusive_scan(Welford mine, Welford *sh) {
-    sh[threadIdx.x] = mine;
-    __syncthreads();
-    for (int off = 1; off < (int)blockDim.x; off <<= 1) {
-        Welford v = sh[threadIdx.x];
-        Welford u = threadIdx.x >= (unsigned)off ? sh[threadIdx.x - off] : Welford{0, 0, 0};
-        __syncthreads();
-        sh[threadIdx.x] = threadIdx.x >= (unsigned)off ? wmerge(u, v) : v;
-        __syncthreads();
-    }
-    Welford incl = sh[threadIdx.x];
-    Welford excl = threadIdx.x > 0 ? sh[threadIdx.x - 1] : Welford{0, 0, 0};
-    (void)incl;
-    __syncthreads();
-    return excl;
-}
-
-constexpr int RN_PAD = RN_IPT + 1;
-template <typename V>
-__device__ __forceinline__ void rn_stage(size_t n, const V *X, V *xs) {
-    const size_t base = (size_t)blockIdx.x * RN_SEG;
-    V v[RN_IPT];
-#pragma unroll
-    for (int j = 0; j < RN_IPT; j++) {
-        const size_t i = base + threadIdx.x + (size_t)j * RN_BLOCK;
-        v[j] = i < n ? X[i] : (V)0;
-    }
-#pragma unroll
-    for (int j = 0; j < RN_IPT; j++) {
-        const int k = threadIdx.x + j * RN_BLOCK;
-        xs[(k / RN_IPT) * RN_PAD + (k % RN_IPT)] = v[j];
-    }
-    __syncthreads();
-}
-
 __global__ void __launch_bounds__(RN_BLOCK) k_rn_block_agg(size_t n, const double *X, Welford *agg) {
-    __shared__ Welford sh[RN_BLOCK];
-    __shared__ double xs[RN_BLOCK * RN_PAD];
-    rn_stage(n, X, xs);
-    const size_t base = (size_t)blockIdx.x * RN_SEG + (size_t)threadIdx.x * RN_IPT;
-    Welford s{0, 0, 0};
-    for (int k = 0; k < RN_IPT; k++)
-        if (base + k < n && !isnan(xs[threadIdx.x * RN_PAD + k])) wpush(s, xs[threadIdx.x * RN_PAD + k]);
-    Welford ex = block_exclusive_scan(s, sh);
-    if (threadIdx.x == blockDim.x - 1) agg[blockIdx.x] = wmerge(ex, s);
+    __shared__ RnAggLds l;
+    rn_block_agg_role(blockIdx.x, n, X, agg, l);
 }
 
 __global__ void __launch_bounds__(1024) k_rn_agg_scan(int nb, Welford *agg, double *stats) {
@@ -466,56 +375,28 @@
 __global__ void __launch_bounds__(RN_BLOCK) k_rn_apply(size_t n, const double *X,
                                                        const float *rew_raw, const Welford *agg,
                                                        float clip, float *rew) {
-    __shared__ Welford sh[RN_BLOCK];
-    __shared__ double xs[RN_BLOCK * RN_PAD];
-    __shared__ float rs[RN_BLOCK * RN_PAD];
-    rn_stage(n, rew_raw, rs);
-    rn_stage(n, X, xs);
-    const size_t base = (size_t)blockIdx.x * RN_SEG + (size_t)threadIdx.x * RN_IPT;
-    Welford s{0, 0, 0};
-    for (int k = 0; k < RN_IPT; k++)
-        if (base + k < n && !isnan(xs[threadIdx.x * RN_PAD + k])) wpush(s, xs[threadIdx.x * RN_PAD + k]);
-    Welford ex = block_exclusive_scan(s, sh);
-    Welford run = wmerge(agg[blockIdx.x], ex);
-    for (int k = 0; k < RN_IPT; k++) {
-        const size_t i = base + k;
-        if (i >= n) break;
-        if (!isnan(xs[threadIdx.x * RN_PAD + k])) wpush(run, xs[threadIdx.x * RN_PAD + k]);
-        float r = rs[threadIdx.x * RN_PAD + k];
-        if (run.n >= 2.0) {
-            const double sd = sqrt(run.m2 / run.n + 1e-8);
-            float z = (float)((double)r / sd);
-            z = z < -clip ? -clip : z;
-            z = z > clip ? clip : z;
-            r = z;
-        }
-        rs[threadIdx.x * RN_PAD + k] = r;
-    }
-    __syncthreads();
-    const size_t b0 = (size_t)blockIdx.x * RN_SEG;
-    for (int k = threadIdx.x; k < RN_SEG; k += RN_BLOCK)
-        if (b0 + k < n) rew[b0 + k] = rs[(k / RN_IPT) * RN_PAD + (k % RN_IPT)];
+    __shared__ RnApplyLds l;
+    rn_apply_role(blockIdx.x, n, X, rew_raw, agg, clip, rew, l);
+}
+
+void launch_rn_agg_scan(bppo_ctx *c, int nb) {
+    hipLaunchKernelGGL(k_rn_agg_scan, dim3(1), dim3(1024), 0, c->stream, nb, c->d_scan_agg,
+                       c->d_rn_stats);
 }
 
 bppo_status launch_return_norm(bppo_ctx *c) {
     const size_t n = (size_t)c->T * c->N;
     const int nb = (int)((n + RN_SEG - 1) / RN_SEG);
-    if (c->wide)
-        hipLaunchKernelGGL(k_rn_returns_mp, dim3((c->N + 255) / 256), dim3(256), 0, c->stream, c->T, c->N, c->P,
-                           c->cfg.gamma, c->d_rew_raw, c->d_done, c->d_players, c->n_opp ? c->d_valid : nullptr,
-                           c->d_rn_returns, c->d_X);
-    else
-        hipLaunchKernelGGL(k_rn_returns, dim3((c->N + 255) / 256), dim3(256), 0, c->stream, c->T, c->N,
-                           c->cfg.gamma, c->d_rew_raw, c->d_done, c->d_rn_returns, c->d_X);
+    hipLaunchKernelGGL(k_rn_returns_mp, dim3((c->N + 255) / 256), dim3(256), 0, c->stream, c->T, c->N, c->P,
+                       c->cfg.gamma, c->d_rew_raw, c->d_done, c->d_players, c->n_opp ? c->d_valid : nullptr,
+                       c->d_rn_returns, c->d_X);
     hipLaunchKernelGGL(k_rn_block_agg, dim3(nb), dim3(RN_BLOCK), 0, c->stream, n, c->d_X,
                        c->d_scan_agg);
-    hipLaunchKernelGGL(k_rn_agg_scan, dim3(1), dim3(1024), 0, c->stream, nb, c->d_scan_agg,
-                       c->d_rn_stats);
+    launch_rn_agg_scan(c, nb);
     hipLaunchKernelGGL(k_rn_apply, dim3(nb), dim3(RN_BLOCK), 0, c->stream, n, c->d_X, c->d_rew_raw,
                        c->d_scan_agg, (float)c->cfg.return_clip, c->d_rew);
-    if (c->wide)
-        hipLaunchKernelGGL(k_rn_scatter_acting, dim3((unsigned)std::min<size_t>((n + 255) / 256, 4096)), dim3(256), 0,
-                           c->stream, n, c->P, c->d_players, c->d_rew, c->d_allr);
+    hipLaunchKernelGGL(k_rn_scatter_acting, dim3((unsigned)std::min<size_t>((n + 255) / 256, 4096)), dim3(256), 0,
+                       c->stream, n, c->P, c->d_players, c->d_rew, c->d_allr);
     TRY(launch_check(c, __func__));
     return BPPO_OK;
 }
diff --git a/burn-ppo_amd/csrc/k_rollout.hip b/burn-ppo_amd/csrc/k_rollout.hip
--- a/burn-ppo_amd/csrc/k_rollout.hip
+++ b/burn-ppo_amd/csrc/k_rollout.hip
@@ -1,5 +1,6 @@
 #include "bppo_internal.h"
 #include "bppo_mlp64.h"
+#include "bppo_retnorm.h"
 
 namespace bppo {
 
@@ -205,12 +206,11 @@
 }
 
 constexpr int GUM_THREADS = 256;
-__global__ void __launch_bounds__(GUM_THREADS) k_gumbel_words(Key8 key, uint64_t stream, uint64_t base,
-                                                              uint64_t count, float *__restrict__ g,
-                                                              int32_t *zero0, int32_t *zero1) {
-    __shared__ float tile[16 * GUM_THREADS + GUM_THREADS / 2];
-    if (blockIdx.x == 0 && threadIdx.x == 0) { *zero0 = 0; *zero1 = 0; }
-    const uint64_t blk0 = (base >> 4) + blockIdx.x * (uint64_t)GUM_THREADS;
+__device__ __forceinline__ void gumbel_words_role(int bid, float *tile, Key8 key, uint64_t stream, uint64_t base,
+                                                  uint64_t count, float *__restrict__ g,
+                                                  int32_t *zero0, int32_t *zero1) {
+    if (bid == 0 && threadIdx.x == 0) { *zero0 = 0; *zero1 = 0; }
+    const uint64_t blk0 = (base >> 4) + bid * (uint64_t)GUM_THREADS;
     const uint64_t b = blk0 + threadIdx.x, wb = blk0 * 16;
     if (b * 16 < base + count) {
         uint32_t blk[16];
@@ -230,9 +230,10 @@
     }
 }
 
-__global__ void __launch_bounds__(256) k_reset_pool(int N, int K, uint64_t seed_base, const uint64_t *__restrict__ env_pos,
-                                                    float4 *__restrict__ pool, uint64_t *__restrict__ ppos) {
-    const int e = blockIdx.x * blockDim.x + threadIdx.x;
+__device__ __forceinline__ void reset_pool_role(int bid, int N, int K, uint64_t seed_base,
+                                                const uint64_t *__restrict__ env_pos,
+                                                float4 *__restrict__ pool, uint64_t *__restrict__ ppos) {
+    const int e = bid * blockDim.x + threadIdx.x;
     if (e >= N) return;
     WordCursor c;
     c.init(seed_key(seed_base + (uint64_t)e), 0, env_pos[e]);
@@ -242,6 +243,18 @@
         pool[(size_t)j * N + e] = make_float4(s.x, s.x_dot, s.theta, s.theta_dot);
         ppos[(size_t)j * N + e] = c.pos;
     }
+}
+
+struct PreRolloutArgs {
+    int n_gum;
+    Key8 key; uint64_t stream, base, count; float *g; int32_t *zero0, *zero1;
+    int N, K; uint64_t seed_base; const uint64_t *env_pos; float4 *pool; uint64_t *ppos;
+};
+__global__ void __launch_bounds__(GUM_THREADS) k_pre_rollout(PreRolloutArgs a) {
+    __shared__ float tile[16 * GUM_THREADS + GUM_THREADS / 2];
+    const int b = blockIdx.x;
+    if (b < a.n_gum) gumbel_words_role(b, tile, a.key, a.stream, a.base, a.count, a.g, a.zero0, a.zero1);
+    else reset_pool_role(b - a.n_gum, a.N, a.K, a.seed_base, a.env_pos, a.pool, a.ppos);
 }
 
 __global__ void __launch_bounds__(512, 2) k_cartpole_rollout_mfma(RolloutArgs a, const float *__restrict__ gum) {
@@ -728,15 +741,14 @@
 }
 
 template <int H, int NL, int ACT>
-__global__ void __launch_bounds__(256) k_cartpole_bootstrap(int N, const float *cp,
-                                                            const int32_t *steps,
-                                                            const float *params, const double *on,
-                                                            int norm_on, float *last_v) {
-    extern __shared__ __attribute__((aligned(16))) float sP[];
+__device__ __forceinline__ void cartpole_bootstrap_role(int bid, float *sP, int N, const float *cp,
+                                                        const int32_t *steps,
+                                                        const float *params, const double *on,
+                                                        int norm_on, float *last_v) {
     constexpr CpOffsets O = cp_offsets<H, NL>();
     for (int i = threadIdx.x; i < O.n; i += blockDim.x) sP[i] = params[i];
     __syncthreads();
-    int e = blockIdx.x * blockDim.x + threadIdx.x;
+    int e = bid * blockDim.x + threadIdx.x;
     if (e >= N) return;
     CartPoleState s;
     load_state(cp, steps, N, e, s);
@@ -768,10 +780,13 @@
 }
 
 constexpr int OBS_PART_BLOCKS = 64, OBS_MAX_D = 8;
-__global__ void __launch_bounds__(256) k_obs_norm_part(int N, int D, double T, const double *part, double *bp) {
-    __shared__ double sn[256], sm[256][OBS_MAX_D], sq[256][OBS_MAX_D];
-    const int per = (N + gridDim.x - 1) / gridDim.x;
-    const int e0 = blockIdx.x * per, e1 = min(N, e0 + per);
+struct ObsPartLds { double sn[256], sm[256][OBS_MAX_D], sq[256][OBS_MAX_D]; };
+__device__ __forceinline__ void obs_norm_part_role(int bid, int nblk, ObsPartLds &l, int N, int D, double T,
+                                                   const double *part, double *bp) {
+    double (&sn)[256] = l.sn;
+    double (&sm)[256][OBS_MAX_D] = l.sm, (&sq)[256][OBS_MAX_D] = l.sq;
+    const int per = (N + nblk - 1) / nblk;
+    const int e0 = bid * per, e1 = min(N, e0 + per);
     double n = 0.0, mean[OBS_MAX_D], m2[OBS_MAX_D];
     for (int d = 0; d < OBS_MAX_D; d++) mean[d] = m2[d] = 0.0;
     for (int e = e0 + threadIdx.x; e < e1; e += blockDim.x) {
@@ -803,11 +818,11 @@
         __syncthreads();
     }
     if (threadIdx.x < D) {
-        double *o = bp + ((size_t)blockIdx.x * OBS_MAX_D + threadIdx.x) * 3;
+        double *o = bp + ((size_t)bid * OBS_MAX_D + threadIdx.x) * 3;
         o[0] = sn[0]; o[1] = sm[0][threadIdx.x]; o[2] = sq[0][threadIdx.x];
     }
 }
-__global__ void k_obs_norm_final(int D, int nblk, const double *bp, double *on) {
+__device__ __forceinline__ void obs_norm_final_role(int D, int nblk, const double *bp, double *on) {
     const int d = threadIdx.x;
     if (d >= D) return;
     double n = 0.0, mean = 0.0, m2 = 0.0;
@@ -889,23 +904,24 @@
         }
         const uint64_t count = (uint64_t)c->T * c->N * 2;
         const uint64_t blocks = ((base_pos + count + 15) >> 4) - (base_pos >> 4);
-        hipLaunchKernelGGL(k_gumbel_words, dim3((unsigned)((blocks + 255) / 256)), dim3(256), 0, c->stream,
-                           c->rng_key, (uint64_t)c->cfg.rng_stream, base_pos, count, c->d_gumbel, c->d_ep_count,
-                           (int32_t *)c->d_err);
-        TRY(launch_check(c, "k_gumbel_words"));
+        const int pk = std::max(0, std::min(RPOOL_K, env_int("BPPO_RESET_POOL_K", RPOOL_K)));
+        const bool pool = lanes64 && c->d_rpool && pk > 0;
+        PreRolloutArgs pa;
+        pa.n_gum = (int)((blocks + 255) / 256);
+        pa.key = c->rng_key; pa.stream = (uint64_t)c->cfg.rng_stream; pa.base = base_pos; pa.count = count;
+        pa.g = c->d_gumbel; pa.zero0 = c->d_ep_count; pa.zero1 = (int32_t *)c->d_err;
+        pa.N = c->N; pa.K = pk; pa.seed_base = c->cfg.env_seed_base; pa.env_pos = (const uint64_t *)c->d_env_pos;
+        pa.pool = c->d_rpool; pa.ppos = c->d_rpos;
+        hipLaunchKernelGGL(k_pre_rollout, dim3((unsigned)(pa.n_gum + (pool ? (c->N + 255) / 256 : 0))), dim3(GUM_THREADS),
+                           0, c->stream, pa);
+        TRY(launch_check(c, "k_pre_rollout"));
+        if (pool) { a.rpool = c->d_rpool; a.rpos = c->d_rpos; a.rpool_k = pk; }
         if (!lanes64) {
             const int waves = (c->N + mmb::TR - 1) / mmb::TR;
             hipLaunchKernelGGL(k_cartpole_rollout_mfma, dim3((waves + mmb::WAVES - 1) / mmb::WAVES), dim3(64 * mmb::WAVES),
                                mmb::LDS, c->stream, a, (const float *)c->d_gumbel);
         } else {
             const int waves = (c->N + 63) / 64;
-            const int pk = std::max(0, std::min(RPOOL_K, env_int("BPPO_RESET_POOL_K", RPOOL_K)));
-            if (c->d_rpool && pk > 0) {
-                hipLaunchKernelGGL(k_reset_pool, dim3((c->N + 255) / 256), dim3(256), 0, c->stream, c->N, pk,
-                                   c->cfg.env_seed_base, (const uint64_t *)c->d_env_pos, c->d_rpool, c->d_rpos);
-                TRY(launch_check(c, "k_reset_pool"));
-                a.rpool = c->d_rpool; a.rpos = c->d_rpos; a.rpool_k = pk;
-            }
 #ifdef BPPO_RO_STAMPS
             static unsigned long long *d_st = nullptr;
             if (!d_st) BPPO_HIP(c, hipMalloc((void **)&d_st, sizeof(unsigned long long) * (size_t)waves * RO_NSEG));
@@ -943,18 +959,6 @@
     return BPPO_ERR_UNSUPPORTED;
 }
 
-bppo_status launch_bootstrap(bppo_ctx *c, const double *, const double *, int norm_on) {
-    const int h = c->cfg.hidden_size, nl = c->cfg.num_hidden;
-    dim3 grid((c->N + 255) / 256), blk(256);
-#define L(H_, NL_, A_)                                                                          \
-    hipLaunchKernelGGL((k_cartpole_bootstrap<H_, NL_, A_>), grid, blk, (cp_lds<H_, NL_>(A_, 256)), c->stream, c->N, c->d_cp, \
-                       c->d_steps, c->d_params, c->d_on, norm_on, c->d_last_v)
-    CP_DISPATCH(16, 1, L) CP_DISPATCH(16, 2, L) CP_DISPATCH(32, 1, L) CP_DISPATCH(32, 2, L)
-    CP_DISPATCH(64, 1, L) CP_DISPATCH(64, 2, L)
-#undef L
-    return BPPO_ERR_UNSUPPORTED;
-}
-
 bppo_status launch_forward_rows(bppo_ctx *c, const float *d_obs, int B, float *d_logits,
                                 float *d_values) {
     const int h = c->cfg.hidden_size, nl = c->cfg.num_hidden;
@@ -1058,55 +1062,126 @@
 __global__ void k_obsw_count(int D, double add, double *on) { on[2 * D] += add; }
 
 bppo_status launch_obs_norm_merge(bppo_ctx *c) {
-    if (c->wide) {
-        const size_t rows = (size_t)c->T * c->N;
-        if ((size_t)OBSW_CHUNKS * c->D * 3 > c->obsw_part_n) { c->err = "obs normalizer scratch too small"; return BPPO_ERR_ARG; }
-        hipLaunchKernelGGL(k_obsw_part, dim3((c->D + 255) / 256, OBSW_CHUNKS), dim3(256), 0, c->stream, rows, c->D,
-                           c->d_obs_raw, c->d_obsw_part);
-        hipLaunchKernelGGL(k_obsw_final, dim3((c->D + 255) / 256), dim3(256), 0, c->stream, c->D, OBSW_CHUNKS,
-                           c->d_obsw_part, c->d_on);
-        hipLaunchKernelGGL(k_obsw_count, dim3(1), dim3(1), 0, c->stream, c->D, (double)rows, c->d_on);
-        TRY(launch_check(c, __func__));
-        return BPPO_OK;
-    }
-    if (c->D > OBS_MAX_D) { c->err = "observation normalizer: obs dim > 8"; return BPPO_ERR_UNSUPPORTED; }
-    const int nblk = std::min(OBS_PART_BLOCKS, std::max(1, (c->N + 255) / 256));
-    hipLaunchKernelGGL(k_obs_norm_part, dim3(nblk), dim3(256), 0, c->stream, c->N, c->D, (double)c->T,
-                       c->d_obs_part, c->d_red);
-    hipLaunchKernelGGL(k_obs_norm_final, dim3(1), dim3(64), 0, c->stream, c->D, nblk, c->d_red, c->d_on);
+    const size_t rows = (size_t)c->T * c->N;
+    if ((size_t)OBSW_CHUNKS * c->D * 3 > c->obsw_part_n) { c->err = "obs normalizer scratch too small"; return BPPO_ERR_ARG; }
+    hipLaunchKernelGGL(k_obsw_part, dim3((c->D + 255) / 256, OBSW_CHUNKS), dim3(256), 0, c->stream, rows, c->D,
+                       c->d_obs_raw, c->d_obsw_part);
+    hipLaunchKernelGGL(k_obsw_final, dim3((c->D + 255) / 256), dim3(256), 0, c->stream, c->D, OBSW_CHUNKS,
+                       c->d_obsw_part, c->d_on);
+    hipLaunchKernelGGL(k_obsw_count, dim3(1), dim3(1), 0, c->stream, c->D, (double)rows, c->d_on);
     TRY(launch_check(c, __func__));
     return BPPO_OK;
 }
 
-__global__ void __launch_bounds__(256) k_ep_summary(const EpisodeRec *eps, const int32_t *count, const int32_t *err,
-                                                    int cap, double *host_slot) {
+__device__ __forceinline__ void ep_summary_role(int bid, double (&sh)[2][4], const EpisodeRec *eps, const int32_t *count,
+                                                const int32_t *err, int cap, double *host_slot) {
     const int cnt = *count;
     const int n = min(cnt, cap);
     double *part = host_slot + 2;
-    if (blockIdx.x == 0 && threadIdx.x == 0) {
+    if (bid == 0 && threadIdx.x == 0) {
         int32_t *hv = reinterpret_cast<int32_t *>(host_slot);
         hv[0] = cnt;
         hv[1] = *err;
     }
     double sr = 0.0, sl = 0.0;
-    for (int i = blockIdx.x * blockDim.x + threadIdx.x; i < n; i += gridDim.x * blockDim.x) {
+    for (int i = bid * blockDim.x + threadIdx.x; i < n; i += EP_SUMMARY_BLOCKS * blockDim.x) {
         sr += (double)eps[i].total_reward[0];
         sl += (double)eps[i].length;
     }
-    __shared__ double sh[2][4];
     for (int o = 32; o > 0; o >>= 1) { sr += __shfl_down(sr, o, 64); sl += __shfl_down(sl, o, 64); }
     const int w = threadIdx.x >> 6;
     if ((threadIdx.x & 63) == 0) { sh[0][w] = sr; sh[1][w] = sl; }
     __syncthreads();
     if (threadIdx.x == 0) {
-        part[2 * blockIdx.x] = sh[0][0] + sh[0][1] + sh[0][2] + sh[0][3];
-        part[2 * blockIdx.x + 1] = sh[1][0] + sh[1][1] + sh[1][2] + sh[1][3];
-    }
+        part[2 * bid] = sh[0][0] + sh[0][1] + sh[0][2] + sh[0][3];
+        part[2 * bid + 1] = sh[1][0] + sh[1][1] + sh[1][2] + sh[1][3];
+    }
+}
+
+struct PostHeadArgs {
+    int n_ret, n_obs;
+    int T, N; double gamma; const float *rew_raw, *done; double *returns_state, *X;
+    int D; const double *obs_part; double *bp;
+    const EpisodeRec *eps; const int32_t *count, *err; int cap; double *slot;
+};
+__global__ void __launch_bounds__(256) k_post_head(PostHeadArgs a) {
+    __shared__ union { ObsPartLds obs; double sum[2][4]; } l;
+    const int b = blockIdx.x;
+    if (b < a.n_ret) rn_returns_role(b, a.T, a.N, a.gamma, a.rew_raw, a.done, a.returns_state, a.X);
+    else if (b < a.n_ret + a.n_obs) obs_norm_part_role(b - a.n_ret, a.n_obs, l.obs, a.N, a.D, (double)a.T, a.obs_part, a.bp);
+    else ep_summary_role(b - a.n_ret - a.n_obs, l.sum, a.eps, a.count, a.err, a.cap, a.slot);
+}
+
+__global__ void __launch_bounds__(RN_BLOCK) k_post_mid(int n_agg, size_t n, const double *X, Welford *agg, int D,
+                                                       int n_obs, const double *bp, double *on) {
+    __shared__ RnAggLds l;
+    const int b = blockIdx.x;
+    if (b < n_agg) rn_block_agg_role(b, n, X, agg, l);
+    else obs_norm_final_role(D, n_obs, bp, on);
+}
+
+struct PostTailArgs {
+    int n_app;
+    size_t n; const double *X; const float *rew_raw; const Welford *agg; float clip; float *rew;
+    int N; const float *cp; const int32_t *steps; const float *params; const double *on; int norm_on; float *last_v;
+};
+template <int H, int NL, int ACT>
+__global__ void __launch_bounds__(RN_BLOCK) k_post_tail(PostTailArgs a) {
+    extern __shared__ __attribute__((aligned(16))) float smem[];
+    const int b = blockIdx.x;
+    if (b < a.n_app) rn_apply_role(b, a.n, a.X, a.rew_raw, a.agg, a.clip, a.rew, *reinterpret_cast<RnApplyLds *>(smem));
+    else cartpole_bootstrap_role<H, NL, ACT>(b - a.n_app, smem, a.N, a.cp, a.steps, a.params, a.on, a.norm_on, a.last_v);
+}
+
+static bppo_status launch_post_tail(bppo_ctx *c, bool apply, bool boot) {
+    const int h = c->cfg.hidden_size, nl = c->cfg.num_hidden;
+    const size_t n = (size_t)c->T * c->N;
+    PostTailArgs a;
+    a.n_app = apply ? (int)((n + RN_SEG - 1) / RN_SEG) : 0;
+    a.n = n; a.X = c->d_X; a.rew_raw = c->d_rew_raw; a.agg = c->d_scan_agg; a.clip = (float)c->cfg.return_clip;
+    a.rew = c->d_rew;
+    a.N = c->N; a.cp = c->d_cp; a.steps = c->d_steps; a.params = c->d_params; a.on = c->d_on;
+    a.norm_on = c->cfg.normalize_obs; a.last_v = c->d_last_v;
+    const dim3 grid(a.n_app + (boot ? (c->N + 255) / 256 : 0)), blk(RN_BLOCK);
+    if (grid.x == 0) return BPPO_OK;
+#define L(H_, NL_, A_)                                                                                             \
+    hipLaunchKernelGGL((k_post_tail<H_, NL_, A_>), grid, blk,                                                      \
+                       std::max(apply ? sizeof(RnApplyLds) : (size_t)0, boot ? cp_lds<H_, NL_>(A_, 256) : (size_t)0), \
+                       c->stream, a)
+    CP_DISPATCH(16, 1, L) CP_DISPATCH(16, 2, L) CP_DISPATCH(32, 1, L) CP_DISPATCH(32, 2, L)
+    CP_DISPATCH(64, 1, L) CP_DISPATCH(64, 2, L)
+#undef L
+    return BPPO_ERR_UNSUPPORTED;
+}
+
+bppo_status launch_bootstrap(bppo_ctx *c) { return launch_post_tail(c, false, true); }
+
+bppo_status launch_post_rollout(bppo_ctx *c, double *host_slot, bool boot) {
+    const bool rn = c->cfg.normalize_returns, on = c->cfg.normalize_obs;
+    if (on && c->D > OBS_MAX_D) { c->err = "observation normalizer: obs dim > 8"; return BPPO_ERR_UNSUPPORTED; }
+    const size_t n = (size_t)c->T * c->N;
+    const int nb = (int)((n + RN_SEG - 1) / RN_SEG);
+    PostHeadArgs a;
+    a.n_ret = rn ? (c->N + 255) / 256 : 0;
+    a.n_obs = on ? std::min(OBS_PART_BLOCKS, std::max(1, (c->N + 255) / 256)) : 0;
+    a.T = c->T; a.N = c->N; a.gamma = c->cfg.gamma; a.rew_raw = c->d_rew_raw; a.done = c->d_done;
+    a.returns_state = c->d_rn_returns; a.X = c->d_X;
+    a.D = c->D; a.obs_part = c->d_obs_part; a.bp = c->d_red;
+    a.eps = c->d_eps; a.count = c->d_ep_count; a.err = (const int32_t *)c->d_err; a.cap = c->eps_cap; a.slot = host_slot;
+    const int n_head = a.n_ret + a.n_obs + (host_slot ? EP_SUMMARY_BLOCKS : 0);
+    if (n_head > 0) hipLaunchKernelGGL(k_post_head, dim3(n_head), dim3(256), 0, c->stream, a);
+    if (rn || on)
+        hipLaunchKernelGGL(k_post_mid, dim3((rn ? nb : 0) + (on ? 1 : 0)), dim3(RN_BLOCK), 0, c->stream, rn ? nb : 0, n,
+                           (const double *)c->d_X, c->d_scan_agg, c->D, a.n_obs, (const double *)c->d_red, c->d_on);
+    if (rn) launch_rn_agg_scan(c, nb);
+    TRY(launch_check(c, __func__));
+    return launch_post_tail(c, rn, boot);
 }
 
 bppo_status launch_episode_summary(bppo_ctx *c, double *host_slot) {
-    hipLaunchKernelGGL(k_ep_summary, dim3(EP_SUMMARY_BLOCKS), dim3(256), 0, c->stream, c->d_eps, c->d_ep_count,
-                       (const int32_t *)c->d_err, c->eps_cap, host_slot);
+    PostHeadArgs a{};
+    a.eps = c->d_eps; a.count = c->d_ep_count; a.err = (const int32_t *)c->d_err; a.cap = c->eps_cap; a.slot = host_slot;
+    hipLaunchKernelGGL(k_post_head, dim3(EP_SUMMARY_BLOCKS), dim3(256), 0, c->stream, a);
     TRY(launch_check(c, __func__));
     return BPPO_OK;
 }
```

Result: slower. 756.1 million (-2.6%).
